# erlgo/openair4G

Measured on AMD Instinct MI355X. Metric: DL subframes/sec (20 MHz, 2x2, 64-QAM), higher is better.
Workload: dtype int16; 1 GPU; dlsim 20 MHz 2x2 TM3 (LARGE_CDD) 64-QAM MCS19x2CW, 2x14 IDFT-2048; config_id=C3, global_batch=8192, subframe_index=7, full_grid=False, parallelism=subframe-sharded x1

## Files before the change

include/oai4g.h:

```cpp
#ifndef OAI4G_H
#define OAI4G_H

#include <stddef.h>
#include <stdint.h>

#ifdef __cplusplus
extern "C" {
#endif

#define OAI4G_LTE_NULL 2
#define OAI4G_NSOFT 1827072
#define OAI4G_MAX_SEGMENTS 16
#define OAI4G_MAX_CHANNEL_BITS (14 * 1200 * 6)
#define OAI4G_D_BYTES (96 + 12 + 3 + 3 * 6144)
#define OAI4G_W_BYTES (3 * 6144 + 96)

enum {
  OAI4G_SISO = 0,
  OAI4G_ALAMOUTI = 1,
  OAI4G_LARGE_CDD = 2,
  OAI4G_UNIFORM_PRECODING11 = 3,
  OAI4G_UNIFORM_PRECODING1m1 = 4,
  OAI4G_UNIFORM_PRECODING1j = 5,
  OAI4G_UNIFORM_PRECODING1mj = 6,
  OAI4G_PUSCH_PRECODING0 = 7,
  OAI4G_PUSCH_PRECODING1 = 8
};
enum { OAI4G_CYCLIC_PREFIX = 0, OAI4G_CYCLIC_SUFFIX = 1, OAI4G_ZEROS = 2, OAI4G_NONE = 3 };

typedef struct {
  uint16_t N_RB_DL;
  uint16_t Nid_cell;
  uint8_t Ncp;
  uint8_t nushift;
  uint8_t mode1_flag;
  uint8_t nb_antennas_tx;
  uint8_t frame_type;
  uint8_t symbols_per_tti;
  uint8_t log2_symbol_size;
  uint8_t Nid_cell_mbsfn;
  uint16_t ofdm_symbol_size;
  uint16_t first_carrier_offset;
  uint16_t nb_prefix_samples;
  uint16_t nb_prefix_samples0;
  uint32_t samples_per_tti;
  uint8_t phich_resource;
  uint8_t phich_duration;
  uint8_t tdd_config;
  uint8_t nb_antennas_tx_eNB;
} oai4g_frame_parms_t;

typedef struct {
  uint8_t dci_length;
  uint8_t L;
  int32_t nCCE;
  uint8_t ra_flag;
  uint16_t rnti;
  uint32_t format;
  uint8_t dci_pdu[8];
} oai4g_dci_alloc_t;

typedef struct {
  uint32_t TBS;
  uint32_t B;
  uint8_t *b;
  uint8_t *c[OAI4G_MAX_SEGMENTS];
  uint32_t RTC[OAI4G_MAX_SEGMENTS];
  uint8_t round;
  uint8_t mcs;
  uint8_t rvidx;
  uint8_t mimo_mode;
  uint32_t rb_alloc[4];
  uint16_t nb_rb;
  uint8_t *e;
  uint8_t *d[OAI4G_MAX_SEGMENTS];
  uint8_t *w[OAI4G_MAX_SEGMENTS];
  uint32_t C, Cminus, Cplus, Kminus, Kplus, F;
  uint8_t Nl;
  uint8_t Nlayers;
  uint8_t first_layer;
  uint16_t pmi_alloc;
} oai4g_dl_harq_t;

typedef struct {
  uint16_t rnti;
  uint8_t current_harq_pid;
  uint8_t Mdlharq;
  uint8_t Kmimo;
  int16_t sqrt_rho_a;
  int16_t sqrt_rho_b;
  oai4g_dl_harq_t *harq_processes[8];
} oai4g_dlsch_t;

int oai4g_init(void);
const char *oai4g_last_error(void);
int oai4g_device_name(char *buf, int len);

int oai4g_init_frame_parms(oai4g_frame_parms_t *fp, uint16_t N_RB_DL, uint16_t Nid_cell, uint8_t Ncp,
                           uint8_t nb_antennas_tx, uint8_t mode1_flag, uint8_t frame_type);
uint8_t oai4g_get_Qm(uint8_t mcs);
int oai4g_get_G(const oai4g_frame_parms_t *fp, uint16_t nb_rb, const uint32_t *rb_alloc, uint8_t mod_order,
                uint8_t Nl, uint8_t num_pdcch_symbols, int frame, uint8_t subframe);
uint8_t oai4g_get_Qm_ul(uint8_t mcs);
uint8_t oai4g_get_I_TBS(uint8_t mcs);
uint8_t oai4g_get_I_TBS_UL(uint8_t mcs);
uint32_t oai4g_tbs_bits(uint8_t I_TBS, uint16_t nb_rb);
uint32_t oai4g_get_TBS_DL(uint8_t mcs, uint16_t nb_rb);
uint32_t oai4g_get_TBS_UL(uint8_t mcs, uint16_t nb_rb);
oai4g_dlsch_t *oai4g_new_dlsch(uint8_t Kmimo, uint8_t Mdlharq, uint8_t N_RB_DL);
void oai4g_free_dlsch(oai4g_dlsch_t *dlsch);
uint32_t oai4g_lte_gold_generic(uint32_t *x1, uint32_t *x2, uint8_t reset);
int oai4g_qpp_fold32(uint32_t K, uint32_t *s, uint16_t *tab);
int oai4g_rsc_scan_rows(uint32_t q, uint32_t rows[6]);
int oai4g_rm_pair_schedule(uint32_t C, uint32_t n0, const uint32_t nt[2], const uint32_t wrapt[2],
                           uint32_t *pairs, uint32_t *pair0);
int oai4g_mod_item_map(uint32_t item, uint32_t ips, uint32_t lz, uint32_t per, uint32_t *sf, uint32_t *l,
                       uint32_t *pair);
uint8_t oai4g_get_pmi(uint8_t N_RB_DL, uint8_t mimo_mode, uint16_t pmi_alloc, uint16_t rb);
void oai4g_set_modofdm_grid_cap(int n_workgroups);

uint32_t oai4g_crc24a(const uint8_t *in, int bitlen);
uint32_t oai4g_crc24b(const uint8_t *in, int bitlen);
int oai4g_lte_segmentation(const uint8_t *input_buffer, uint8_t **output_buffers, uint32_t B, uint32_t *C,
                           uint32_t *Cplus, uint32_t *Cminus, uint32_t *Kplus, uint32_t *Kminus, uint32_t *F);
void oai4g_threegpplte_turbo_encoder(const uint8_t *input, uint16_t input_length_bytes, uint8_t *output,
                                     uint8_t F, uint16_t interleaver_f1, uint16_t interleaver_f2);
uint32_t oai4g_sub_block_interleaving_turbo(uint32_t D, uint8_t *d, uint8_t *w);
uint32_t oai4g_lte_rate_matching_turbo(uint32_t RTC, uint32_t G, const uint8_t *w, uint8_t *e, uint8_t C,
                                       uint32_t Nsoft, uint8_t Mdlharq, uint8_t Kmimo, uint8_t rvidx,
                                       uint8_t Qm, uint8_t Nl, uint8_t r, uint8_t nb_rb, uint8_t m);
int oai4g_dlsch_encoding(uint8_t *a, const oai4g_frame_parms_t *frame_parms, uint8_t num_pdcch_symbols,
                         oai4g_dlsch_t *dlsch, int frame, uint8_t subframe);
void oai4g_dlsch_scrambling(const oai4g_frame_parms_t *frame_parms, int mbsfn_flag, oai4g_dlsch_t *dlsch, int G,
                            uint8_t q, uint8_t Ns);
int oai4g_dlsch_modulation(int32_t **txdataF, int16_t amp, uint32_t subframe_offset,
                           const oai4g_frame_parms_t *frame_parms, uint8_t num_pdcch_symbols,
                           oai4g_dlsch_t *dlsch0, oai4g_dlsch_t *dlsch1);
void oai4g_PHY_ofdm_mod(const int32_t *input, int32_t *output, uint8_t log2fftsize, uint8_t nb_symbols,
                        uint16_t nb_prefix_samples, int etype);
void oai4g_normal_prefix_mod(const int32_t *txdataF, int32_t *txdata, uint8_t nsymb,
                             const oai4g_frame_parms_t *frame_parms);
void oai4g_do_OFDM_mod(int32_t **txdataF, int32_t **txdata, uint32_t frame, uint16_t next_slot,
                       const oai4g_frame_parms_t *frame_parms);
void oai4g_generate_pilots(int32_t **txdataF, int16_t amp, const oai4g_frame_parms_t *frame_parms, uint16_t Ntti);
int oai4g_lte_dl_cell_spec(int32_t *output, int16_t amp, const oai4g_frame_parms_t *frame_parms, uint8_t Ns,
                           uint8_t l, uint8_t p);
int oai4g_idft(int log2n, const int16_t *x, int16_t *y, int scale);
void oai4g_idft2048(const int16_t *x, int16_t *y, int scale);
void oai4g_idft1024(const int16_t *x, int16_t *y, int scale);
void oai4g_idft512(const int16_t *x, int16_t *y, int scale);
void oai4g_idft256(const int16_t *x, int16_t *y, int scale);
void oai4g_idft128(const int16_t *x, int16_t *y, int scale);
void oai4g_idft64(const int16_t *x, int16_t *y, int scale);

void oai4g_generate_pcfich_reg_mapping(const oai4g_frame_parms_t *frame_parms, uint16_t pcfich_reg[4],
                                       uint8_t *pcfich_first_reg_idx);
int oai4g_generate_pcfich(uint8_t num_pdcch_symbols, int16_t amp, const oai4g_frame_parms_t *frame_parms,
                          int32_t **txdataF, uint8_t subframe);

uint8_t oai4g_get_mi(const oai4g_frame_parms_t *frame_parms, uint8_t subframe);
uint16_t oai4g_get_nquad(uint8_t num_pdcch_symbols, const oai4g_frame_parms_t *frame_parms, uint8_t mi);
uint16_t oai4g_get_nCCE(uint8_t num_pdcch_symbols, const oai4g_frame_parms_t *frame_parms, uint8_t mi);
uint8_t oai4g_get_num_pdcch_symbols(uint8_t num_dci, const oai4g_dci_alloc_t *dci_alloc,
                                    const oai4g_frame_parms_t *frame_parms, uint8_t subframe);
int oai4g_generate_phich_reg_mapping(const oai4g_frame_parms_t *frame_parms, uint16_t phich_reg[56][3]);
void oai4g_init_nCCE_table(void);
int oai4g_get_nCCE_offset(uint8_t L, int nCCE, int common_dci, uint16_t rnti, uint8_t subframe);
uint8_t oai4g_generate_dci_top(uint8_t num_ue_spec_dci, uint8_t num_common_dci, const oai4g_dci_alloc_t *dci_alloc,
                               uint32_t n_rnti, int16_t amp, const oai4g_frame_parms_t *frame_parms,
                               int32_t **txdataF, uint32_t subframe);

int oai4g_phy_viterbi_lte(const int8_t *y, uint8_t *decoded_bytes, uint16_t n);
int oai4g_diag_viterbi_lte(const int8_t *y, uint16_t n, uint8_t *decoded, uint8_t metrics[64], uint8_t *start_state);
int oai4g_cc_rx_plan(uint32_t D, uint16_t *plan);
int oai4g_dci_decoding(uint8_t DCI_LENGTH, uint8_t aggregation_level, const int8_t *e, uint8_t *decoded_output);
int oai4g_dci_decoding_crc(uint8_t DCI_LENGTH, uint8_t aggregation_level, const int8_t *e, uint8_t *decoded_output,
                           uint16_t *crc);
int oai4g_pbch_decode(const int8_t *llr, const oai4g_frame_parms_t *frame_parms, uint8_t frame_mod4,
                      uint8_t decoded_output[3]);
int oai4g_pbch_decode_batch(const int8_t *d_llr, int n, const oai4g_frame_parms_t *frame_parms,
                            const uint8_t *d_frame_mod4, uint8_t *d_out, void *stream);

int oai4g_pdcch_soft_bit_table(const oai4g_frame_parms_t *frame_parms, uint8_t subframe, uint8_t num_pdcch_symbols,
                               uint32_t *table, uint32_t cap);
int oai4g_pdcch_soft_bits(const int32_t *rxdataF_comp, const oai4g_frame_parms_t *frame_parms, uint8_t subframe,
                          uint8_t num_pdcch_symbols, int8_t *e_rx);
int oai4g_pdcch_candidates(const oai4g_frame_parms_t *frame_parms, uint8_t num_pdcch_symbols, uint8_t subframe,
                           uint16_t crnti, int do_common, uint8_t L, uint16_t *cce, int cap);
int oai4g_dci_decoding_procedure0(const int8_t *e_rx, uint8_t num_pdcch_symbols, uint16_t crnti, uint8_t *nCCE,
                                  int do_common, uint8_t subframe, oai4g_dci_alloc_t *dci_alloc,
                                  const oai4g_frame_parms_t *frame_parms, uint8_t mi, uint16_t si_rnti, uint16_t ra_rnti,
                                  uint8_t L, uint8_t format_si, uint8_t format_ra, uint8_t format_c, uint8_t sizeof_bits,
                                  uint8_t sizeof_bytes, uint8_t *dci_cnt, uint8_t *format0_found, uint8_t *format_c_found,
                                  uint32_t *CCEmap0, uint32_t *CCEmap1, uint32_t *CCEmap2);

typedef struct {
  uint8_t do_common, L, sizeof_bits, sizeof_bytes, format_si, format_ra, format_c, stop_if_found;
} oai4g_pdcch_plan_t;
#define OAI4G_PDCCH_MAX_DCI 8
typedef struct {
  uint8_t dci_cnt, format0_found, format_c_found;
  uint8_t overflow;
  int32_t nCCE;
  uint32_t CCEmap[3];
  oai4g_dci_alloc_t dci[OAI4G_PDCCH_MAX_DCI];
} oai4g_pdcch_rx_result_t;
typedef struct oai4g_pdcch_rx_config oai4g_pdcch_rx_config_t;
oai4g_pdcch_rx_config_t *oai4g_pdcch_rx_config_create(const oai4g_frame_parms_t *frame_parms, uint8_t num_pdcch_symbols,
                                                      uint16_t crnti, uint16_t si_rnti, uint16_t ra_rnti,
                                                      const oai4g_pdcch_plan_t *plan, int n_plan);
void oai4g_pdcch_rx_config_destroy(oai4g_pdcch_rx_config_t *cfg);
int oai4g_pdcch_rx_candidates(const oai4g_pdcch_rx_config_t *cfg, uint8_t subframe, uint16_t *cce, uint8_t *plan_entry,
                              int cap);
int oai4g_pdcch_rx_batch(oai4g_pdcch_rx_config_t *cfg, const int32_t *d_comp, int n_sf, int first_subframe,
                         oai4g_pdcch_rx_result_t *d_out, void *stream);
int oai4g_pdcch_rx_batch_detected(oai4g_pdcch_rx_config_t *const cfg[3], const int32_t *d_comp, const uint8_t *d_cfi,
                                  int n_sf, int first_subframe, int subframe_step, oai4g_pdcch_rx_result_t *d_out,
                                  void *stream);

int oai4g_rx_pdcch_front(int32_t *const *rxdataF, int32_t *const *dl_ch_estimates, const oai4g_frame_parms_t *frame_parms,
                         uint8_t nb_antennas_rx, uint8_t subframe, uint8_t mimo_mode, uint32_t high_speed_flag,
                         int32_t *rxdataF_comp, uint8_t *log2_maxh, uint8_t *num_pdcch_symbols, int32_t *diag_planes);
int oai4g_rx_pcfich(const oai4g_frame_parms_t *frame_parms, uint8_t subframe, const int32_t *rxdataF_comp, uint8_t mimo_mode);
int oai4g_rx_pdcch(int32_t *const *rxdataF, int32_t *const *dl_ch_estimates, const oai4g_frame_parms_t *frame_parms,
                   uint8_t nb_antennas_rx, uint8_t subframe, uint8_t mimo_mode, uint32_t high_speed_flag, int8_t *e_rx,
                   uint8_t *num_pdcch_symbols);
typedef struct oai4g_pdcch_front_config oai4g_pdcch_front_config_t;
oai4g_pdcch_front_config_t *oai4g_pdcch_front_config_create(const oai4g_frame_parms_t *frame_parms, uint8_t nb_antennas_rx,
                                                            uint8_t mimo_mode, uint32_t high_speed_flag,
                                                            uint8_t first_subframe, uint8_t subframe_step);
void oai4g_pdcch_front_config_destroy(oai4g_pdcch_front_config_t *cfg);
int oai4g_pdcch_front_batch(const oai4g_pdcch_front_config_t *cfg, int n_sf, const int32_t *d_rxdataF,
                            const int32_t *const d_est[4], int32_t *d_comp, uint8_t *d_cfi, uint8_t *d_log2_maxh,
                            void *stream);

int oai4g_rx_pbch_front(int32_t *const *rxdataF, int32_t *const *dl_ch_estimates, const oai4g_frame_parms_t *frame_parms,
                        uint8_t nb_antennas_rx, uint8_t nb_ports, uint8_t mimo_mode, uint32_t high_speed_flag,
                        int32_t *rxdataF_comp, uint8_t log2_maxh[4], int8_t *llr, int32_t *diag_planes);
int oai4g_rx_pbch(int32_t *const *rxdataF, int32_t *const *dl_ch_estimates, const oai4g_frame_parms_t *frame_parms,
                  uint8_t nb_antennas_rx, uint8_t nb_ports, uint8_t mimo_mode, uint32_t high_speed_flag,
                  uint8_t frame_mod4, uint8_t decoded_output[3]);
typedef struct oai4g_pbch_front_config oai4g_pbch_front_config_t;
oai4g_pbch_front_config_t *oai4g_pbch_front_config_create(const oai4g_frame_parms_t *frame_parms, uint8_t nb_antennas_rx,
                                                          uint8_t nb_ports, uint32_t high_speed_flag);
void oai4g_pbch_front_config_destroy(oai4g_pbch_front_config_t *cfg);
int oai4g_pbch_front_batch(const oai4g_pbch_front_config_t *cfg, int n, const int32_t *d_rxdataF,
                           const int32_t *const d_est[4], int8_t *d_llr, uint8_t *d_log2_maxh, void *stream);
typedef struct {
  uint8_t tx_ant;
  uint8_t frame_mod4, mimo_mode;
  uint8_t mib[3];
  uint8_t pad[2];
} oai4g_pbch_detect_t;
int oai4g_pbch_detect_batch(oai4g_pbch_front_config_t *cfg, int n, const int8_t *d_llr, oai4g_pbch_detect_t *d_out,
                            void *stream);

int oai4g_lte_sync_time_replicas(const oai4g_frame_parms_t *frame_parms, int32_t *out);
typedef struct oai4g_sync_config oai4g_sync_config_t;
oai4g_sync_config_t *oai4g_sync_config_create(const oai4g_frame_parms_t *frame_parms, uint8_t nb_antennas_rx);
void oai4g_sync_config_destroy(oai4g_sync_config_t *cfg);
int oai4g_sync_time_batch(oai4g_sync_config_t *cfg, int n, const int32_t *d_rx, int32_t *d_peak, int32_t *d_corr,
                          void *stream);
int oai4g_lte_sync_time(int32_t *const *rxdata, const oai4g_frame_parms_t *frame_parms, uint8_t nb_antennas_rx, int *eNB_id,
                        uint32_t *peak_val, int32_t *sync_corr);

int oai4g_fep_offset_batch(const oai4g_frame_parms_t *frame_parms, int n, int nb_antennas_rx, const int32_t *d_rx,
                           const int32_t *d_offset, uint32_t offset_stride, uint8_t first_slot, int nsym, int32_t *d_rxF,
                           size_t frame_stride, void *stream);
typedef struct {
  int32_t Nid_cell, rx_offset, metric, flip, phase, status;
} oai4g_cell_t;
int oai4g_sss_batch(oai4g_sync_config_t *cfg, int n, const int32_t *d_rx, const int32_t *d_peak, oai4g_cell_t *d_cell,
// ... 362 lines not shown
```

openair4g_amd/__init__.py:

```python
import ctypes
import os

import numpy as np

_HERE = os.path.dirname(os.path.abspath(__file__))
LIB_PATH = os.path.join(_HERE, "lib", "libopenair4g_amd.so")

LTE_NULL = 2
NSOFT = 1827072
MAX_SEGMENTS = 16
MAX_CHANNEL_BITS = 14 * 1200 * 6
D_BYTES = 96 + 12 + 3 + 3 * 6144
W_BYTES = 3 * 6144 + 96
SISO, ALAMOUTI, LARGE_CDD = 0, 1, 2
(UNIFORM_PRECODING11, UNIFORM_PRECODING1m1, UNIFORM_PRECODING1j, UNIFORM_PRECODING1mj, PUSCH_PRECODING0,
 PUSCH_PRECODING1) = 3, 4, 5, 6, 7, 8
CYCLIC_PREFIX = 0


class OAI4GError(RuntimeError):
    pass


u8p = ctypes.POINTER(ctypes.c_uint8)
# ... 168 lines not shown
                                                       ctypes.c_uint8, ctypes.c_uint8, ctypes.c_uint8, ctypes.c_uint8]),
    "oai4g_chest_filters": (None, [ctypes.c_uint8, ctypes.c_void_p]),
    "oai4g_chest_dc_filters": (None, [ctypes.c_uint8, ctypes.c_void_p]),
    "oai4g_ul_config_set_decoder": (ctypes.c_int, [ctypes.c_void_p, ctypes.c_int]),
    "oai4g_set_device": (ctypes.c_int, [ctypes.c_int]),
    "oai4g_dist_unique_id": (ctypes.c_int, [ctypes.c_void_p]),
    "oai4g_dist_init": (ctypes.c_int, [ctypes.c_int, ctypes.c_int, ctypes.c_void_p]),
    "oai4g_dist_broadcast_params": (ctypes.c_int, [ctypes.c_void_p, ctypes.c_int]),
    "oai4g_dist_allreduce_sum_u64": (ctypes.c_int, [ctypes.c_void_p, ctypes.c_int]),
    "oai4g_dist_allreduce_max_f64": (ctypes.c_int, [ctypes.c_void_p, ctypes.c_int]),
    "oai4g_dist_barrier": (ctypes.c_int, []),
    "oai4g_dist_rank": (ctypes.c_int, []),
    "oai4g_dist_world": (ctypes.c_int, []),
    "oai4g_dist_finalize": (ctypes.c_int, []),
    "oai4g_shard_range": (None, [ctypes.c_int, ctypes.c_int, ctypes.c_int, ctypes.POINTER(ctypes.c_int),
                                 ctypes.POINTER(ctypes.c_int)]),
    "oai4g_payload_seed": (ctypes.c_uint64, [ctypes.c_uint64, ctypes.c_uint64, ctypes.c_uint32, ctypes.c_uint32]),
    "oai4g_chest_config_set_stride": (ctypes.c_int, [ctypes.c_void_p, ctypes.c_uint32, ctypes.c_uint32]),
    "oai4g_rx_pdsch_tm3": (ctypes.c_int, [ctypes.POINTER(FrameParms), ctypes.c_int, ctypes.c_void_p, ctypes.c_void_p,
                                          ctypes.c_void_p, ctypes.c_uint8, ctypes.c_uint8, ctypes.c_uint8,
                                          ctypes.c_uint8, ctypes.c_uint8, ctypes.c_void_p, ctypes.c_void_p]),
    "oai4g_rx_config_create_tm3": (ctypes.c_void_p, [ctypes.POINTER(FrameParms), ctypes.c_void_p, ctypes.c_uint8,
                                                     ctypes.c_uint8, ctypes.c_uint8, ctypes.c_uint8, ctypes.c_uint16,
                                                     ctypes.c_uint8, ctypes.c_uint8, ctypes.c_uint8]),
    "oai4g_rx_batch_tm3": (ctypes.c_int, [ctypes.c_void_p, ctypes.c_int, ctypes.c_void_p, ctypes.c_void_p,
                                          ctypes.c_void_p, ctypes.c_int, ctypes.c_void_p]),
    "oai4g_rx_pdsch_tm3_2cw": (ctypes.c_int, [ctypes.POINTER(FrameParms), ctypes.c_int, ctypes.c_void_p,
                                              ctypes.c_void_p, ctypes.c_void_p, ctypes.c_uint8, ctypes.c_uint8,
                                              ctypes.c_uint8, ctypes.c_void_p, ctypes.c_void_p, ctypes.c_void_p]),
    "oai4g_rx_batch_tm3_2cw": (ctypes.c_int, [ctypes.c_void_p, ctypes.c_int, ctypes.c_void_p, ctypes.c_void_p,
                                              ctypes.c_void_p, ctypes.c_void_p, ctypes.c_int, ctypes.c_void_p]),
    "oai4g_rx_pdsch_tm2": (ctypes.c_int, [ctypes.POINTER(FrameParms), ctypes.c_int, ctypes.c_void_p, ctypes.c_void_p,
                                          ctypes.c_void_p, ctypes.c_uint8, ctypes.c_uint8, ctypes.c_uint8,
                                          ctypes.c_void_p, ctypes.c_void_p]),
    "oai4g_rx_config_create_tm2": (ctypes.c_void_p, [ctypes.POINTER(FrameParms), ctypes.c_void_p, ctypes.c_uint8,
                                                     ctypes.c_uint8, ctypes.c_uint16, ctypes.c_uint8, ctypes.c_uint8,
                                                     ctypes.c_uint8]),
    "oai4g_rx_batch_tm2": (ctypes.c_int, [ctypes.c_void_p, ctypes.c_int, ctypes.c_void_p, ctypes.c_void_p,
                                          ctypes.c_void_p, ctypes.c_int, ctypes.c_void_p]),
    "oai4g_rx_pdsch_tm56": (ctypes.c_int, [ctypes.POINTER(FrameParms), ctypes.c_int, ctypes.c_void_p, ctypes.c_void_p,
                                           ctypes.c_void_p, ctypes.c_uint8, ctypes.c_uint8, ctypes.c_uint16,
                                           ctypes.c_uint8, ctypes.c_uint8, ctypes.c_uint8, ctypes.c_void_p,
                                           ctypes.c_void_p]),
    "oai4g_rx_config_create_tm56": (ctypes.c_void_p, [ctypes.POINTER(FrameParms), ctypes.c_void_p, ctypes.c_uint8,
                                                      ctypes.c_uint8, ctypes.c_uint16, ctypes.c_int, ctypes.c_uint8,
                                                      ctypes.c_uint8, ctypes.c_uint16, ctypes.c_uint8, ctypes.c_uint8,
                                                      ctypes.c_uint8]),
    "oai4g_rx_batch_tm56": (ctypes.c_int, [ctypes.c_void_p, ctypes.c_int, ctypes.c_void_p, ctypes.c_void_p,
                                           ctypes.c_void_p, ctypes.c_int, ctypes.c_void_p]),
    "oai4g_rx_batch_tm56_pilots": (ctypes.c_int, [ctypes.c_void_p, ctypes.c_int, ctypes.c_void_p, ctypes.c_void_p,
                                                  ctypes.c_void_p, ctypes.c_int, ctypes.c_void_p]),
    "oai4g_dl_ch_estimates_time": (ctypes.c_int, [ctypes.POINTER(FrameParms), ctypes.c_int, ctypes.c_void_p,
                                                  ctypes.c_void_p]),
    "oai4g_chest_time_batch": (ctypes.c_int, [ctypes.POINTER(FrameParms), ctypes.c_int, ctypes.c_void_p,
                                              ctypes.c_size_t, ctypes.c_void_p, ctypes.c_size_t, ctypes.c_void_p]),
    "oai4g_lte_est_freq_offset": (ctypes.c_int, [ctypes.c_void_p, ctypes.POINTER(FrameParms), ctypes.c_int,
                                                 ctypes.POINTER(ctypes.c_int), ctypes.c_int]),
    "oai4g_freq_offset_omega_batch": (ctypes.c_int, [ctypes.POINTER(FrameParms), ctypes.c_int, ctypes.c_void_p,
                                                     ctypes.c_size_t, ctypes.c_int, ctypes.c_void_p, ctypes.c_void_p]),
    "oai4g_freq_offset_update": (ctypes.c_int, [ctypes.POINTER(FrameParms), ctypes.c_int32,
                                                ctypes.POINTER(ctypes.c_int), ctypes.POINTER(ctypes.c_int)]),
    "oai4g_signal_energy": (ctypes.c_int32, [ctypes.c_void_p, ctypes.c_uint32]),
    "oai4g_signal_energy_batch": (ctypes.c_int, [ctypes.c_void_p, ctypes.c_int, ctypes.c_size_t, ctypes.c_uint32,
                                                 ctypes.c_void_p, ctypes.c_void_p]),
    "oai4g_awgn_batch": (ctypes.c_int, [ctypes.c_void_p, ctypes.c_size_t, ctypes.c_uint32, ctypes.c_void_p,
                                        ctypes.c_uint32, ctypes.c_void_p, ctypes.c_size_t, ctypes.c_int,
                                        ctypes.c_void_p, ctypes.c_double, ctypes.c_uint64, ctypes.c_uint32,
                                        ctypes.c_void_p]),
    "oai4g_chest_config_create": (ctypes.c_void_p, [ctypes.POINTER(FrameParms), ctypes.c_uint8, ctypes.c_uint8,
                                                    ctypes.c_uint8]),
    "oai4g_chest_config_destroy": (None, [ctypes.c_void_p]),
    "oai4g_rx_batch_estimated": (ctypes.c_int, [ctypes.c_void_p, ctypes.c_void_p, ctypes.c_int, ctypes.c_void_p,
                                                ctypes.c_void_p, ctypes.c_int, ctypes.c_void_p]),
    "oai4g_chest_batch": (ctypes.c_int, [ctypes.c_void_p, ctypes.c_int, ctypes.c_void_p, ctypes.c_void_p,
                                         ctypes.c_void_p]),
    "oai4g_chest_batch_pilots": (ctypes.c_int, [ctypes.c_void_p, ctypes.c_int, ctypes.c_void_p, ctypes.c_void_p,
                                                ctypes.c_void_p]),
    "oai4g_rx_batch_tm3_pilots": (ctypes.c_int, [ctypes.c_void_p, ctypes.c_int, ctypes.c_void_p, ctypes.c_void_p,
                                                 ctypes.c_void_p, ctypes.c_int, ctypes.c_void_p]),
    "oai4g_rx_batch_tm3_2cw_pilots": (ctypes.c_int, [ctypes.c_void_p, ctypes.c_int, ctypes.c_void_p, ctypes.c_void_p,
                                                     ctypes.c_void_p, ctypes.c_void_p, ctypes.c_int, ctypes.c_void_p]),
    "oai4g_phy_threegpplte_turbo_decoder8": (ctypes.c_uint8, [ctypes.c_void_p, ctypes.c_void_p, ctypes.c_uint16,
                                                              ctypes.c_uint16, ctypes.c_uint16, ctypes.c_uint8,
                                                              ctypes.c_uint8, ctypes.c_uint8]),
    "oai4g_td8_scratch_bytes": (ctypes.c_size_t, [ctypes.c_uint16, ctypes.c_int]),
    "oai4g_td8_batch": (ctypes.c_int, [ctypes.c_int, ctypes.c_uint16, ctypes.c_void_p, ctypes.c_size_t, ctypes.c_void_p,
                                       ctypes.c_size_t, ctypes.c_void_p, ctypes.c_uint8, ctypes.c_uint8, ctypes.c_uint8,
                                       ctypes.c_void_p, ctypes.c_void_p]),
    "oai4g_generate_dummy_w": (ctypes.c_uint32, [ctypes.c_uint32, ctypes.c_void_p, ctypes.c_uint8]),
    "oai4g_ul_config_create": (ctypes.c_void_p, [ctypes.c_uint32, ctypes.c_uint32, ctypes.c_uint8, ctypes.c_uint8,
                                                 ctypes.c_uint8, ctypes.c_uint32, ctypes.c_uint8]),
    "oai4g_ul_config_destroy": (None, [ctypes.c_void_p]),
    "oai4g_ul_config_C": (ctypes.c_int, [ctypes.c_void_p]),
    "oai4g_ul_config_E": (ctypes.c_uint32, [ctypes.c_void_p, ctypes.c_int]),
    "oai4g_ul_config_G_offset": (ctypes.c_uint32, [ctypes.c_void_p, ctypes.c_int]),
    "oai4g_ul_decode_batch": (ctypes.c_int, [ctypes.c_void_p, ctypes.c_int, ctypes.c_void_p, ctypes.c_size_t,
                                             ctypes.c_void_p, ctypes.c_size_t, ctypes.c_void_p, ctypes.c_void_p]),
    "oai4g_ul_config_w_entries": (ctypes.c_size_t, [ctypes.c_void_p]),
    "oai4g_ul_decode_batch_harq": (ctypes.c_int, [ctypes.c_void_p, ctypes.c_int, ctypes.c_void_p, ctypes.c_size_t,
                                                  ctypes.c_void_p, ctypes.c_size_t, ctypes.c_uint8, ctypes.c_uint8,
                                                  ctypes.c_void_p, ctypes.c_size_t, ctypes.c_void_p, ctypes.c_void_p]),
    "oai4g_dft": (ctypes.c_int, [ctypes.c_int, ctypes.c_void_p, ctypes.c_void_p, ctypes.c_int]),
    "oai4g_dft2048": (None, [ctypes.c_void_p, ctypes.c_void_p, ctypes.c_int]),
    "oai4g_dft1024": (None, [ctypes.c_void_p, ctypes.c_void_p, ctypes.c_int]),
    "oai4g_dft512": (None, [ctypes.c_void_p, ctypes.c_void_p, ctypes.c_int]),
    "oai4g_dft256": (None, [ctypes.c_void_p, ctypes.c_void_p, ctypes.c_int]),
    "oai4g_dft128": (None, [ctypes.c_void_p, ctypes.c_void_p, ctypes.c_int]),
    "oai4g_dft64": (None, [ctypes.c_void_p, ctypes.c_void_p, ctypes.c_int]),
    "oai4g_slot_fep_offset": (ctypes.c_int64, [ctypes.POINTER(FrameParms), ctypes.c_uint8, ctypes.c_uint8,
                                               ctypes.c_int, ctypes.c_int]),
    "oai4g_slot_fep": (ctypes.c_int, [ctypes.POINTER(ctypes.c_void_p), ctypes.POINTER(ctypes.c_void_p),
                                      ctypes.POINTER(FrameParms), ctypes.c_uint8, ctypes.c_uint8, ctypes.c_uint8,
                                      ctypes.c_int, ctypes.c_int]),
    "oai4g_fep_batch": (ctypes.c_int, [ctypes.POINTER(FrameParms), ctypes.c_int, ctypes.c_int, ctypes.c_void_p,
                                       ctypes.c_void_p, ctypes.c_void_p]),
    "oai4g_tx_config_create": (ctypes.c_void_p, [ctypes.POINTER(TxParams)]),
    "oai4g_tx_config_destroy": (None, [ctypes.c_void_p]),
    "oai4g_tx_G": (ctypes.c_uint32, [ctypes.c_void_p, ctypes.c_int, ctypes.c_int]),
    "oai4g_tx_ebits_words": (ctypes.c_uint32, [ctypes.c_void_p]),
    "oai4g_tx_iq_samples": (ctypes.c_uint32, [ctypes.c_void_p]),
    "oai4g_tx_workspace_bytes": (ctypes.c_size_t, [ctypes.c_void_p, ctypes.c_int]),
    "oai4g_tx_batch": (ctypes.c_int, [ctypes.c_void_p, ctypes.c_int, ctypes.c_void_p, ctypes.c_void_p,
                                      ctypes.c_void_p, ctypes.c_void_p]),
    "oai4g_tx_batch_timed": (ctypes.c_int, [ctypes.c_void_p, ctypes.c_int, ctypes.c_void_p, ctypes.c_void_p,
                                            ctypes.c_void_p, ctypes.c_void_p, ctypes.POINTER(ctypes.c_float)]),
    "oai4g_tx_encode": (ctypes.c_int, [ctypes.c_void_p, ctypes.c_int, ctypes.c_void_p, ctypes.c_void_p,
                                       ctypes.c_void_p]),
    "oai4g_tx_modulate": (ctypes.c_int, [ctypes.c_void_p, ctypes.c_int, ctypes.c_void_p, ctypes.c_void_p,
                                         ctypes.c_void_p]),
    "oai4g_tx_mod_nosat": (ctypes.c_int, [ctypes.c_void_p]),
    "oai4g_diag_encode_phase_ms": (ctypes.c_int, [ctypes.c_void_p, ctypes.c_int, ctypes.c_void_p, ctypes.c_void_p,
                                                  ctypes.c_int, ctypes.c_int, ctypes.POINTER(ctypes.c_float)]),
    "oai4g_diag_encode_occupancy": (ctypes.c_int, [ctypes.c_void_p, ctypes.POINTER(ctypes.c_int),
                                                   ctypes.POINTER(ctypes.c_size_t)]),
    "oai4g_diag_stream": (ctypes.c_int, [ctypes.c_void_p, ctypes.c_void_p, ctypes.c_size_t, ctypes.c_int,
                                         ctypes.c_void_p]),
    "oai4g_dev_alloc": (ctypes.c_void_p, [ctypes.c_size_t]),
    "oai4g_dev_free": (None, [ctypes.c_void_p]),
    "oai4g_memcpy_h2d": (ctypes.c_int, [ctypes.c_void_p, ctypes.c_void_p, ctypes.c_size_t]),
    "oai4g_memcpy_d2h": (ctypes.c_int, [ctypes.c_void_p, ctypes.c_void_p, ctypes.c_size_t]),
    "oai4g_memset_d": (ctypes.c_int, [ctypes.c_void_p, ctypes.c_int, ctypes.c_size_t]),
    "oai4g_sync": (ctypes.c_int, []),
    "oai4g_fill_payload": (ctypes.c_int, [ctypes.c_void_p, ctypes.c_size_t, ctypes.c_uint64, ctypes.c_void_p]),
    "oai4g_qpp_fold32": (ctypes.c_int, [ctypes.c_uint32, ctypes.POINTER(ctypes.c_uint32), ctypes.c_void_p]),
    "oai4g_rsc_scan_rows": (ctypes.c_int, [ctypes.c_uint32, ctypes.POINTER(ctypes.c_uint32)]),
    "oai4g_rm_pair_schedule": (ctypes.c_int, [ctypes.c_uint32, ctypes.c_uint32, ctypes.POINTER(ctypes.c_uint32),
                                              ctypes.POINTER(ctypes.c_uint32), ctypes.POINTER(ctypes.c_uint32),
                                              ctypes.POINTER(ctypes.c_uint32)]),
    "oai4g_mod_item_map": (ctypes.c_int, [ctypes.c_uint32, ctypes.c_uint32, ctypes.c_uint32, ctypes.c_uint32,
                                          ctypes.POINTER(ctypes.c_uint32), ctypes.POINTER(ctypes.c_uint32),
                                          ctypes.POINTER(ctypes.c_uint32)]),
    "oai4g_get_pmi": (ctypes.c_uint8, [ctypes.c_uint8, ctypes.c_uint8, ctypes.c_uint16, ctypes.c_uint16]),
    "oai4g_set_modofdm_grid_cap": (None, [ctypes.c_int]),
    "oai4g_tx_mod_lz": (ctypes.c_int, [ctypes.c_void_p]),
    "oai4g_harq_advance": (ctypes.c_int, [ctypes.c_int, ctypes.c_int, ctypes.c_uint8, ctypes.c_int, ctypes.c_int]
                           + [ctypes.c_void_p] * 8 + [ctypes.c_size_t, ctypes.c_uint64, ctypes.c_void_p]),
    "oai4g_tx_config_enable_tb_rv": (ctypes.c_int, [ctypes.c_void_p]),
    "oai4g_tx_batch_rv": (ctypes.c_int, [ctypes.c_void_p, ctypes.c_int, ctypes.c_void_p, ctypes.c_void_p,
                                         ctypes.c_void_p, ctypes.c_void_p, ctypes.c_void_p]),
    "oai4g_tx_encode_rv": (ctypes.c_int, [ctypes.c_void_p, ctypes.c_int, ctypes.c_void_p, ctypes.c_void_p,
                                          ctypes.c_void_p, ctypes.c_void_p]),
    "oai4g_ul_decode_batch_harq_tb": (ctypes.c_int, [ctypes.c_void_p, ctypes.c_int, ctypes.c_void_p, ctypes.c_size_t,
                                                     ctypes.c_void_p, ctypes.c_size_t, ctypes.c_void_p, ctypes.c_void_p,
                                                     ctypes.c_void_p, ctypes.c_size_t, ctypes.c_void_p, ctypes.c_void_p]),
    "oai4g_phy_viterbi_lte": (ctypes.c_int, [ctypes.c_void_p, ctypes.c_void_p, ctypes.c_uint16]),
    "oai4g_diag_viterbi_lte": (ctypes.c_int, [ctypes.c_void_p, ctypes.c_uint16, ctypes.c_void_p, ctypes.c_void_p,
                                              ctypes.c_void_p]),
    "oai4g_cc_rx_plan": (ctypes.c_int, [ctypes.c_uint32, ctypes.c_void_p]),
    "oai4g_dci_decoding": (ctypes.c_int, [ctypes.c_uint8, ctypes.c_uint8, ctypes.c_void_p, ctypes.c_void_p]),
    "oai4g_dci_decoding_crc": (ctypes.c_int, [ctypes.c_uint8, ctypes.c_uint8, ctypes.c_void_p, ctypes.c_void_p,
                                              ctypes.POINTER(ctypes.c_uint16)]),
    "oai4g_pbch_decode": (ctypes.c_int, [ctypes.c_void_p, ctypes.POINTER(FrameParms), ctypes.c_uint8, ctypes.c_void_p]),
    "oai4g_pbch_decode_batch": (ctypes.c_int, [ctypes.c_void_p, ctypes.c_int, ctypes.POINTER(FrameParms),
                                               ctypes.c_void_p, ctypes.c_void_p, ctypes.c_void_p]),
    "oai4g_pdcch_soft_bit_table": (ctypes.c_int, [ctypes.POINTER(FrameParms), ctypes.c_uint8, ctypes.c_uint8,
                                                  ctypes.c_void_p, ctypes.c_uint32]),
    "oai4g_pdcch_soft_bits": (ctypes.c_int, [ctypes.c_void_p, ctypes.POINTER(FrameParms), ctypes.c_uint8, ctypes.c_uint8,
                                             ctypes.c_void_p]),
    "oai4g_dci_decoding_procedure0": (ctypes.c_int, [ctypes.c_void_p, ctypes.c_uint8, ctypes.c_uint16, ctypes.c_void_p,
                                                     ctypes.c_int, ctypes.c_uint8, ctypes.c_void_p,
                                                     ctypes.POINTER(FrameParms), ctypes.c_uint8, ctypes.c_uint16,
                                                     ctypes.c_uint16] + [ctypes.c_uint8] * 6 + [ctypes.c_void_p] * 6),
    "oai4g_pdcch_candidates": (ctypes.c_int, [ctypes.POINTER(FrameParms), ctypes.c_uint8, ctypes.c_uint8, ctypes.c_uint16,
                                              ctypes.c_int, ctypes.c_uint8, ctypes.c_void_p, ctypes.c_int]),
    "oai4g_pdcch_rx_config_create": (ctypes.c_void_p, [ctypes.POINTER(FrameParms), ctypes.c_uint8, ctypes.c_uint16,
                                                       ctypes.c_uint16, ctypes.c_uint16, ctypes.c_void_p, ctypes.c_int]),
    "oai4g_pdcch_rx_config_destroy": (None, [ctypes.c_void_p]),
    "oai4g_pdcch_rx_candidates": (ctypes.c_int, [ctypes.c_void_p, ctypes.c_uint8, ctypes.c_void_p, ctypes.c_void_p,
                                                 ctypes.c_int]),
    "oai4g_pdcch_rx_batch": (ctypes.c_int, [ctypes.c_void_p, ctypes.c_void_p, ctypes.c_int, ctypes.c_int, ctypes.c_void_p,
                                            ctypes.c_void_p]),
    "oai4g_pdcch_rx_batch_detected": (ctypes.c_int, [ctypes.POINTER(ctypes.c_void_p), ctypes.c_void_p, ctypes.c_void_p,
                                                     ctypes.c_int, ctypes.c_int, ctypes.c_int, ctypes.c_void_p,
                                                     ctypes.c_void_p]),
    "oai4g_rx_pdcch_front": (ctypes.c_int, [ctypes.POINTER(ctypes.c_void_p), ctypes.POINTER(ctypes.c_void_p),
                                            ctypes.POINTER(FrameParms), ctypes.c_uint8, ctypes.c_uint8, ctypes.c_uint8,
                                            ctypes.c_uint32, ctypes.c_void_p, ctypes.POINTER(ctypes.c_uint8),
                                            ctypes.POINTER(ctypes.c_uint8), ctypes.c_void_p]),
    "oai4g_rx_pcfich": (ctypes.c_int, [ctypes.POINTER(FrameParms), ctypes.c_uint8, ctypes.c_void_p, ctypes.c_uint8]),
    "oai4g_rx_pdcch": (ctypes.c_int, [ctypes.POINTER(ctypes.c_void_p), ctypes.POINTER(ctypes.c_void_p),
                                      ctypes.POINTER(FrameParms), ctypes.c_uint8, ctypes.c_uint8, ctypes.c_uint8,
                                      ctypes.c_uint32, ctypes.c_void_p, ctypes.POINTER(ctypes.c_uint8)]),
    "oai4g_pdcch_front_config_create": (ctypes.c_void_p, [ctypes.POINTER(FrameParms), ctypes.c_uint8, ctypes.c_uint8,
                                                          ctypes.c_uint32, ctypes.c_uint8, ctypes.c_uint8]),
    "oai4g_pdcch_front_config_destroy": (None, [ctypes.c_void_p]),
    "oai4g_pdcch_front_batch": (ctypes.c_int, [ctypes.c_void_p, ctypes.c_int, ctypes.c_void_p,
                                               ctypes.POINTER(ctypes.c_void_p), ctypes.c_void_p, ctypes.c_void_p,
                                               ctypes.c_void_p, ctypes.c_void_p]),
    "oai4g_rx_pbch_front": (ctypes.c_int, [ctypes.POINTER(ctypes.c_void_p), ctypes.POINTER(ctypes.c_void_p),
                                           ctypes.POINTER(FrameParms), ctypes.c_uint8, ctypes.c_uint8, ctypes.c_uint8,
                                           ctypes.c_uint32, ctypes.c_void_p, ctypes.c_void_p, ctypes.c_void_p,
                                           ctypes.c_void_p]),
    "oai4g_rx_pbch": (ctypes.c_int, [ctypes.POINTER(ctypes.c_void_p), ctypes.POINTER(ctypes.c_void_p),
                                     ctypes.POINTER(FrameParms), ctypes.c_uint8, ctypes.c_uint8, ctypes.c_uint8,
                                     ctypes.c_uint32, ctypes.c_uint8, ctypes.c_void_p]),
    "oai4g_pbch_front_config_create": (ctypes.c_void_p, [ctypes.POINTER(FrameParms), ctypes.c_uint8, ctypes.c_uint8,
                                                         ctypes.c_uint32]),
    "oai4g_pbch_front_config_destroy": (None, [ctypes.c_void_p]),
    "oai4g_pbch_front_batch": (ctypes.c_int, [ctypes.c_void_p, ctypes.c_int, ctypes.c_void_p,
                                              ctypes.POINTER(ctypes.c_void_p), ctypes.c_void_p, ctypes.c_void_p,
                                              ctypes.c_void_p]),
    "oai4g_pbch_detect_batch": (ctypes.c_int, [ctypes.c_void_p, ctypes.c_int, ctypes.c_void_p, ctypes.c_void_p,
                                               ctypes.c_void_p]),
    "oai4g_lte_sync_time_replicas": (ctypes.c_int, [ctypes.POINTER(FrameParms), ctypes.c_void_p]),
    "oai4g_sync_config_create": (ctypes.c_void_p, [ctypes.POINTER(FrameParms), ctypes.c_uint8]),
    "oai4g_sync_config_destroy": (None, [ctypes.c_void_p]),
    "oai4g_sync_time_batch": (ctypes.c_int, [ctypes.c_void_p, ctypes.c_int, ctypes.c_void_p, ctypes.c_void_p,
                                             ctypes.c_void_p, ctypes.c_void_p]),
    "oai4g_lte_sync_time": (ctypes.c_int, [ctypes.POINTER(ctypes.c_void_p), ctypes.POINTER(FrameParms), ctypes.c_uint8,
                                           ctypes.POINTER(ctypes.c_int), ctypes.POINTER(ctypes.c_uint32),
                                           ctypes.c_void_p]),
    "oai4g_fep_offset_batch": (ctypes.c_int, [ctypes.POINTER(FrameParms), ctypes.c_int, ctypes.c_int, ctypes.c_void_p,
                                              ctypes.c_void_p, ctypes.c_uint32, ctypes.c_uint8, ctypes.c_int,
                                              ctypes.c_void_p, ctypes.c_size_t, ctypes.c_void_p]),
    "oai4g_sss_batch": (ctypes.c_int, [ctypes.c_void_p, ctypes.c_int, ctypes.c_void_p, ctypes.c_void_p, ctypes.c_void_p,
                                       ctypes.c_void_p]),
    "oai4g_sss_rows_batch": (ctypes.c_int, [ctypes.c_void_p, ctypes.c_int, ctypes.c_void_p, ctypes.c_void_p,
                                            ctypes.c_void_p, ctypes.c_void_p]),
    "oai4g_rx_sss": (ctypes.c_int, [ctypes.POINTER(ctypes.c_void_p), ctypes.POINTER(FrameParms), ctypes.c_uint8,
                                    ctypes.c_uint8, ctypes.c_int, ctypes.POINTER(ctypes.c_int32),
                                    ctypes.POINTER(ctypes.c_uint8), ctypes.POINTER(ctypes.c_uint8)]),
    "oai4g_initial_sync": (ctypes.c_int, [ctypes.POINTER(ctypes.c_void_p), ctypes.POINTER(FrameParms), ctypes.c_uint8,
                                          ctypes.c_uint8, ctypes.c_uint32, ctypes.c_void_p]),
    "oai4g_rx_phich": (ctypes.c_int, [ctypes.POINTER(FrameParms), ctypes.c_uint8, ctypes.c_void_p, ctypes.c_uint8,
                                      ctypes.c_uint8, ctypes.POINTER(ctypes.c_int16)]),
    "oai4g_phich_rx_config_create": (ctypes.c_void_p, [ctypes.POINTER(FrameParms), ctypes.c_uint8, ctypes.c_uint8]),
    "oai4g_phich_rx_config_destroy": (None, [ctypes.c_void_p]),
    "oai4g_phich_rx_batch": (ctypes.c_int, [ctypes.c_void_p, ctypes.c_void_p, ctypes.c_int, ctypes.c_void_p, ctypes.c_int,
                                            ctypes.c_void_p, ctypes.c_void_p]),
    "oai4g_channel_config_create": (ctypes.c_void_p, [ctypes.c_uint8, ctypes.c_uint8, ctypes.c_int, ctypes.c_double,
                                                      ctypes.c_double, ctypes.c_int32, ctypes.c_double, ctypes.c_int]),
    "oai4g_channel_config_destroy": (None, [ctypes.c_void_p]),
    "oai4g_channel_config_query": (ctypes.c_int, [ctypes.c_void_p, ctypes.c_void_p, ctypes.c_void_p]),
    "oai4g_channel_model_describe": (ctypes.c_int, [ctypes.c_int, ctypes.c_uint8, ctypes.c_uint8, ctypes.c_double,
                                                    ctypes.c_void_p, ctypes.c_void_p]),
    "oai4g_channel_random_batch": (ctypes.c_int, [ctypes.c_void_p, ctypes.c_int, ctypes.c_uint64, ctypes.c_uint32,
                                                  ctypes.c_uint32, ctypes.c_void_p, ctypes.c_void_p]),
    "oai4g_channel_set_taps": (ctypes.c_int, [ctypes.c_void_p, ctypes.c_int, ctypes.c_int, ctypes.c_void_p, ctypes.c_void_p]),
    "oai4g_channel_get_taps": (ctypes.c_int, [ctypes.c_void_p, ctypes.c_int, ctypes.c_int, ctypes.c_void_p, ctypes.c_void_p]),
    "oai4g_multipath_batch": (ctypes.c_int, [ctypes.c_void_p, ctypes.c_int, ctypes.c_void_p, ctypes.c_size_t, ctypes.c_size_t,
                                             ctypes.c_uint32, ctypes.c_void_p, ctypes.c_uint32, ctypes.c_void_p,
                                             ctypes.c_size_t, ctypes.c_size_t, ctypes.c_uint32, ctypes.c_size_t,
                                             ctypes.c_void_p, ctypes.c_double, ctypes.c_uint64, ctypes.c_uint32,
                                             ctypes.c_void_p]),
    "oai4g_random_channel": (ctypes.c_int, [ctypes.c_void_p]),
    "oai4g_multipath_channel": (ctypes.c_int, [ctypes.c_void_p] + [ctypes.POINTER(ctypes.c_void_p)] * 4
                                + [ctypes.c_uint32, ctypes.c_uint8]),
    "oai4g_pusch_dft_plan": (ctypes.c_int, [ctypes.c_int32, ctypes.c_void_p, ctypes.c_void_p, ctypes.c_uint32]),
    "oai4g_pusch_config_create": (ctypes.c_void_p, [ctypes.POINTER(FrameParms), ctypes.c_uint16, ctypes.c_uint16, ctypes.c_uint8,
                                                    ctypes.c_uint8, ctypes.c_uint16, ctypes.c_uint8, ctypes.c_uint8]),
    "oai4g_pusch_config_destroy": (None, [ctypes.c_void_p]),
    "oai4g_pusch_mod_batch": (ctypes.c_int, [ctypes.c_void_p, ctypes.c_int, ctypes.c_void_p, ctypes.c_size_t, ctypes.c_int16,
                                             ctypes.c_void_p, ctypes.c_void_p]),
    "oai4g_pusch_dft_batch": (ctypes.c_int, [ctypes.c_void_p, ctypes.c_int, ctypes.c_void_p, ctypes.c_void_p, ctypes.c_void_p]),
    "oai4g_pusch_idft_batch": (ctypes.c_int, [ctypes.c_void_p, ctypes.c_int, ctypes.c_void_p, ctypes.c_void_p]),
    "oai4g_dft_lte": (ctypes.c_int, [ctypes.c_void_p, ctypes.c_void_p, ctypes.c_int32, ctypes.c_uint8]),
    "oai4g_pusch_dft": (ctypes.c_int, [ctypes.c_int32, ctypes.c_void_p, ctypes.c_void_p, ctypes.c_uint8]),
    "oai4g_lte_idft": (ctypes.c_int, [ctypes.POINTER(FrameParms), ctypes.c_void_p, ctypes.c_uint16]),
    "oai4g_ulsch_modulation": (ctypes.c_int, [ctypes.POINTER(ctypes.c_void_p), ctypes.c_int16, ctypes.c_uint32, ctypes.c_uint32,
                                              ctypes.POINTER(FrameParms), ctypes.c_void_p]),
}


def load_library(path=None):
    global _lib
    if _lib is not None:
        return _lib
    path = path or os.environ.get("OAI4G_LIB") or LIB_PATH
    if not os.path.exists(path):
        raise OAI4GError(f"HIP library not built: {path} (run __graft_entry__.build())")
    lib = ctypes.CDLL(path)
    for name, (res, args) in _SIGS.items():
        fn = getattr(lib, name)
        fn.restype = res
        fn.argtypes = args
    _lib = lib
    return lib


def exported_symbols():
    return sorted(_SIGS)


def lib():
    return load_library()

# ... 1630 lines not shown
```

openair4g_amd/csrc/oai4g_encode.hip:

```cpp
#include "oai4g_internal.h"

struct rsc_tables_t {
  uint8_t next[8][16];
  uint8_t par[8][16];
  uint8_t apow[8][8];
  uint32_t hz;
  uint32_t zs[8];
  uint32_t fm[3];
};

static constexpr uint8_t rsc_step_c(uint8_t u, uint8_t s, uint8_t *out)
{
  *out = (uint8_t)((u ^ (s >> 2) ^ (s >> 1)) & 1);
  return (uint8_t)((((u << 2) ^ (s >> 1)) ^ ((s >> 1) << 2) ^ (s << 2)) & 7);
}

static constexpr rsc_tables_t make_rsc_tables()
{
  rsc_tables_t t{};
  for (int s = 0; s < 8; s++)
    for (int nib = 0; nib < 16; nib++) {
      uint8_t st = (uint8_t)s, p = 0;
      for (int b = 0; b < 4; b++) {
        uint8_t o = 0;
// ... 65 lines not shown
}

__constant__ rsc_tables_t c_rsc = k_rsc;



static __device__ __forceinline__ uint32_t bytes_to_seq(uint32_t le) { return __builtin_bswap32(__builtin_bitreverse32(le)); }

static __device__ void crc_table_init(uint32_t *tab, uint32_t poly)
{
  for (uint32_t v = threadIdx.x; v < 256; v += blockDim.x) {
    uint32_t r = v << 16;
    for (int i = 0; i < 8; i++) r = (r & 0x800000u) ? ((r << 1) ^ poly) & 0xffffffu : (r << 1) & 0xffffffu;
    tab[v] = r;
  }
}

static __device__ __forceinline__ void gold_step(uint32_t &x1, uint32_t &x2)
{
  x1 = (x1 >> 1) ^ (x1 >> 4);
  x1 = x1 ^ (x1 << 31) ^ (x1 << 28);
  x2 = (x2 >> 1) ^ (x2 >> 2) ^ (x2 >> 3) ^ (x2 >> 4);
  x2 = x2 ^ (x2 << 31) ^ (x2 << 30) ^ (x2 << 29) ^ (x2 << 28);
}

typedef const __attribute__((address_space(1))) uint32_t gu32_t;

[[maybe_unused]] static __device__ __forceinline__ void gold_generate(uint32_t *gold, uint32_t nwords, uint32_t c_init,
                                                     const uint32_t *gx1, const uint32_t *gx2j)
{
  const uint32_t l = threadIdx.x, w0 = OAI4G_GOLD_STRIDE * l;
  if (l >= OAI4G_GOLD_LANES || w0 >= nwords) return;
  const uint32_t x2i = c_init ^ ((c_init ^ (c_init >> 1) ^ (c_init >> 2) ^ (c_init >> 3)) << 31);
  gu32_t *col = (gu32_t *)(gx2j + l);
  uint32_t cv[32];
#pragma unroll
  for (int b = 0; b < 32; b++) cv[b] = col[OAI4G_GOLD_LANES * b];
  uint32_t x2 = 0;
#pragma unroll
  for (int b = 0; b < 32; b++) x2 ^= cv[b] & (0u - ((x2i >> b) & 1u));
  uint32_t x1 = *(gu32_t *)(gx1 + l);
  const uint32_t wend = min(w0 + OAI4G_GOLD_STRIDE, nwords);
  gold[w0] = x1 ^ x2;
  for (uint32_t w = w0 + 1; w < wend; w++) {
    gold_step(x1, x2);
    gold[w] = x1 ^ x2;
  }
}

static __device__ __forceinline__ uint32_t crc_step(uint32_t reg, uint32_t byte, const uint32_t *tab)
{
  return ((reg << 8) & 0xffffffu) ^ tab[((reg >> 16) ^ byte) & 0xffu];
}

static __device__ __forceinline__ uint32_t crc_mul_tab(uint32_t a, const uint32_t *t )
{
  return t[a & 15u] ^ t[16 + ((a >> 4) & 15u)] ^ t[32 + ((a >> 8) & 15u)] ^ t[48 + ((a >> 12) & 15u)] ^
         t[64 + ((a >> 16) & 15u)] ^ t[80 + ((a >> 20) & 15u)];
}

static __device__ __forceinline__ uint32_t crc_chunk(const uint8_t *buf, uint32_t nbytes, uint32_t per, uint32_t lane,
                                                     uint32_t nl, const uint32_t *tab)
{
  const int vstart = (int)(lane * per) - (int)(per * nl - nbytes);
  uint32_t reg = 0;
  for (uint32_t i = 0; i < per; i += 4) {
    uint32_t b[4];
#pragma unroll
    for (int q = 0; q < 4; q++) {
      const int idx = vstart + (int)i + q;
      b[q] = idx >= 0 ? (uint32_t)buf[idx] : 0u;
    }
#pragma unroll
    for (int q = 0; q < 4; q++) reg = crc_step(reg, b[q], tab);
  }
  return reg;
}

static __device__ __forceinline__ uint32_t crc_stream_word(const uint32_t *base32, uint32_t start, int o)
{
  const uint32_t ad = start + (uint32_t)(o > 0 ? o : 0), wi = ad >> 2;
  uint32_t w = __builtin_amdgcn_alignbit(base32[wi + 1], base32[wi], (ad & 3u) * 8u);
  if (o < 0) w = o <= -4 ? 0u : w << (8 * (uint32_t)(-o));
  return w;
}

static __device__ __forceinline__ void crc_chunk_w2r(const uint32_t *base32, uint32_t start, uint32_t nbytes,
                                                     uint32_t per, uint32_t pos, uint32_t nl, const uint8_t *r2a,
                                                     const uint8_t *r2b, uint32_t &ra, uint32_t &rb)
{
  const int vstart = (int)(pos * per) - (int)(per * nl - nbytes);
  uint32_t a = 0, b = 0;
  for (uint32_t i = 0; i < per; i += 4) {
    const uint32_t w = crc_stream_word(base32, start, vstart + (int)i);
    const uint32_t x[4] = {w << 2, w >> 6, w >> 14, w >> 22};
#pragma unroll
    for (int q = 0; q < 4; q++) {
      a = (a >> 8) ^ *(const uint32_t *)(r2a + ((a ^ x[q]) & 0x3fcu));
      b = (b >> 8) ^ *(const uint32_t *)(r2b + ((b ^ x[q]) & 0x3fcu));
    }
  }
  ra = __builtin_bitreverse32(a >> 2) >> 8;
  rb = __builtin_bitreverse32(b >> 2) >> 8;
}

static __device__ __forceinline__ uint32_t crc_chunk_w1r(const uint32_t *base32, uint32_t start, uint32_t nbytes,
                                                         uint32_t per, uint32_t pos, uint32_t nl, const uint8_t *r2a)
{
  const int vstart = (int)(pos * per) - (int)(per * nl - nbytes);
  uint32_t a = 0;
  for (uint32_t i = 0; i < per; i += 4) {
    const uint32_t w = crc_stream_word(base32, start, vstart + (int)i);
    const uint32_t x[4] = {w << 2, w >> 6, w >> 14, w >> 22};
#pragma unroll
    for (int q = 0; q < 4; q++) a = (a >> 8) ^ *(const uint32_t *)(r2a + ((a ^ x[q]) & 0x3fcu));
  }
  return __builtin_bitreverse32(a >> 2) >> 8;
}

static __device__ __forceinline__ uint32_t crc_step_r2(uint32_t a, uint32_t byte, const uint8_t *r2)
{
  return (a >> 8) ^ *(const uint32_t *)(r2 + ((a ^ (__builtin_bitreverse32(byte) >> 22)) & 0x3fcu));
}

static __device__ __forceinline__ void crc_group_tree2(uint32_t &ra, uint32_t &rb, uint32_t pos, uint32_t lpb,
                                                       const uint32_t (*ma)[8][96], const uint32_t (*mb)[8][96])
{
  const uint32_t j0 = 7 - (pos & 7), j1 = (lpb >> 3) - 1 - (pos >> 3);
  ra = crc_mul_tab(ra, ma[0][j0]);
  rb = crc_mul_tab(rb, mb[0][j0]);
#pragma unroll
  for (int m = 1; m < 8; m <<= 1) {
    ra ^= __shfl_xor(ra, m, 64);
    rb ^= __shfl_xor(rb, m, 64);
  }
  ra = crc_mul_tab(ra, ma[1][j1]);
  rb = crc_mul_tab(rb, mb[1][j1]);
  for (uint32_t m = 8; m < lpb; m <<= 1) {
    ra ^= __shfl_xor(ra, (int)m, 64);
    rb ^= __shfl_xor(rb, (int)m, 64);
  }
}

[[maybe_unused]] static __device__ __forceinline__ uint32_t crc_wave_tree(uint32_t reg, const uint32_t *mul)
{
  const uint32_t lane = threadIdx.x & 63;
  for (int d = 0; d < 6; d++) {
    uint32_t other = __shfl_down(reg, 1u << d, 64);
    if ((lane & ((2u << d) - 1u)) == 0) reg = crc_mul_tab(reg, mul + d * 96) ^ other;
  }
  return reg;
}

static __device__ __forceinline__ uint32_t crc_wave_tree2(uint32_t reg, const uint32_t (*mul)[8][96])
{
  const uint32_t lane = threadIdx.x & 63;
  reg = crc_mul_tab(reg, mul[0][7 - (lane & 7)]);
  reg ^= __shfl_xor(reg, 1, 64);
  reg ^= __shfl_xor(reg, 2, 64);
  reg ^= __shfl_xor(reg, 4, 64);
  reg = crc_mul_tab(reg, mul[1][7 - (lane >> 3)]);
  reg ^= __shfl_xor(reg, 8, 64);
  reg ^= __shfl_xor(reg, 16, 64);
  reg ^= __shfl_xor(reg, 32, 64);
  return reg;
}

static __device__ __forceinline__ uint32_t crc_mulmod(uint32_t a, uint32_t b, uint32_t poly)
{
  uint32_t r = 0;
  for (int i = 23; i >= 0; i--) {
    r <<= 1;
    if (r & 0x1000000u) r ^= 0x1000000u | poly;
    if ((b >> i) & 1u) r ^= a;
  }
  return r;
}

static __device__ uint32_t crc24_wave(const uint8_t *buf, uint32_t nbytes, uint32_t poly, const uint32_t *tab)
{
  const uint32_t lane = threadIdx.x & 63;
  uint32_t per = (((nbytes + 63) >> 6) + 3) & ~3u;
  if (nbytes == 0) return 0;
  uint32_t reg = crc_chunk(buf, nbytes, per, lane, 64, tab);
  uint32_t m = 1;
  for (uint32_t i = 0; i < per; i++) m = crc_step(m, 0, tab);
  for (int d = 0; d < 6; d++) {
    uint32_t other = __shfl_down(reg, 1u << d, 64);
    if ((lane & ((2u << d) - 1u)) == 0) reg = crc_mulmod(reg, m, poly) ^ other;
    m = crc_mulmod(m, m, poly);
  }
  return __shfl(reg, 0, 64);
}

struct enc_tabs_t {
  uint8_t next[8][16];
  uint8_t par[8][16];
  uint8_t apow[8][8];
  uint32_t zs[8];
};

static __device__ __forceinline__ uint32_t qpp_start(uint32_t K, uint32_t f1, uint32_t f2, uint32_t j)
{
  uint32_t k = 32 * j;
  uint32_t pi = (((f2 * k) % K) * k + f1 * k) % K;
  uint32_t dl = (f1 + ((f2 * ((2 * k + 1) % K)) % K)) % K;
  return pi | (dl << 16);
}

static __device__ __forceinline__ uint32_t qpp_gather_word(const uint32_t *sys, uint32_t K, uint32_t start,
                                                           uint32_t d2, uint32_t j)
{
  uint32_t pi = start & 0xffffu, dl = start >> 16, word = 0;
#pragma unroll
  for (int b = 0; b < 32; b++) {
    word |= __builtin_amdgcn_ubfe(sys[pi >> 5], pi & 31u, 1u) << b;
    pi += dl;
    pi = min(pi, pi - K);
    dl += d2;
    dl = min(dl, dl - K);
  }
  const uint32_t n = K - 32 * j;
  return n >= 32 ? word : word & ((1u << n) - 1u);
}

static __device__ __forceinline__ void turbo_segment(const uint32_t *in, uint32_t *par_out, uint32_t K,
                                                     uint32_t *tail_out, const enc_tabs_t *tb)
{
  const uint32_t lane = threadIdx.x & 63;
  const uint32_t nch = (K + 31) >> 5;
  const uint32_t lq = nch <= 64 ? 0 : (nch <= 128 ? 1 : 2), qp = 1u << lq;
  uint32_t u[4], v[4];
  uint32_t S = 0;
#pragma unroll
  for (int t = 0; t < 4; t++) {
    u[t] = 0;
    uint32_t j = lane * qp + t;
    if (t < (int)qp && j < nch) u[t] = in[j];
    v[t] = rsc_feedback_word(u[t]);
    if (t < (int)qp) S = tb->apow[0][S] ^ (v[t] >> 29);
  }
#pragma unroll
  for (int d = 0; d < 6; d++) {
    uint32_t other = __shfl_up(S, 1u << d, 64);
    uint32_t ln = lane;
    asm volatile("" : "+v"(ln));
    S ^= tb->apow[lq + d][ln >= (1u << d) ? other : 0u];
  }
  uint32_t s = __shfl_up(S, 1, 64);
  if (lane == 0) s = 0;
#pragma unroll
  for (int t = 0; t < 4; t++) {
    uint32_t j = lane * qp + t;
    if (t < (int)qp && j < nch) {
      uint32_t n = min(32u, K - 32 * j);
      uint32_t par = rsc_parity_of_feedback(v[t]) ^ tb->zs[s];
      if (n < 32) {
        par &= (1u << n) - 1u;
        for (uint32_t q = 0; q < (n >> 2); q++) s = tb->next[s][(u[t] >> (4 * q)) & 15u];
      } else {
        s = tb->apow[0][s] ^ (v[t] >> 29);
      }
      par_out[j] = par;
      if (j == nch - 1) {
        uint32_t tbits = 0;
        for (int stp = 0; stp < 3; stp++) {
          uint32_t z = ((s >> 2) ^ s) & 1u, x = (s ^ (s >> 1)) & 1u;
          s >>= 1;
          tbits |= (x << (2 * stp)) | (z << (2 * stp + 1));
        }
        *tail_out = tbits;
      }
    }
  }
}

static constexpr uint32_t rsc_prop_packed(uint32_t n)
{
  uint32_t w = 0;
  for (uint32_t s = 0; s < 8; s++) {
    uint8_t st = (uint8_t)s;
    for (uint32_t i = 0; i < n % 7; i++) {
      uint8_t o = 0;
      st = rsc_step_c(0, st, &o);
    }
    w |= (uint32_t)st << (4 * s);
  }
  return w;
}
static_assert(rsc_prop_packed(7) == 0x76543210u && rsc_prop_packed(1) != 0x76543210u, "RSC zero-input period");

static __device__ __forceinline__ uint32_t rsc_prop(uint32_t packed, uint32_t s) { return (packed >> (4 * s)) & 7u; }

extern "C" int oai4g_rsc_scan_rows(uint32_t q, uint32_t rows[6])
{
  if (q < 1 || q > 3) return -1;
  for (uint32_t d = 0; d < 6; d++) rows[d] = rsc_prop_packed((32 * q) << d);
  return 0;
}

template <int Q>
static __device__ __forceinline__ void turbo_segment32(const uint32_t *in, uint32_t *par_out, uint32_t nch,
                                                       uint32_t *tail_out, const enc_tabs_t *tb)
{
  constexpr uint32_t A1 = rsc_prop_packed(32), AQinv = rsc_prop_packed(7 - (32 * Q) % 7);
  const uint32_t lane = threadIdx.x & 63, j0 = lane * Q, last = nch - 1;
  uint32_t v[Q], S = 0;
#pragma unroll
  for (int t = 0; t < Q; t++) {
    v[t] = rsc_feedback_word(in[min(j0 + t, last)]);
    S = (t ? rsc_prop(A1, S) : 0u) ^ (v[t] >> 29);
  }
  const uint32_t Sloc = S;
#pragma unroll
  for (int d = 0; d < 6; d++) {
    const uint32_t o = (uint32_t)__builtin_amdgcn_ds_bpermute((int)((lane - (1u << d)) << 2), (int)S);
    uint32_t ln = lane;
    asm volatile("" : "+v"(ln));
    S ^= rsc_prop(rsc_prop_packed((32u * Q) << d), ln >= (1u << d) ? o : 0u);
  }
  uint32_t s = rsc_prop(AQinv, S ^ Sloc), fin = 0;
  uint32_t par[Q];
#pragma unroll
  for (int t = 0; t < Q; t++) {
    const uint32_t j = j0 + t;
    const uint32_t p = rsc_parity_of_feedback(v[t]) ^ tb->zs[s];
    s = rsc_prop(A1, s) ^ (v[t] >> 29);
    par[t] = (t == 0 || j < nch) ? p : 0u;
    fin = j == last ? s : fin;
  }
  uint32_t tbits = 0;
#pragma unroll
  for (int stp = 0; stp < 3; stp++) {
    const uint32_t z = ((fin >> 2) ^ fin) & 1u, x = (fin ^ (fin >> 1)) & 1u;
    fin >>= 1;
    tbits |= (x << (2 * stp)) | (z << (2 * stp + 1));
  }
  if (j0 < nch) {
#pragma unroll
    for (int t = 0; t < Q; t++) par_out[j0 + t] = par[t];
  }
  if (last - j0 < (uint32_t)Q) *tail_out = tbits;
}

static __device__ __forceinline__ uint32_t tail_bit(const uint32_t *tails, uint32_t r, uint32_t m)
{
  return m < 6 ? (tails[2 * r] >> m) & 1u : (tails[2 * r + 1] >> (m - 6)) & 1u;
}

static __device__ __forceinline__ uint32_t dstream_bit(const uint32_t *blk, uint32_t sw, const uint32_t *tails,
                                                       uint32_t r, uint32_t K, uint32_t s, uint32_t idx)
{
  if (idx < K) return (blk[s * sw + (idx >> 5)] >> (idx & 31)) & 1u;
  return tail_bit(tails, r, 3 * (idx - K) + s);
}

static __device__ __forceinline__ uint32_t colperm(uint32_t col) { return __builtin_bitreverse32(col) >> 27; }

struct wwalk_t {
  uint32_t p, region, col, row, which;
};

static __device__ __forceinline__ void wwalk_init(wwalk_t &w, uint32_t p, uint32_t R, uint32_t Kpi)
{
  w.p = p;
  if (p < Kpi) {
    w.region = 0; w.col = p / R; w.row = p - w.col * R; w.which = 0;
  } else {
    uint32_t q = p - Kpi;
    w.region = 1; w.col = q / (2 * R);
    uint32_t rr = q - w.col * 2 * R;
    w.row = rr >> 1; w.which = rr & 1u;
  }
}

static __device__ __forceinline__ uint32_t wwalk_bit(const wwalk_t &w, const uint32_t *blk, uint32_t sw,
                                                     const uint32_t *tails, uint32_t r, uint32_t K, uint32_t ND,
                                                     uint32_t Kpi)
{
  uint32_t j = colperm(w.col) + 32 * w.row;
  if (w.region == 0) return dstream_bit(blk, sw, tails, r, K, 0, j - ND);
  if (w.which == 0) return dstream_bit(blk, sw, tails, r, K, 1, j - ND);
  uint32_t j2 = (j + 1 == Kpi) ? 0 : j + 1;
  return dstream_bit(blk, sw, tails, r, K, 2, j2 - ND);
}

static __device__ __forceinline__ bool wwalk_null(const wwalk_t &w, uint32_t R, uint32_t ND)
{
  if (w.row != 0) return (w.region == 1 && w.which == 1 && w.col == 31 && w.row == R - 1 && ND > 0);
  uint32_t cp = colperm(w.col);
  if (w.region == 0 || w.which == 0) return cp < ND;
  return (cp + 1 < ND) || (w.col == 31 && R == 1 && ND > 0);
}

[[maybe_unused]] static __device__ __forceinline__ uint32_t sx32(const uint32_t *a, int pos)
{
  const int wi = pos >> 5;
  const uint32_t lo = a[(uint32_t)max(wi, 0)] & (wi >= 0 ? 0xffffffffu : 0u);
  const uint32_t hi = a[(uint32_t)(wi + 1)];
  return __builtin_amdgcn_alignbit(hi, lo, (uint32_t)pos & 31u);
}

#ifndef OAI4G_ENC_XOR_DPP
template <uint32_t J>
static __device__ __forceinline__ uint32_t xor_lane(uint32_t x)
{
  if constexpr (J == 1) return (uint32_t)__builtin_amdgcn_mov_dpp((int)x, 0xB1, 0xf, 0xf, false);
  else if constexpr (J == 2) return (uint32_t)__builtin_amdgcn_mov_dpp((int)x, 0x4E, 0xf, 0xf, false);
  else return (uint32_t)__builtin_amdgcn_ds_swizzle((int)x, (int)((J << 10) | 0x1f));
}
#else
template <uint32_t J>
static __device__ __forceinline__ uint32_t xor_lane(uint32_t x)
{
  if constexpr (J == 1) return (uint32_t)__builtin_amdgcn_mov_dpp((int)x, 0xB1, 0xf, 0xf, false);
  else if constexpr (J == 2) return (uint32_t)__builtin_amdgcn_mov_dpp((int)x, 0x4E, 0xf, 0xf, false);
  else if constexpr (J == 4) {
    const int m = __builtin_amdgcn_mov_dpp((int)x, 0x141, 0xf, 0xf, false);
    return (uint32_t)__builtin_amdgcn_mov_dpp(m, 0x1B, 0xf, 0xf, false);
  } else if constexpr (J == 8) {
    return (uint32_t)__builtin_amdgcn_mov_dpp((int)x, 0x128, 0xf, 0xf, false);
  } else {
    static_assert(J == 16, "xor_lane");
    const auto r = __builtin_amdgcn_permlane16_swap(x, x, false, false);
    return (threadIdx.x & 16u) ? (uint32_t)r[0] : (uint32_t)r[1];
  }
}
#endif

struct tp_lane_t {
  uint32_t sel16, sel8;
  uint32_t rot[3], mm[3];
};

static __device__ __forceinline__ tp_lane_t tp_lane(uint32_t lane32)
{
  tp_lane_t t;
  t.sel16 = (lane32 & 16u) ? 0x03020706u : 0x05040100u;
  t.sel8 = (lane32 & 8u) ? 0x03070105u : 0x06020400u;
  const uint32_t M[3] = {0x0f0f0f0fu, 0x33333333u, 0x55555555u};
#pragma unroll
  for (int k = 0; k < 3; k++) {
    const uint32_t J = 4u >> k;
    const bool hi = (lane32 & J) != 0;
    t.rot[k] = hi ? J : 32u - J;
    t.mm[k] = hi ? ~M[k] : M[k];
  }
  return t;
}

template <int K = 0>
static __device__ __forceinline__ uint32_t transpose32_t(uint32_t x, const tp_lane_t &t)
{
  if constexpr (K == 5) {
    return x;
  } else if constexpr (K < 2) {
    const uint32_t p = xor_lane<(16u >> K)>(x);
    return transpose32_t<K + 1>(__builtin_amdgcn_perm(p, x, K == 0 ? t.sel16 : t.sel8), t);
  } else {
    const uint32_t p = xor_lane<(16u >> K)>(x);
    const uint32_t sh = __builtin_amdgcn_alignbit(p, p, t.rot[K - 2]);
    uint32_t r;
    asm("v_bitop3_b32 %0, %1, %2, %3 bitop3:0xe4" : "=v"(r) : "v"(x), "v"(sh), "v"(t.mm[K - 2]));
    return transpose32_t<K + 1>(r, t);
  }
}

static __device__ __forceinline__ void or_bits(uint32_t *w, uint32_t bit, uint32_t v)
{
  if (!v) return;
  const uint32_t wi = bit >> 5, sh = bit & 31u;
  atomicOr(&w[wi], v << sh);
  if (sh && (v >> (32 - sh))) atomicOr(&w[wi + 1], v >> (32 - sh));
}

static __device__ __forceinline__ void or_bits2(uint32_t *w, uint32_t bit, uint32_t v)
{
  const uint64_t s = (uint64_t)v << (bit & 31u);
  uint32_t *p = w + (bit >> 5);
  atomicOr(p, (uint32_t)s);
  atomicOr(p + 1, (uint32_t)(s >> 32));
}

template <bool DEBUG, bool RV = false>
static __device__ void encode_codeword(const cfg_dev_t *__restrict__ c, uint32_t sf, uint32_t cwi,
                                       const uint8_t *__restrict__ payload, uint32_t *__restrict__ ebits,
                                       enc_debug_t dbg, uint32_t *lds_base, int stop_phase = 99, uint32_t sf0 = 0,
                                       const enc_rv_tab_t *__restrict__ rvt = nullptr)
{
  const cw_dev_t &cw = c->cw[cwi];
  const uint32_t tid = threadIdx.x, nth = blockDim.x, lane = tid & 63, nwaves = nth >> 6;
  const uint32_t wave = __builtin_amdgcn_readfirstlane(tid >> 6);
  const uint32_t sfi = DEBUG ? sf : (c->first_sf + (sf0 + sf) * c->sf_step) % 10;
  const uint32_t C = __builtin_amdgcn_readfirstlane(cw.C), sw = __builtin_amdgcn_readfirstlane(cw.stream_words);
  uint32_t *strm = lds_base + c->lds_a_words;
  uint32_t *crctab_a = lds_base;
  uint32_t *crctab_b = crctab_a + 256;
  uint32_t *tails = strm + c->lds_b_words;
  uint32_t *crcs = tails + 2 * OAI4G_MAX_CB;
  uint32_t *red = crcs + OAI4G_MAX_CB + 2;
  enc_tabs_t *tabs = (enc_tabs_t *)(red + 4);
  uint32_t *dbg_ebuf = (uint32_t *)(tabs + 1);
  const uint32_t G = cw.G[sfi];

  const uint32_t nw = cw.ilv_off[C], u0 = cw.u0, n0 = cw.n0;
  const uint32_t kw0 = __builtin_amdgcn_readfirstlane(cw.kw[0]), kw1 = __builtin_amdgcn_readfirstlane(cw.kw[1]);
  const uint32_t km0 = __builtin_amdgcn_readfirstlane(cw.kmag[0]), km1 = __builtin_amdgcn_readfirstlane(cw.kmag[1]);
  const uint32_t kk0 = __builtin_amdgcn_readfirstlane(cw.kk[0]), kk1 = __builtin_amdgcn_readfirstlane(cw.kk[1]);
  const uint32_t L8 = __builtin_amdgcn_readfirstlane(cw.L) >> 3, F8 = __builtin_amdgcn_readfirstlane(cw.F) >> 3;
  const uint32_t cb0 = (kk0 >> 3) - L8, cb1 = (kk1 >> 3) - L8;
  auto seg_of = [&](uint32_t r, uint32_t &fill, uint32_t &ncopy, uint32_t &s0) {
    const uint32_t ki = r >= n0 ? 1u : 0u;
    fill = r == 0 ? F8 : 0u;
    ncopy = (ki ? cb1 : cb0) - fill;
    s0 = r == 0 ? 0u : (ki ? n0 * cb0 + (r - n0) * cb1 : r * cb0) - F8;
  };

  const uint8_t *src = payload + (size_t)(DEBUG ? 0 : (sf * c->n_cw + cwi)) * c->payload_stride;
  const uint32_t Ab = cw.A_bytes;
  {
    constexpr uint32_t ENC_BLK = 6;
    const uint32_t nsl = (kw1 + 63) >> 6;
    const uint32_t lim = ((Ab + 3) & ~3u) - 4;
    for (uint32_t sl = wave; sl < nsl; sl += nwaves) {
      const uint32_t j0 = sl << 6, j = j0 + lane, i0 = 4 * j;
      for (uint32_t rb = 0; rb < C; rb += ENC_BLK) {
        uint32_t v[ENC_BLK];
#pragma unroll
        for (uint32_t u = 0; u < ENC_BLK; u++) {
          const uint32_t r = rb + u;
          v[u] = 0;
          if (r >= C) break;
          uint32_t fill, ncopy, s0;
          seg_of(r, fill, ncopy, s0);
          const uint32_t a = s0 + (i0 > fill ? i0 - fill : 0u);
          v[u] = ld_u32_any(src + min(a, lim));
        }
#pragma unroll
        for (uint32_t u = 0; u < ENC_BLK; u++) {
          const uint32_t r = rb + u;
          if (r >= C) break;
          const uint32_t kw = r < n0 ? kw0 : kw1;
          if (j0 >= kw) continue;
          uint32_t fill, ncopy, s0;
          seg_of(r, fill, ncopy, s0);
          const uint32_t nd = s0 + ncopy > Ab ? (Ab > s0 ? Ab - s0 : 0u) : ncopy;
          const uint32_t dend = fill + nd;
          uint32_t *sys = strm + r * 3 * sw;
          if ((sl == 0 && fill != 0) || 4 * (j0 + 64) > dend) {
            if (j < kw) {
              const int pre = (int)fill - (int)i0, valid = (int)dend - (int)i0;
              const uint32_t a = s0 + (pre < 0 ? (uint32_t)-pre : 0u);
              uint32_t le = v[u] >> ((8 * (a - min(a, lim))) & 31u);
              if (pre > 0) le <<= (8 * (uint32_t)pre) & 31u;
              if (valid < 4) le &= (1u << ((8 * (uint32_t)valid) & 31u)) - 1u;
              if (valid <= 0 || pre >= 4) le = 0;
              sys[j] = bytes_to_seq(le);
            }
          } else {
            sys[j] = bytes_to_seq(v[u]);
          }
        }
      }
    }
    for (uint32_t i = tid; i < C * 3 * 4; i += nth) {
      const uint32_t slot = i >> 2, r = slot / 3;
      const uint32_t w = (r < n0 ? kw0 : kw1) + (i & 3u);
      if (w < sw) strm[slot * sw + w] = 0u;
    }
    if (tid == 0) crcs[0] = 0u;
    {
      const uint32_t tv = __builtin_bitreverse32(tid) >> 24, tr = tid & 127u;
      const uint32_t ta = c->crctab[0][tv], tb = c->crctab[1][tv];
      const uint32_t rsc_n = (&c_rsc.next[0][0])[tr], rsc_p = (&c_rsc.par[0][0])[tr];
      const uint32_t rsc_a = (&c_rsc.apow[0][0])[tr & 63u], rsc_z = c_rsc.zs[tr & 7u];
      crctab_a[tid] = __builtin_bitreverse32(ta << 8) << 2;
      if (C > 1) crctab_b[tid] = __builtin_bitreverse32(tb << 8) << 2;
      if (tid < 128) {
        (&tabs->next[0][0])[tid] = (uint8_t)rsc_n;
        (&tabs->par[0][0])[tid] = (uint8_t)rsc_p;
        if (tid < 64) (&tabs->apow[0][0])[tid] = (uint8_t)rsc_a;
        if (tid < 8) tabs->zs[tid] = rsc_z;
      }
    }
  }
  __syncthreads();
  if (stop_phase <= 0) return;

  if (C > 1) {
    const uint32_t lpb = __builtin_amdgcn_readfirstlane(cw.crc_lpb), per = __builtin_amdgcn_readfirstlane(cw.crc_per_cb);
    const uint32_t pos = tid & (lpb - 1);
    for (uint32_t r = tid / lpb; r < C; r += nth / lpb) {
      uint32_t fill, n, s0;
      seg_of(r, fill, n, s0);
      if (s0 + n > Ab) n = Ab > s0 ? Ab - s0 : 0;
      uint32_t ra, rb;
      crc_chunk_w2r(strm, 4 * (r * 3 * sw) + fill, n, per, pos, lpb, (const uint8_t *)crctab_a, (const uint8_t *)crctab_b, ra,
                    rb);
      crc_group_tree2(ra, rb, pos, lpb, cw.crc2_cb[0], cw.crc2_cb[1]);
      if (pos == 0) {
        crcs[1 + r] = rb;
        atomicXor(&crcs[0], crc_mul_tab(ra, cw.crcmul_blk[r]));
      }
    }
    __syncthreads();
    if (tid >= 1 && tid < C) {
      const uint32_t r = tid - 1;
      const uint32_t v = __builtin_bitreverse32(crcs[1 + r] << 8);
      uint8_t *p = (uint8_t *)(strm + r * 3 * sw) + ((r < n0 ? kk0 : kk1) >> 3) - 3;
      p[0] = (uint8_t)v;
      p[1] = (uint8_t)(v >> 8);
      p[2] = (uint8_t)(v >> 16);
    }
    if (tid == 0) {
      const uint32_t crc = crcs[0];
      uint32_t a = __builtin_bitreverse32(crcs[C] << 8) << 2;
      const uint8_t *r2b = (const uint8_t *)crctab_b;
      a = crc_step_r2(a, crc >> 16, r2b);
      a = crc_step_r2(a, (crc >> 8) & 0xffu, r2b);
      a = crc_step_r2(a, crc & 0xffu, r2b);
      const uint32_t va = __builtin_bitreverse32(crc << 8), vb = a >> 2;
      uint8_t *p = (uint8_t *)(strm + (C - 1) * 3 * sw) + (kk1 >> 3) - 6;
      p[0] = (uint8_t)va;
      p[1] = (uint8_t)(va >> 8);
      p[2] = (uint8_t)(va >> 16);
      p[3] = (uint8_t)vb;
      p[4] = (uint8_t)(vb >> 8);
      p[5] = (uint8_t)(vb >> 16);
    }
  } else {
    const uint32_t reg = crc_wave_tree2(crc_chunk_w1r(strm, F8, Ab, cw.crc_per_tb, tid, nth, (const uint8_t *)crctab_a), cw.crc2_tb);
    if (lane == 0) red[wave] = reg;
    __syncthreads();
    if (tid == 0) {
      uint32_t v01 = crc_mul_tab(red[0], cw.crcmul_tb[6][0]) ^ red[1];
      uint32_t v23 = crc_mul_tab(red[2], cw.crcmul_tb[6][0]) ^ red[3];
      uint32_t crc = crc_mul_tab(v01, cw.crcmul_tb[7][0]) ^ v23;
      const uint32_t va = __builtin_bitreverse32(crc << 8);
      uint8_t *p = (uint8_t *)strm + F8 + Ab;
      p[0] = (uint8_t)va;
      p[1] = (uint8_t)(va >> 8);
      p[2] = (uint8_t)(va >> 16);
      if (DEBUG) crcs[0] = crc;
    }
  }
  __syncthreads();
  if (DEBUG && dbg.b) {
    for (uint32_t i = tid; i < Ab; i += nth) dbg.b[i] = src[i];
    if (tid < 3) dbg.b[Ab + tid] = (uint8_t)(crcs[0] >> (8 * (2 - tid)));
  }
  if (stop_phase <= 2) return;

  auto unit_of = [&](uint32_t i, uint32_t &r, uint32_t &j, uint32_t &K, uint32_t &ki) {
    ki = i >= u0 ? 1u : 0u;
    const uint32_t ii = ki ? i - u0 : i, kw = ki ? kw1 : kw0;
    const uint32_t rr = __umul24(ii, ki ? km1 : km0) >> 20;
    j = ii - __umul24(rr, kw);
    r = ki ? n0 + rr : rr;
    K = ki ? kk1 : kk0;
  };

  uint32_t *ilv = lds_base;
  const uint32_t fw0 = __builtin_amdgcn_readfirstlane(cw.qpp_f32[0]), fw1 = __builtin_amdgcn_readfirstlane(cw.qpp_f32[1]);
  const bool f32a = n0 != 0 && fw0 != 0, f32b = fw1 != 0;
  const uint32_t ft0 = f32a ? n0 * (kw0 >> 5) : 0u, ftn = ft0 + (f32b ? (C - n0) * (kw1 >> 5) : 0u);
  const uint32_t fm0 = fw0 >> 5, fm1 = fw1 >> 5;
  uint32_t *etab0 = strm + 2 * sw, *etab1 = strm + (n0 * 3 + 2) * sw;
  uint32_t te0 = 0, te1 = 0;
  if (f32a && tid < kw0) te0 = ((const uint16_t *)cw.qpp_tab[0])[tid];
  if (f32b && tid < kw1) te1 = ((const uint16_t *)cw.qpp_tab[1])[tid];
  auto tile_of = [&](uint32_t i, uint32_t &r, uint32_t &t, uint32_t &nt, uint32_t &ki) {
    ki = i >= ft0 ? 1u : 0u;
    const uint32_t ii = ki ? i - ft0 : i;
    nt = (ki ? kw1 : kw0) >> 5;
    const uint32_t rr = __umul24(ii, ki ? fm1 : fm0) >> 20;
    t = ii - __umul24(rr, nt);
    r = ki ? n0 + rr : rr;
  };
  if (ftn) {
    const tp_lane_t tpl = tp_lane(tid & 31);
    const uint32_t l32 = tid & 31u;
    const uint32_t sa = fw0 & 31u, sb = fw1 & 31u;
    for (uint32_t base = 0; base < ftn; base += nth >> 5) {
      uint32_t r, t, nt, ki;
      tile_of(min(base + (tid >> 5), ftn - 1), r, t, nt, ki);
      uint32_t *sys = strm + r * 3 * sw;
      const uint32_t v = sys[t + nt * (((ki ? sb : sa) * l32) & 31u)];
      sys[sw + 32 * t + l32] = transpose32_t<0>(v, tpl);
    }
    if (f32a && tid < kw0) etab0[tid] = te0;
    if (f32b && tid < kw1) etab1[tid] = te1;
  }
  for (uint32_t r = 0; r < C; r++) {
    if (r < n0 ? f32a : f32b) continue;
    const uint32_t K = r < n0 ? kk0 : kk1, Kw = (K + 31) >> 5, Q = K >> 2, io = r < n0 ? r * kw0 : u0 + (r - n0) * kw1;
    const uint32_t *sys = strm + r * 3 * sw;
    for (uint32_t w = tid; w < Kw; w += nth) ilv[io + w] = 0u;
    const uint32_t ng = (Q + 31) >> 5, nbw = (Q + 7) >> 3;
    for (uint32_t g = tid; g < ng; g += nth) {
      uint32_t P[4];
#pragma unroll
      for (uint32_t q = 0; q < 4; q++) {
        const uint32_t src = 32 * g + q * Q, wi = src >> 5;
        const uint32_t lo = sys[wi], hi = wi + 1 < Kw ? sys[wi + 1] : 0u;
        uint32_t v = __builtin_amdgcn_alignbit(hi, lo, src);
        if (src + 32 > K) v |= sys[0] << (K - src);
        P[q] = v;
      }
#pragma unroll
      for (uint32_t jb = 0; jb < 4; jb++) {
        const uint32_t t01 = __builtin_amdgcn_perm(P[1], P[0], 0x0c0c0000u | jb | ((4 + jb) << 8));
        const uint32_t t23 = __builtin_amdgcn_perm(P[3], P[2], 0x00000c0cu | (jb << 16) | ((4 + jb) << 24));
        if (4 * g + jb < nbw) strm[(r * 3 + 1) * sw + 4 * g + jb] = t01 | t23;
      }
    }
  }
  __syncthreads();
  if (ftn) {
    const tp_lane_t tpl = tp_lane(tid & 31);
    const uint32_t l32 = tid & 31u;
    for (uint32_t base = 0; base < ftn; base += nth >> 5) {
      uint32_t r, t, nt, ki;
      tile_of(min(base + (tid >> 5), ftn - 1), r, t, nt, ki);
      const uint32_t e = (ki ? etab1 : etab0)[32 * t + l32];
      const uint32_t *T = strm + (r * 3 + 1) * sw;
      const uint32_t D = *(const uint32_t *)((const uint8_t *)T + __builtin_amdgcn_ubfe(e, 5, 10));
      const uint32_t io = r < n0 ? r * kw0 : u0 + (r - n0) * kw1;
      ilv[io + t + nt * l32] = transpose32_t<0>(__builtin_amdgcn_alignbit(D, D, e), tpl);
    }
  }
  {
    const bool s3a = __builtin_amdgcn_readfirstlane(cw.qpp_s3[0]) != 0, s3b = __builtin_amdgcn_readfirstlane(cw.qpp_s3[1]) != 0;
    const uint32_t ulo = f32a ? u0 : 0u, uhi = f32b ? u0 : nw;
    for (uint32_t i = ulo + tid; i < uhi; i += nth) {
      uint32_t r, j, K, ki;
      unit_of(i, r, j, K, ki);
      const uint32_t Q = K >> 2;
      const uint4 e4 = *(const uint4 *)&cw.qpp_tab[ki][4 * j];
      const uint32_t ew[4] = {e4.x, e4.y, e4.z, e4.w};
      const uint32_t *b8 = strm + (r * 3 + 1) * sw;
      uint32_t acc = 0;
#pragma unroll
      for (int b = 0; b < 8; b++) {
        const uint32_t e = (b & 1) ? ew[b >> 1] >> 16 : ew[b >> 1];
        const uint32_t D = *(const uint32_t *)((const uint8_t *)b8 + __builtin_amdgcn_ubfe(e, 5, 10));
        acc |= __builtin_amdgcn_alignbit(D, D, e) & (0x01010101u << b);
      }
      uint32_t a0 = acc & 0xffu, a1 = (acc >> 8) & 0xffu, a2 = (acc >> 16) & 0xffu, a3 = acc >> 24;
      const uint32_t n = Q - 8 * j;
      if (n < 8) {
        const uint32_t m = (1u << n) - 1u;
        a0 &= m; a1 &= m; a2 &= m; a3 &= m;
      }
      const bool s3 = ki ? s3b : s3a;
      const uint32_t q1 = s3 ? a3 : a1, q3 = s3 ? a1 : a3;
      uint32_t *o = ilv + (i - j);
      if ((Q & 7u) == 0) {
        uint8_t *ob = (uint8_t *)o + j;
        const uint32_t qb = Q >> 3;
        ob[0] = (uint8_t)a0; ob[qb] = (uint8_t)q1; ob[2 * qb] = (uint8_t)a2; ob[3 * qb] = (uint8_t)q3;
      } else {
        or_bits(o, 8 * j, a0);
        or_bits(o, Q + 8 * j, q1);
        or_bits(o, 2 * Q + 8 * j, a2);
        or_bits(o, 3 * Q + 8 * j, q3);
      }
    }
  }
  __syncthreads();
  if (stop_phase == 23) return;

  for (uint32_t seg = wave; seg < 2 * C; seg += nwaves) {
    const uint32_t r = seg >> 1, e = seg & 1u;
    uint32_t *blk = strm + r * 3 * sw;
    const uint32_t io = r < n0 ? r * kw0 : u0 + (r - n0) * kw1;
    const uint32_t *in = e ? ilv + io : blk;
    uint32_t *par = blk + (1 + e) * sw, *tail = &tails[2 * r + e];
    const uint32_t K = r < n0 ? kk0 : kk1, nch = K >> 5;
    if (K & 31u) turbo_segment(in, par, K, tail, tabs);
    else if (nch > 128) turbo_segment32<3>(in, par, nch, tail, tabs);
    else if (nch > 64) turbo_segment32<2>(in, par, nch, tail, tabs);
    else turbo_segment32<1>(in, par, nch, tail, tabs);
  }
  __syncthreads();
  if (stop_phase <= 3) return;

  if (DEBUG) {
    for (uint32_t r = 0; r < C; r++) {
      uint32_t K = cw.K[r], R = cw.R[r], Kpi = cw.Kpi[r], ND = cw.ND[r];
      const uint32_t *blk = strm + r * 3 * sw;
      if (dbg.c)
        for (uint32_t i = tid; i < K / 8; i += nth) {
          uint32_t wv = blk[(i >> 2)];
          uint32_t byte = (wv >> (8 * (i & 3))) & 0xffu;
          dbg.c[r * (8 + 3 + 768) + i] = (uint8_t)(__builtin_bitreverse32(byte) >> 24);
        }
      if (dbg.d) {
        uint8_t *d = dbg.d + (size_t)r * OAI4G_D_BYTES;
        for (uint32_t i = tid; i < 96; i += nth) d[i] = OAI4G_LTE_NULL;
        for (uint32_t i = tid; i < 3 * K + 12; i += nth) {
          uint32_t kk = i / 3, s = i - 3 * kk;
          d[96 + i] = (uint8_t)(kk < K ? dstream_bit(blk, sw, tails, r, K, s, kk) : tail_bit(tails, r, i - 3 * K));
        }
        if (tid == 0) d[96 + 3 * (K + 4) + 2] = (uint8_t)dstream_bit(blk, sw, tails, r, K, 2, 0);
      }
      if (dbg.w) {
        uint8_t *w = dbg.w + (size_t)r * OAI4G_W_BYTES;
        for (uint32_t p = tid; p < 3 * Kpi; p += nth) {
          wwalk_t wk;
          wwalk_init(wk, p, R, Kpi);
          w[p] = wwalk_null(wk, R, ND) ? OAI4G_LTE_NULL : (uint8_t)wwalk_bit(wk, blk, sw, tails, r, K, ND, Kpi);
        }
      }
    }
    if (!dbg.e) return;
  }

  const uint32_t nd0 = __builtin_amdgcn_readfirstlane(cw.NDk[0]), nd1 = __builtin_amdgcn_readfirstlane(cw.NDk[1]);
  for (uint32_t r = tid; r < C; r += nth) {
    const uint32_t K = r < n0 ? kk0 : kk1, ND = r < n0 ? nd0 : nd1;
    uint32_t *blk = strm + r * 3 * sw;
    for (uint32_t s = 0; s < 3; s++) {
      uint32_t t4 = tail_bit(tails, r, s) | (tail_bit(tails, r, 3 + s) << 1) | (tail_bit(tails, r, 6 + s) << 2) |
                    (tail_bit(tails, r, 9 + s) << 3);
      uint32_t w0 = K >> 5, off = K & 31;
      blk[s * sw + w0] |= t4 << off;
      if (off > 28) blk[s * sw + (w0 + 1)] |= t4 >> (32 - off);
    }
    if (ND == 0) blk[2 * sw + ((K + 4) >> 5)] |= (blk[2 * sw] & 1u) << ((K + 4) & 31u);
  }
  __syncthreads();

  {
    const tp_lane_t tpl = tp_lane(tid & 31);
    const uint32_t sw3 = __builtin_amdgcn_readfirstlane(3 * sw);
    const uint32_t Nnn0 = __builtin_amdgcn_readfirstlane(cw.Nnnk[0]), Nnn1 = __builtin_amdgcn_readfirstlane(cw.Nnnk[1]);
    bool once;
    {
      const uint32_t Elo = __builtin_amdgcn_readfirstlane(cw.E[sfi][0]), Ehi = __builtin_amdgcn_readfirstlane(cw.E[sfi][C - 1]);
      const uint32_t *wrapt = RV ? rvt->rm_wrapt : cw.rm_wrapt;
      const uint32_t wrapt0 = __builtin_amdgcn_readfirstlane(wrapt[0]), wrapt1 = __builtin_amdgcn_readfirstlane(wrapt[1]);
      once = Ehi <= min(Nnn0, Nnn1) && Elo <= min(Nnn0, Nnn1) && wrapt0 != ~1u && wrapt1 != ~1u;
    }
    typedef const __attribute__((address_space(4))) uint32_t cu32_t;
    cu32_t *pdesc = (cu32_t *)(RV ? rvt->rm_pairs : cw.rm_pairs), *ppair0 = (cu32_t *)(RV ? rvt->rm_pair0 : cw.rm_pair0);
    cu32_t *pE = (cu32_t *)cw.E[sfi], *proff = (cu32_t *)cw.roff[sfi];
    gu32_t *gold = (gu32_t *)(c->gold_tab + (size_t)(sfi * c->n_cw + cwi) * c->ebits_words);
    uint32_t *eout = DEBUG ? nullptr : ebits + (size_t)(sf * c->n_cw + cwi) * c->ebits_words;
    uint32_t *ebuf = DEBUG ? dbg_ebuf : lds_base;
    const uint32_t hb = DEBUG ? C : (C + 1) >> 1, nhalf = DEBUG ? 1u : 2u;
    uint32_t carry = 0;
    for (uint32_t h = 0; h < nhalf; h++) {
      const uint32_t rb0 = h ? hb : 0, rb1 = h ? C : hb;
      const uint32_t eb0 = proff[rb0], eb1 = rb1 < C ? proff[rb1] : G;
      const uint32_t w0 = eb0 >> 5, nwh = ((eb1 + 31) >> 5) - w0;
      for (uint32_t i = tid; i < nwh + 1; i += nth) ebuf[i] = (i == 0 && h) ? carry : 0u;
      __syncthreads();
      const uint32_t pb = ppair0[rb0], pe = ppair0[rb1], bit0 = 32 * w0;
      const char *rsrc0 = (const char *)&cw.rm_src[0][0][0];
      const char *rdst0 = (const char *)(RV ? &rvt->rm_dst[0][0][0] : &cw.rm_dst[0][0][0]);
      auto pair_loop = [&](auto ONCE) {
        uint32_t P = pb + wave;
        if (P >= pe) return;
        const uint32_t plast = pe - 1;
        uint32_t d = pdesc[P], dn = pdesc[min(P + nwaves, plast)];
        uint32_t E, ro, nsrc, ndst;
        auto fetch = [&]() {
          E = pE[(d >> 2) & 15u];
          ro = proff[(d >> 2) & 15u];
          nsrc = *(const uint32_t *)(rsrc0 + ((d >> 16) + 4 * lane));
          ndst = *(const uint32_t *)(rdst0 + ((d >> 16) + 4 * lane));
        };
        fetch();
        for (;;) {
          const uint32_t src = nsrc, dst = ndst, dc = d, Ec = E, rob = ro - bit0;
          d = dn;
          dn = pdesc[min(P + 2 * nwaves, plast)];
          fetch();
          const uint32_t *bb = (const uint32_t *)((const char *)strm + (dc & 0x3cu) * sw3) - 1;
          const uint32_t *wp = bb + ((src >> 5) & 0x7fffu);
          uint32_t y = __builtin_amdgcn_alignbit(wp[1], wp[0], src);
          y = transpose32_t<0>(y, tpl);
          y >>= (dst >> 16) & 31u;
          const uint32_t o = dst & 0xffffu, m = __builtin_amdgcn_ubfe(dst, 21, 6);
          if constexpr (decltype(ONCE)::value) {
            const int l = min((int)m, (int)Ec - (int)o);
            if (l > 0) or_bits2(ebuf, rob + o, y & (0xffffffffu >> (32 - l)));
            if (dc & 1u) {
              asm volatile("" ::: "memory");
              if (dst & OAI4G_RM_DST_WRAP) {
                const uint32_t ma = ((dc & 2u) ? Nnn1 : Nnn0) - o;
                const uint32_t l2 = min(m - ma, Ec);
                or_bits2(ebuf, rob, (y >> ma) & (0xffffffffu >> (32 - l2)));
              }
            }
          } else if (m) {
            const uint32_t Nnn = (dc & 2u) ? Nnn1 : Nnn0;
            y &= 0xffffffffu >> (32 - m);
            const uint32_t ma = min(m, Nnn - o);
            for (uint32_t part = 0; part < 2; part++) {
              const uint32_t len = part ? m - ma : ma, os = part ? 0u : o;
              const uint32_t v = part ? (ma < 32 ? y >> ma : 0u) : (ma < 32 ? y & ((1u << ma) - 1u) : y);
              for (uint32_t x = os; len && x < Ec; x += Nnn) {
                const uint32_t l = min(len, Ec - x);
                or_bits(ebuf, rob + x, v & (0xffffffffu >> (32 - l)));
              }
            }
          }
          P += nwaves;
          if (P >= pe) break;
        }
      };
      if (once) pair_loop(std::true_type{});
      else pair_loop(std::false_type{});
      __syncthreads();
      if (DEBUG) {
        for (uint32_t k = tid; k < G; k += nth) dbg.e[k] = (uint8_t)((ebuf[k >> 5] >> (k & 31)) & 1u);
        return;
      }
      const uint32_t nst = stop_phase <= 4 ? 0u : ((h + 1 < nhalf && (eb1 & 31u)) ? nwh - 1 : nwh);
      for (uint32_t i = tid; i < nst; i += nth) {
        const uint32_t wi = w0 + i;
        uint32_t v = ebuf[i] ^ gold[wi];
        const uint32_t nb = min(32u, G - 32 * wi);
        if (nb < 32) v &= (1u << nb) - 1u;
        eout[wi] = v;
      }
      if (h + 1 < nhalf) {
        carry = (eb1 & 31u) ? ebuf[nwh - 1] : 0u;
        __syncthreads();
      }
    }
  }
}

__global__ void __launch_bounds__(256) __attribute__((amdgpu_num_sgpr(80))) k_encode(const cfg_dev_t *__restrict__ c, const uint8_t *__restrict__ payload,
                                                uint32_t *__restrict__ ebits, int stop_phase, uint32_t sf0)
{
  extern __shared__ uint32_t lds_dyn[];
  uint32_t sf = blockIdx.x / c->n_cw, cwi = blockIdx.x % c->n_cw;
  enc_debug_t none = {nullptr, nullptr, nullptr, nullptr, nullptr};
  encode_codeword<false>(c, sf, cwi, payload, ebits, none, lds_dyn, stop_phase, sf0);
}

__global__ void __launch_bounds__(256) __attribute__((amdgpu_num_sgpr(80))) k_encode_rv(const cfg_dev_t *__restrict__ c, const uint8_t *__restrict__ payload,
                                                const uint8_t *__restrict__ rv, const enc_rv_tab_t *__restrict__ tabs,
                                                uint32_t *__restrict__ ebits)
{
  extern __shared__ uint32_t lds_dyn[];
  uint32_t sf = blockIdx.x / c->n_cw, cwi = blockIdx.x % c->n_cw;
  const uint32_t v = __builtin_amdgcn_readfirstlane((uint32_t)rv[blockIdx.x]) & 3u;
  enc_debug_t none = {nullptr, nullptr, nullptr, nullptr, nullptr};
  encode_codeword<false, true>(c, sf, cwi, payload, ebits, none, lds_dyn, 99, 0, tabs + (v * c->n_cw + cwi));
}

__global__ void __launch_bounds__(256) k_encode_debug(const cfg_dev_t *__restrict__ c, uint32_t sf, uint32_t cwi,
                                                      const uint8_t *__restrict__ payload, enc_debug_t dbg)
{
  extern __shared__ uint32_t lds_dyn[];
  encode_codeword<true>(c, sf, cwi, payload, nullptr, dbg, lds_dyn);
}

static size_t enc_lds_bytes(const cfg_dev_t *h)
{
  size_t words = (size_t)h->lds_a_words + h->lds_b_words + 2 * OAI4G_MAX_CB + OAI4G_MAX_CB + 2 + 4;
  size_t bytes = words * 4 + sizeof(enc_tabs_t);
#ifdef OAI4G_ENC_LDS_PAD
  bytes += OAI4G_ENC_LDS_PAD;
#endif
  return (bytes + 15) & ~(size_t)15;
}

static hipError_t launch_encode_impl(const cfg_dev_t *d_cfg, const cfg_dev_t *h_cfg, int sf0, int n_sf,
                                     const uint8_t *d_payload, uint32_t *d_ebits, int stop_phase, hipStream_t s);

hipError_t oai4g_launch_encode(const cfg_dev_t *d_cfg, const cfg_dev_t *h_cfg, int sf0, int n_sf,
                               const uint8_t *d_payload, uint32_t *d_ebits, hipStream_t s)
{
  return launch_encode_impl(d_cfg, h_cfg, sf0, n_sf, d_payload, d_ebits, 99, s);
}

hipError_t oai4g_launch_encode_phase(const cfg_dev_t *d_cfg, const cfg_dev_t *h_cfg, int n_sf,
                                     const uint8_t *d_payload, uint32_t *d_ebits, int stop_phase, hipStream_t s)
{
  return launch_encode_impl(d_cfg, h_cfg, 0, n_sf, d_payload, d_ebits, stop_phase, s);
}

static hipError_t launch_encode_impl(const cfg_dev_t *d_cfg, const cfg_dev_t *h_cfg, int sf0, int n_sf,
                                     const uint8_t *d_payload, uint32_t *d_ebits, int stop_phase, hipStream_t s)
{
  if (n_sf <= 0) return hipSuccess;
  d_payload += (size_t)sf0 * h_cfg->n_cw * h_cfg->payload_stride;
  d_ebits += (size_t)sf0 * h_cfg->n_cw * h_cfg->ebits_words;
  size_t lds = enc_lds_bytes(h_cfg);
  static bool attr_set = false;
  if (!attr_set) {
    (void)hipFuncSetAttribute((const void *)k_encode, hipFuncAttributeMaxDynamicSharedMemorySize, 160 * 1024);
    (void)hipFuncSetAttribute((const void *)k_encode_debug, hipFuncAttributeMaxDynamicSharedMemorySize, 160 * 1024);
    attr_set = true;
  }
  hipLaunchKernelGGL(k_encode, dim3(n_sf * h_cfg->n_cw), dim3(256), lds, s, d_cfg, d_payload, d_ebits, stop_phase,
                     (uint32_t)sf0);
  return hipGetLastError();
}

hipError_t oai4g_launch_encode_rv(const cfg_dev_t *d_cfg, const cfg_dev_t *h_cfg, int n_sf, const uint8_t *d_payload,
                                  const uint8_t *d_rv, const enc_rv_tab_t *d_tabs, uint32_t *d_ebits, hipStream_t s)
{
  if (n_sf <= 0) return hipSuccess;
  static bool attr_set = false;
  if (!attr_set) {
    (void)hipFuncSetAttribute((const void *)k_encode_rv, hipFuncAttributeMaxDynamicSharedMemorySize, 160 * 1024);
    attr_set = true;
  }
  hipLaunchKernelGGL(k_encode_rv, dim3(n_sf * h_cfg->n_cw), dim3(256), enc_lds_bytes(h_cfg), s, d_cfg, d_payload, d_rv,
                     d_tabs, d_ebits);
  return hipGetLastError();
}

hipError_t oai4g_encode_occupancy(const cfg_dev_t *h_cfg, int *blocks_per_cu, size_t *lds_bytes)
{
  *lds_bytes = enc_lds_bytes(h_cfg);
  (void)hipFuncSetAttribute((const void *)k_encode, hipFuncAttributeMaxDynamicSharedMemorySize, 160 * 1024);
  return hipOccupancyMaxActiveBlocksPerMultiprocessor(blocks_per_cu, k_encode, 256, *lds_bytes);
}

hipError_t oai4g_launch_encode_debug(const cfg_dev_t *d_cfg, const cfg_dev_t *h_cfg, int cw, int sf,
                                     const uint8_t *d_payload, enc_debug_t dbg, hipStream_t s)
{
  size_t lds = enc_lds_bytes(h_cfg) + 4 * ((size_t)h_cfg->lds_gold_words + 1);
  (void)hipFuncSetAttribute((const void *)k_encode_debug, hipFuncAttributeMaxDynamicSharedMemorySize, 160 * 1024);
  hipLaunchKernelGGL(k_encode_debug, dim3(1), dim3(256), lds, s, d_cfg, (uint32_t)sf, (uint32_t)cw, d_payload, dbg);
  return hipGetLastError();
}


__global__ void __launch_bounds__(64) k_crc24(const uint8_t *__restrict__ in, int bitlen, uint32_t poly,
                                              uint32_t *__restrict__ out)
{
  __shared__ uint32_t tab[256];
  extern __shared__ uint8_t buf[];
  uint32_t nbytes = (uint32_t)bitlen / 8, rem = (uint32_t)bitlen % 8;
  for (uint32_t i = threadIdx.x; i < nbytes + (rem ? 1 : 0); i += blockDim.x) buf[i] = in[i];
  crc_table_init(tab, poly);
  __syncthreads();
  uint32_t reg = crc24_wave(buf, nbytes, poly, tab);
  if (threadIdx.x == 0) {
    if (rem) {
      uint32_t r32 = reg << 8;
      uint32_t idx = ((uint32_t)buf[nbytes] >> (8 - rem)) ^ (r32 >> (32 - rem));
      out[0] = (r32 << rem) ^ (tab[idx & 0xffu] << 8);
    } else {
      out[0] = reg << 8;
    }
  }
}

hipError_t oai4g_launch_crc24(const uint8_t *d_in, int bitlen, uint32_t poly_top, uint32_t *d_out, hipStream_t s)
{
  uint32_t nbytes = (uint32_t)(bitlen + 7) / 8;
  hipLaunchKernelGGL(k_crc24, dim3(1), dim3(64), nbytes + 4, s, d_in, bitlen, poly_top >> 8, d_out);
  return hipGetLastError();
}

__global__ void __launch_bounds__(256) k_turbo_bytes(const uint8_t *__restrict__ cin, uint32_t K, uint32_t f1,
                                                     uint32_t f2, uint8_t *__restrict__ dout)
{
  const uint32_t sw = 208;
  __shared__ uint32_t strm[3 * sw];
  __shared__ uint32_t tails[2];
  __shared__ enc_tabs_t tabs;
  uint32_t nw = (K + 31) >> 5;
  for (uint32_t i = threadIdx.x; i < 3 * sw; i += blockDim.x) strm[i] = 0;
  if (threadIdx.x < 128) {
    (&tabs.next[0][0])[threadIdx.x] = (&c_rsc.next[0][0])[threadIdx.x];
    (&tabs.par[0][0])[threadIdx.x] = (&c_rsc.par[0][0])[threadIdx.x];
    if (threadIdx.x < 64) (&tabs.apow[0][0])[threadIdx.x] = (&c_rsc.apow[0][0])[threadIdx.x];
    if (threadIdx.x < 8) tabs.zs[threadIdx.x] = c_rsc.zs[threadIdx.x];
  }
  __syncthreads();
  for (uint32_t j = threadIdx.x; j < nw; j += blockDim.x) {
    uint32_t le = 0;
    for (uint32_t q = 0; q < 4; q++) {
      uint32_t i = 4 * j + q;
      le |= (uint32_t)(i < K / 8 ? cin[i] : 0) << (8 * q);
    }
    uint32_t wv = bytes_to_seq(le);
    if (32 * (j + 1) > K) wv &= (1u << (K - 32 * j)) - 1u;
    strm[j] = wv;
  }
  __syncthreads();
  __shared__ uint32_t ilv[OAI4G_MAX_CHUNKS];
  const uint32_t d2 = (2 * f2) % K;
  for (uint32_t j = threadIdx.x; j < nw; j += blockDim.x) ilv[j] = qpp_gather_word(strm, K, qpp_start(K, f1, f2, j), d2, j);
  __syncthreads();
  uint32_t wave = threadIdx.x >> 6;
  if (wave < 2) turbo_segment(wave ? ilv : strm, strm + (1 + wave) * sw, K, &tails[wave], &tabs);
  __syncthreads();
  for (uint32_t i = threadIdx.x; i < 3 * K + 12; i += blockDim.x) {
    uint32_t kk = i / 3, s = i - 3 * kk;
    dout[i] = (uint8_t)(kk < K ? dstream_bit(strm, sw, tails, 0, K, s, kk) : tail_bit(tails, 0, i - 3 * K));
  }
}

hipError_t oai4g_launch_turbo_bytes(const uint8_t *d_c, int nbytes, uint8_t *d_out, uint32_t f1, uint32_t f2,
                                    hipStream_t s)
{
  hipLaunchKernelGGL(k_turbo_bytes, dim3(1), dim3(256), 0, s, d_c, (uint32_t)nbytes * 8, f1, f2, d_out);
  return hipGetLastError();
}

__global__ void __launch_bounds__(256) k_subblock_bytes(uint32_t D, const uint8_t *__restrict__ dfull,
                                                        uint8_t *__restrict__ w)
{
  uint32_t R = (D + 31) >> 5, Kpi = R << 5, ND = Kpi - D;
  const uint8_t *base = dfull + 96 - 3 * ND;
  for (uint32_t k = blockIdx.x * blockDim.x + threadIdx.x; k < Kpi; k += gridDim.x * blockDim.x) {
    uint32_t col = k / R, row = k - col * R;
    uint32_t j = colperm(col) + 32 * row;
    w[k] = base[3 * j];
    w[Kpi + 2 * k] = base[3 * j + 1];
    uint32_t i5 = 3 * j + 5;
    w[Kpi + 2 * k + 1] = (i5 == 3 * Kpi + 2) ? dfull[96 + 2] : base[i5];
    if (ND > 0 && k == Kpi - 1) w[3 * Kpi - 1] = OAI4G_LTE_NULL;
  }
}

hipError_t oai4g_launch_subblock_bytes(uint32_t D, const uint8_t *d_dfull, uint8_t *d_w, hipStream_t s)
{
  hipLaunchKernelGGL(k_subblock_bytes, dim3(32), dim3(256), 0, s, D, d_dfull, d_w);
  return hipGetLastError();
}

static __device__ __forceinline__ void rm_bytes_block(const uint8_t *__restrict__ w, uint32_t Ncb, uint32_t k0,
                                                      uint32_t E, uint8_t *__restrict__ e, uint32_t *status)
{
  extern __shared__ uint8_t comp[];
  __shared__ uint32_t wsum[4];
  __shared__ uint32_t s_start, s_total;
  const uint32_t tid = threadIdx.x, nth = blockDim.x;
  uint32_t per = (Ncb + nth - 1) / nth, a = tid * per, b = min(a + per, Ncb);
  uint32_t cnt = 0, before_k0 = 0;
  for (uint32_t i = a; i < b; i++)
    if (w[i] != OAI4G_LTE_NULL) { cnt++; if (i < k0) before_k0++; }
  uint32_t lane = tid & 63, wv = tid >> 6, incl = cnt;
  for (int off = 1; off < 64; off <<= 1) {
    uint32_t v = __shfl_up(incl, off, 64);
    if (lane >= (uint32_t)off) incl += v;
  }
  if (lane == 63) wsum[wv] = incl;
  if (tid == 0) { s_start = 0; s_total = 0; }
  __syncthreads();
  uint32_t wbase = 0;
  for (uint32_t i = 0; i < wv; i++) wbase += wsum[i];
  uint32_t excl = wbase + incl - cnt;
  uint32_t o = excl;
  for (uint32_t i = a; i < b; i++)
    if (w[i] != OAI4G_LTE_NULL) comp[o++] = w[i];
  atomicAdd(&s_start, before_k0);
  atomicAdd(&s_total, cnt);
  __syncthreads();
  uint32_t nnz = s_total, st = s_start;
  if (nnz == 0) { if (tid == 0) status[0] = 1; return; }
  for (uint32_t k = tid; k < E; k += nth) e[k] = comp[(st + k) % nnz];
  if (tid == 0) status[0] = 0;
}

__global__ void __launch_bounds__(256) k_rm_bytes(const uint8_t *__restrict__ w, uint32_t Ncb, uint32_t k0,
                                                   uint32_t E, uint8_t *__restrict__ e, uint32_t *status)
{
  rm_bytes_block(w, Ncb, k0, E, e, status);
}

__global__ void __launch_bounds__(256) k_rm_bytes_blocks(const uint8_t *__restrict__ w, const rm_blk_t *__restrict__ blk,
                                                          uint8_t *__restrict__ e, uint32_t *status)
{
  const rm_blk_t b = blk[blockIdx.x];
  if (b.E == 0) return;
  rm_bytes_block(w + b.woff, b.Ncb, b.k0, b.E, e + b.eoff, status + blockIdx.x);
}

hipError_t oai4g_launch_rm_bytes(const uint8_t *d_w, uint32_t Ncb, uint32_t k0, uint32_t E, uint8_t *d_e,
                                 uint32_t *d_status, hipStream_t s)
{
  hipLaunchKernelGGL(k_rm_bytes, dim3(1), dim3(256), (Ncb + 15) & ~15u, s, d_w, Ncb, k0, E, d_e, d_status);
  return hipGetLastError();
}

hipError_t oai4g_launch_rm_bytes_blocks(const uint8_t *d_w, const rm_blk_t *d_blk, int C, uint32_t max_Ncb, uint8_t *d_e,
                                        uint32_t *d_status, hipStream_t s)
{
  if (C <= 0) return hipSuccess;
  hipLaunchKernelGGL(k_rm_bytes_blocks, dim3(C), dim3(256), (max_Ncb + 15) & ~15u, s, d_w, d_blk, d_e, d_status);
  return hipGetLastError();
}

__global__ void __launch_bounds__(256) k_scramble_bytes(uint8_t *__restrict__ e, uint32_t n_entries, uint32_t c_init,
                                                        const uint32_t *__restrict__ gx1,
                                                        const uint32_t *__restrict__ gx2j)
{
  extern __shared__ uint32_t gold[];
  uint32_t nwords = (n_entries + 31) >> 5;
  gold_generate(gold, nwords, c_init, gx1, gx2j);
  __syncthreads();
  for (uint32_t k = threadIdx.x; k < n_entries; k += blockDim.x)
    e[k] = (uint8_t)((e[k] & 1u) ^ ((gold[k >> 5] >> (k & 31)) & 1u));
}

hipError_t oai4g_launch_scramble_bytes(uint8_t *d_e, int n_entries, uint32_t c_init, const uint32_t *d_gold_x1,
                                       const uint32_t *d_gold_x2j, hipStream_t s)
{
  uint32_t nwords = ((uint32_t)n_entries + 31) >> 5;
  if (nwords > OAI4G_MAX_GOLD_WORDS) return hipErrorInvalidValue;
  hipLaunchKernelGGL(k_scramble_bytes, dim3(1), dim3(256), nwords * 4, s, d_e, (uint32_t)n_entries, c_init,
                     d_gold_x1, d_gold_x2j);
  return hipGetLastError();
}

__global__ void k_fill(uint8_t *__restrict__ d, size_t bytes, uint64_t seed)
{
  size_t nw = bytes / 8;
  for (size_t i = blockIdx.x * (size_t)blockDim.x + threadIdx.x; i < (bytes + 7) / 8; i += (size_t)gridDim.x * blockDim.x) {
    const uint64_t z = oai4g_payload_word(seed, i);
    if (i < nw) ((uint64_t *)d)[i] = z;
    else
      for (size_t b = 0; b < bytes - 8 * i; b++) d[8 * i + b] = (uint8_t)(z >> (8 * b));
  }
}

hipError_t oai4g_launch_fill(uint8_t *d, size_t bytes, uint64_t seed, hipStream_t s)
{
  hipLaunchKernelGGL(k_fill, dim3(1024), dim3(256), 0, s, d, bytes, seed);
  return hipGetLastError();
}

__global__ void __launch_bounds__(256) k_diag_stream(const uint32_t *__restrict__ src, uint32_t *__restrict__ dst,
                                                     size_t n_words, int mode)
{
  const size_t stride = (size_t)gridDim.x * blockDim.x;
  size_t i = (size_t)blockIdx.x * blockDim.x + threadIdx.x;
  if (mode == 1) {
    for (; i < n_words; i += stride) dst[i] = (uint32_t)i;
    return;
  }
  uint32_t acc = 0;
  for (; i < n_words; i += stride) acc ^= src[i];
  if (acc == 0x9e3779b9u) dst[0] = acc;
}

hipError_t oai4g_launch_diag_stream(const void *src, void *dst, size_t bytes, int mode, hipStream_t s)
// ... 7 lines not shown
```

openair4g_amd/csrc/oai4g_host.cpp:

```cpp
#include <hip/hip_runtime.h>
#include <math.h>
#include <pthread.h>
#include <stdarg.h>
#include <stdio.h>
#include <stdlib.h>
#include <string.h>

#include <algorithm>
#include <cmath>
#include <cstdlib>
#include <vector>
#include <map>
#include <memory>
#include <mutex>
#include <vector>

#include "../../include/oai4g.h"
#include "../../include/oai4g_qpp.h"
#include "../../include/oai4g_tbs.h"
#include "oai4g_internal.h"
#include "oai4g_dev_buf.h"
#include "oai4g_rm_geom.h"

static thread_local char g_err[512] = "";
// ... 455 lines not shown
  if (*C == 1) { *Cplus = 1; *Kminus = 0; *Cminus = 0; }
  else { *Cminus = (*C * *Kplus - Bp) / (*Kplus - *Kminus); *Cplus = *C - *Cminus; }
  *F = *Cplus * *Kplus + *Cminus * *Kminus - Bp;
  return 0;
}

static const uint8_t k_colperm[32] = {0, 16, 8, 24, 4, 20, 12, 28, 2, 18, 10, 26, 6, 22, 14, 30,
                                      1, 17, 9, 25, 5, 21, 13, 29, 3, 19, 11, 27, 7, 23, 15, 31};
static int null_positions(uint32_t K, uint16_t *out, uint32_t maxn)
{
  uint32_t D = K + 4, R = (D + 31) >> 5, Kpi = R << 5, ND = Kpi - D;
  std::vector<uint8_t> d(96 + 3 * D + 16, 0);
  memset(d.data(), OAI4G_LTE_NULL, 96);
  uint8_t *dd = d.data() + 96;
  dd[3 * D + 2] = dd[2];
  const uint8_t *base = dd - 3 * ND;
  std::vector<uint8_t> w(3 * Kpi);
  uint32_t k = 0;
  for (uint32_t col = 0; col < 32; col++)
    for (uint32_t row = 0; row < R; row++, k++) {
      uint32_t j = k_colperm[col] + 32 * row;
      w[k] = base[3 * j];
      w[Kpi + 2 * k] = base[3 * j + 1];
      w[Kpi + 2 * k + 1] = base[3 * j + 5];
    }
  if (ND > 0) w[3 * Kpi - 1] = OAI4G_LTE_NULL;
  uint32_t n = 0;
  for (uint32_t p = 0; p < 3 * Kpi; p++)
    if (w[p] == OAI4G_LTE_NULL) {
      if (n >= maxn) return -1;
      out[n++] = (uint16_t)p;
    }
  return (int)n;
}

static uint32_t crc_mulmod_h(uint32_t a, uint32_t b, uint32_t poly)
{
  uint32_t r = 0;
  for (int i = 23; i >= 0; i--) {
    r <<= 1;
    if (r & 0x1000000u) r ^= 0x1000000u | poly;
    if ((b >> i) & 1u) r ^= a;
  }
  return r;
}

static uint32_t crc_xpow8_h(uint64_t n, uint32_t poly)
{
  uint32_t result = 1, base = 0x100;
  while (n) {
    if (n & 1u) result = crc_mulmod_h(result, base, poly);
    base = crc_mulmod_h(base, base, poly);
    n >>= 1;
  }
  return result;
}

static void crc_mul_tables2(uint32_t per, uint32_t poly, uint32_t (*tab)[8][96])
{
  for (int lv = 0; lv < 2; lv++)
    for (uint32_t j = 0; j < 8; j++) {
      const uint32_t m = crc_xpow8_h((uint64_t)per * j * (lv ? 8u : 1u), poly);
      for (int k = 0; k < 6; k++)
        for (uint32_t v = 0; v < 16; v++) tab[lv][j][16 * k + v] = crc_mulmod_h((v << (4 * k)) & 0xffffffu, m, poly);
    }
}

static void crc_mul_tables(uint32_t per, int levels, uint32_t poly, uint32_t (*tab)[6][16])
{
  for (int d = 0; d < levels; d++) {
    uint32_t m = crc_xpow8_h((uint64_t)per << d, poly);
    for (int k = 0; k < 6; k++)
      for (uint32_t v = 0; v < 16; v++) tab[d][k][v] = crc_mulmod_h((v << (4 * k)) & 0xffffffu, m, poly);
  }
}

static void qam_tables_scaled(int Qm, int16_t amp, int16_t srho_a, int16_t srho_b, bool alamouti, cw_dev_t &c)
{
  int32_t q16[4], q64[8];
  for (int a = -1; a <= 1; a += 2)
    for (int b = -1; b <= 1; b += 2) {
      q16[(1 + a) + (1 + b) / 2] = -a * (20724 + b * 10362);
      for (int cc = -1; cc <= 1; cc += 2)
        q64[(1 + a) * 2 + (1 + b) + (1 + cc) / 2] = -a * (20225 + b * (10112 + cc * 5056));
    }
  int16_t amp_a = (int16_t)(((int32_t)amp * srho_a) >> 13), amp_b = (int16_t)(((int32_t)amp * srho_b) >> 13);
  c.qpsk_a = (int16_t)((amp_a * 23170) >> 15);
  c.qpsk_b = (int16_t)((amp_b * 23170) >> 15);
  const int16_t sa = alamouti ? (int16_t)(((int32_t)amp_a * 23170) >> 15) : amp_a;
  const int16_t sb = alamouti ? (int16_t)(((int32_t)amp_b * 23170) >> 15) : amp_b;
  for (int i = 0; i < 8; i++) {
    const int32_t v = Qm == 4 ? q16[i & 3] : q64[i];
    c.qam_a[i] = (int16_t)((v * sa) >> 15);
    c.qam_b[i] = (int16_t)((v * sb) >> 15);
  }
  const int16_t g[2] = {c.qpsk_a, c.qpsk_b};
  for (int pil = 0; pil < 2; pil++) {
    c.alm_qpsk[pil][0] = (int16_t)(((int32_t)g[pil] * 23170) >> 15);
    c.alm_qpsk[pil][1] = (int16_t)(((int32_t)(int16_t)-g[pil] * 23170) >> 15);
  }
}

static uint32_t mod_nosat_ok(const cfg_dev_t &h, int v_static)
{
  if (h.log2N != 11 || h.nsymb != 14 || getenv("OAI4G_MOD_SAT")) return 0;
  int v = v_static;
  for (uint32_t cw = 0; cw < h.n_cw; cw++) {
    const cw_dev_t &c = h.cw[cw];
    for (int i = 0; i < 8; i++) v = std::max(v, std::max(std::abs((int)c.qam_a[i]), std::abs((int)c.qam_b[i])));
    v = std::max(v, std::max(std::abs((int)c.qpsk_a), std::abs((int)c.qpsk_b)));
    for (int i = 0; i < 2; i++)
      v = std::max(v, std::max(std::abs((int)c.alm_qpsk[i][0]), std::abs((int)c.alm_qpsk[i][1])));
  }
  const double R = std::sqrt(2.0) * v, band = 12.0 * h.N_RB_DL;
  const double c32 = std::ceil(band / 32) + 1, c8 = std::ceil(band / 8) + 1, c2 = std::ceil(band / 2) + 1;
  return (c32 * R + 128 <= 32767 && c8 * R / 8 + 128 <= 32767 && c2 * R / 16 + 128 <= 32767 &&
          (band + 1) * R / 32 + 128 <= 32767) ? 1u : 0u;
}

static int packed_iq_max(const std::vector<uint32_t> &t)
{
  int v = 0;
  for (uint32_t w : t) v = std::max(v, std::max(std::abs((int)(int16_t)(w & 0xFFFFu)), std::abs((int)(int16_t)(w >> 16))));
  return v;
}

static void mod_items_setup(cfg_dev_t &h)
{
  uint32_t lz = 0;
  if (!h.with_crs && !h.ctl_on)
    for (; lz < OAI4G_MOD_LZ_MAX && lz + 1 < h.nsymb / 2; lz++) {
      bool empty = true;
      for (int sf = 0; sf < 10 && empty; sf++) empty = h.symnre[sf][lz] == 0;
      if (!empty) break;
    }
  h.mod_lz = lz;
  h.mod_per = h.nsymb - lz;
  h.mod_permag = oai4g_mod_permag(h.mod_per);
}

extern "C" int oai4g_mod_item_map(uint32_t item, uint32_t ips, uint32_t lz, uint32_t per, uint32_t *sf, uint32_t *l,
                                  uint32_t *pair)
{
  if (ips < 1 || ips > 2 || per < 1 || lz > OAI4G_MOD_LZ_MAX) return -1;
  const oai4g_mod_item_t m = oai4g_mod_item(item, ips, lz, per, oai4g_mod_permag(per));
  *sf = m.sf;
  *l = m.l;
  *pair = m.pair;
  return m.l == lz && lz > 0 ? 1 : 0;
}

int g_modofdm_grid_cap = 0;
extern "C" void oai4g_set_modofdm_grid_cap(int n_workgroups) { g_modofdm_grid_cap = n_workgroups > 0 ? n_workgroups : 0; }

extern "C" uint8_t oai4g_get_pmi(uint8_t N_RB_DL, uint8_t mimo_mode, uint16_t pmi_alloc, uint16_t rb)
{
  const uint32_t sb = N_RB_DL == 6 ? rb : N_RB_DL == 50 ? rb / 6u : N_RB_DL == 100 ? rb >> 3 : rb >> 2;
  const uint32_t two = mimo_mode <= OAI4G_PUSCH_PRECODING1, sh = two ? sb << 1 : sb;
  return sh >= 32 ? 0 : (uint8_t)(((uint32_t)pmi_alloc >> sh) & (two ? 3u : 1u));
}

static int not_pilot(int pilots, int re, int nushift, int use2nd)
{
  int off = (pilots == 2) ? 3 : 0, v = nushift % 3;
  if (pilots == 0) return 1;
  if (use2nd) return (re != nushift + off) && (re != ((nushift + 6 + off) % 12));
  return (re != v) && (re != v + 6) && (re != v + 3) && (re != v + 9);
}

static int build_remap(const oai4g_frame_parms_t *fp, const uint32_t *rb_alloc, int num_pdcch, int subframe,
                       int mimo_mode, uint16_t pmi_alloc, uint16_t *remap , uint32_t *symbase ,
                       int *re_alloc )
{
  const bool alm = mimo_mode == OAI4G_ALAMOUTI, prec1 = oai4g_mode_prec1((uint32_t)mimo_mode);
  int ralloc = 0;
  int N = fp->ofdm_symbol_size, nsymb = fp->Ncp == 0 ? 14 : 12, half = fp->N_RB_DL >> 1;
  int use2nd = fp->mode1_flag == 1;
  for (int i = 0; i < 14 * N; i++) remap[i] = 0xFFFF;
  uint32_t total = 0;
  for (int l = 0; l < 14; l++) symbase[l] = 0;
  for (int l = num_pdcch; l < nsymb; l++) {
    symbase[l] = total;
    uint32_t idx = 0;
    int pilots;
    if (fp->Ncp == 0) pilots = (l == 4 || l == 11) ? 2 : (l == 7 ? 1 : 0);
    else pilots = (l == 3 || l == 9) ? 2 : (l == 6 ? 1 : 0);
    if (fp->nb_antennas_tx == 4 && l % (nsymb >> 1) == 1) pilots = 3;
    int re_offset = fp->first_carrier_offset;
    for (int rb = 0; rb < fp->N_RB_DL; rb++) {
      int alloc = rb_bit(rb_alloc, rb), skip_half = 0, skip_dc = 0;
      if (fp->N_RB_DL & 1) {
        skip_dc = (rb == half);
        if (subframe == 0 && rb > half - 3 && rb < half + 3 && l >= (nsymb >> 1) && l < (nsymb >> 1) + 4) alloc = 0;
        if (subframe == 0 && rb == half - 3 && l >= (nsymb >> 1) && l < (nsymb >> 1) + 4) skip_half = 1;
        else if (subframe == 0 && rb == half + 3 && l >= (nsymb >> 1) && l < (nsymb >> 1) + 4) skip_half = 2;
        if (fp->frame_type == 1) {
          if ((subframe == 0 || subframe == 5) && rb > half - 3 && rb < half + 3 && l == nsymb - 1) alloc = 0;
          if ((subframe == 0 || subframe == 5) && rb == half - 3 && l == nsymb - 1) skip_half = 1;
          else if ((subframe == 0 || subframe == 5) && rb == half + 3 && l == nsymb - 1) skip_half = 2;
          if ((subframe == 1 || subframe == 6) && rb > half - 3 && rb < half + 3 && l == 2) alloc = 0;
          if ((subframe == 1 || subframe == 6) && rb == half - 3 && l == 2) skip_half = 1;
          else if ((subframe == 1 || subframe == 6) && rb == half + 3 && l == 2) skip_half = 2;
        } else {
          int ls = (nsymb >> 1) - 1, lp = (nsymb >> 1) - 2;
          if ((subframe == 0 || subframe == 5) && rb > half - 3 && rb < half + 3 && l == ls) alloc = 0;
          if ((subframe == 0 || subframe == 5) && rb == half - 3 && l == ls) skip_half = 1;
          else if ((subframe == 0 || subframe == 5) && rb == half + 3 && l == ls) skip_half = 2;
          if ((subframe == 0 || subframe == 5) && rb > half - 3 && rb < half + 3 && l == lp) alloc = 0;
          if ((subframe == 0 || subframe == 5) && rb == half - 3 && l == lp) skip_half = 1;
          else if ((subframe == 0 || subframe == 5) && rb == half + 3 && l == lp) skip_half = 2;
        }
      } else {
        if (subframe == 0 && rb >= half - 3 && rb < half + 3 && l >= (nsymb >> 1) && l < (nsymb >> 1) + 4) alloc = 0;
        if (fp->frame_type == 1) {
          if ((subframe == 0 || subframe == 5) && rb >= half - 3 && rb < half + 3 && l == nsymb - 1) alloc = 0;
          if ((subframe == 1 || subframe == 6) && rb >= half - 3 && rb < half + 3 && l == 2) alloc = 0;
        } else {
          if ((subframe == 0 || subframe == 5) && rb >= half - 3 && rb < half + 3 && l == (nsymb >> 1) - 2) alloc = 0;
          if ((subframe == 0 || subframe == 5) && rb >= half - 3 && rb < half + 3 && l == (nsymb >> 1) - 1) alloc = 0;
        }
      }
      if (alloc) {
        int first = 0, last = 12, re_off = re_offset, par = 0;
        if (skip_half == 1) last = 6;
        else if (skip_half == 2) first = 6;
        for (int re = first; re < last; re++) {
          if (skip_dc && re == 6) re_off = re_off - N + 1;
          if (!not_pilot(pilots, re, fp->nushift, use2nd)) continue;
          int k = re_off + re;
          if (k < 0 || k >= N) return -1;
          if (alm) {
            int k2 = k + (not_pilot(pilots, re + 1, fp->nushift, use2nd) ? 1 : 2);
            if (k2 >= N || remap[l * N + k] != 0xFFFF || remap[l * N + k2] != 0xFFFF) return -1;
            remap[l * N + k] = (uint16_t)idx;
            remap[l * N + k2] = (uint16_t)(idx | 1u);
            idx += 2;
            ralloc += 2;
            re++;
            if (!not_pilot(pilots, re, fp->nushift, use2nd)) {
              re++;
              ralloc++;
            }
            continue;
          }
          if (prec1)
            remap[l * N + k] = (uint16_t)(idx | ((uint32_t)oai4g_get_pmi(fp->N_RB_DL, (uint8_t)mimo_mode, pmi_alloc, (uint16_t)rb)
                                                 << OAI4G_MOD_PMI_SHIFT));
          else
            remap[l * N + k] = (uint16_t)(idx | (par << 15));
          idx++;
          ralloc++;
          par ^= 1;
        }
      }
      re_offset += 12;
      if (re_offset >= N) re_offset = skip_dc == 0 ? 1 : 7;
    }
    total += idx;
  }
  if (re_alloc) *re_alloc = ralloc;
  return (int)total;
}

struct oai4g_tx_config {
  oai4g_tx_params_t p;
  oai4g_frame_parms_t fp;
  cfg_dev_t h;
  dev_buf<cfg_dev_t> d;
  dev_buf<uint16_t> d_remap;
  std::vector<uint16_t> h_remap;
  dev_buf<uint32_t> d_gold;
  dev_buf<enc_rv_tab_t> d_rvtab;
  std::vector<uint32_t> h_crs;
  std::vector<uint32_t> h_ctl;
  uint32_t ctl_planes = 2;
  dev_buf<uint32_t> d_stat;
  int ctl_vmax = 0;
  std::vector<oai4g_dci_alloc_t> dci;
  uint8_t n_ue_dci = 0, n_common_dci = 0;
  bool common_on = false;
  oai4g_common_sig_t common;
  int re_count[10];
  int re_alloc[10];
  hipStream_t s_mod = nullptr;
  hipEvent_t ev_enc[OAI4G_PIPE_MAX_CHUNKS] = {};
  hipEvent_t ev_done = nullptr;
  int pipe_chunk = 0;
  ~oai4g_tx_config()
  {
    for (auto &e : ev_enc)
      if (e) hipEventDestroy(e);
    if (ev_done) hipEventDestroy(ev_done);
    if (s_mod) hipStreamDestroy(s_mod);
  }
};

static void rm_plan(cw_dev_t &c, int ki)
{
  const uint32_t R = c.Rk[ki], ND = c.NDk[ki], Ncb = c.Ncbk[ki], Nnn = c.Nnnk[ki], k0c = c.k0ck[ki];
  const uint32_t tz = c.t0k[ki], nt = c.ntk[ki], sw = c.stream_words;
  memset(c.rm_dst[ki], 0, sizeof(c.rm_dst[ki]));
  c.rm_wrapt[ki] = ~0u;
  for (uint32_t t = 0; t <= OAI4G_RM_TILES; t++)
    for (uint32_t L = 0; L < 32; L++) c.rm_src[ki][t][L] = 1u << 5;
  for (uint32_t t = 0; t < nt; t++) {
    const bool il = t >= tz;
// ... 40 lines not shown
  for (uint32_t ki = 0; ki < 2; ki++)
    if ((ki ? n0 < C : n0 > 0) && (nt[ki] < 1 || nt[ki] > OAI4G_RM_TILES)) return -1;
  uint32_t n = 0;
  for (uint32_t r = 0; r < C; r++) {
    const uint32_t ki = r >= n0 ? 1u : 0u, pp = (nt[ki] + 1) / 2;
    pair0[r] = n;
    for (uint32_t p = 0; p < pp; p++) {
      const uint32_t t0 = 2 * p, row = ki * ((OAI4G_RM_TILES + 1) * 32) + t0 * 32;
      const uint32_t wrap = wrapt[ki] - t0 < 2u ? 1u : 0u;
      pairs[n++] = wrap | (ki << 1) | (r << 2) | ((4 * row) << 16);
    }
  }
  pair0[C] = n;
  return (int)n;
}

extern "C" int oai4g_qpp_fold32(uint32_t K, uint32_t *s_out, uint16_t *tab)
{
  const int qi = oai4g_qpp_index(K);
  if (qi < 0 || oai4g_qpp_table[qi].K != K) return -1;
  if (K & 1023u) return 0;
  const uint64_t f1 = oai4g_qpp_table[qi].f1, f2 = oai4g_qpp_table[qi].f2;
  const uint32_t Q = K >> 5;
  auto pi = [&](uint64_t k) { return (uint32_t)((f1 * k + f2 * k * k) % K); };
  const uint32_t d = (pi(Q) + K - pi(0)) % K;
  if (d % Q) return 0;
  const uint32_t s = d / Q;
  if (!(s & 1u)) return 0;
  for (uint32_t k = 0; k < K; k++)
    if ((pi(k + Q) + K - pi(k)) % K != d) return 0;
  uint32_t si = 1;
  while (((si * s) & 31u) != 1u) si += 2;
  *s_out = s;
  for (uint32_t k = 0; k < Q; k++) {
    const uint32_t x = pi(k);
    tab[k] = (uint16_t)(((x % Q) << 7) | ((si * (x / Q)) & 31u));
  }
  return 1;
}

static void rm_condition_exit(const rm_ncb_t &g, uint32_t Nsoft)
{
  printf("Exiting, RM condition (Nir %u, Nsoft %u, Kw %u\n", g.Nir, Nsoft, g.Kw);
}

static uint32_t rm_k0c_of_rv(const cw_dev_t &c, uint32_t ki, uint32_t R, uint32_t Ncb, uint32_t rv)
{
  return rm_compact(rm_k0(R, Ncb, rv), rm_null_list{c.nullpos[ki], c.nnull[ki]});
}

static int derive_cfg(oai4g_tx_config *cfg, const oai4g_tx_params_t *p, const uint8_t Nl[2], bool need_remap,
                      int only_sf)
{
  memset(&cfg->h, 0, sizeof(cfg->h));
  cfg->p = *p;
  oai4g_frame_parms_t &fp = cfg->fp;
  if (oai4g_init_frame_parms(&fp, p->N_RB_DL, p->Nid_cell, p->Ncp, p->nb_antennas_tx, p->mode1_flag,
                             p->frame_type) != 0)
    return -1;
  cfg_dev_t &h = cfg->h;
  if (p->n_cw < 1 || p->n_cw > 2) { set_err("n_cw must be 1 or 2"); return -1; }
  const bool prec1 = oai4g_mode_prec1(p->mimo_mode);
  if (p->mimo_mode != OAI4G_SISO && p->mimo_mode != OAI4G_LARGE_CDD && p->mimo_mode != OAI4G_ALAMOUTI && !prec1) {
    set_err("mimo_mode %u not supported (SISO, ALAMOUTI, LARGE_CDD and the single-layer precoding modes 3..8)", p->mimo_mode);
    return -1;
  }
  if (prec1 && (p->n_cw != 1 || p->nb_antennas_tx > 2)) {
    set_err("single-layer precoding (mimo_mode %u) takes one codeword and at most 2 TX antennas (dlsch_modulation.c:750)",
            p->mimo_mode);
    return -1;
  }
  if (p->pmi_alloc > 0xFFFFu) { set_err("pmi_alloc %#x: only the low 16 bits may be set", p->pmi_alloc); return -1; }
  if (p->mimo_mode == OAI4G_ALAMOUTI && (p->nb_antennas_tx != 2 || p->n_cw != 1)) {
    set_err("ALAMOUTI requires 2 TX antennas and one codeword (dlsch_modulation.c:362)");
    return -1;
  }
  if (p->mimo_mode == OAI4G_LARGE_CDD && ((p->nb_antennas_tx != 2 && p->nb_antennas_tx != 4) || p->n_cw != 2)) {
    set_err("LARGE_CDD requires 2 (dlsch_modulation.c:551) or 4 (C4 extension) TX antennas and 2 codewords");
    return -1;
  }
  if (p->nb_antennas_tx == 4 && p->mimo_mode != OAI4G_LARGE_CDD) {
    set_err("4 TX antennas: LARGE_CDD only (C4 extension)");
    return -1;
  }
  if (p->payload_stride % 4) { set_err("payload_stride must be a multiple of 4"); return -1; }
  h.N_RB_DL = fp.N_RB_DL;
  h.N = fp.ofdm_symbol_size;
  h.log2N = fp.log2_symbol_size;
  h.cp0 = fp.nb_prefix_samples0;
  h.cp = fp.nb_prefix_samples;
  h.spt = fp.samples_per_tti;
  h.nsymb = fp.symbols_per_tti;
  h.n_ant = fp.nb_antennas_tx;
  h.first_carrier = fp.first_carrier_offset;
  h.n_cw = p->n_cw;
  h.mimo_mode = p->mimo_mode;
  h.num_pdcch = p->num_pdcch_symbols;
  h.rnti = p->rnti;
  h.Nid_cell = p->Nid_cell;
  h.first_sf = p->first_subframe % 10;
  h.sf_step = p->subframe_step;
  h.payload_stride = p->payload_stride;
  for (uint32_t v = 0; v < 256; v++) {
    uint32_t ra = v << 16, rb = v << 16;
    for (int i = 0; i < 8; i++) {
      ra = (ra & 0x800000u) ? ((ra << 1) ^ 0x864cfbu) & 0xffffffu : (ra << 1) & 0xffffffu;
      rb = (rb & 0x800000u) ? ((rb << 1) ^ 0x800063u) & 0xffffffu : (rb << 1) & 0xffffffu;
    }
    h.crctab[0][v] = ra;
    h.crctab[1][v] = rb;
  }
  uint32_t max_tb_words = 0, max_stream_words = 0, max_gw = 0, max_bits = 0, max_w = 0, max_inw = 0;
  bool rm_fail = false;
  for (int cw = 0; cw < p->n_cw; cw++) {
    cw_dev_t &c = h.cw[cw];
    c.TBS = p->TBS[cw];
    if (c.TBS == 0 || (c.TBS & 7)) { set_err("TBS[%d]=%u must be a positive multiple of 8", cw, c.TBS); return -1; }
    c.A_bytes = c.TBS >> 3;
    if (p->payload_stride < ((c.A_bytes + 3) & ~3u)) {
      set_err("payload_stride %u < TBS/8 rounded to 4 (%u)", p->payload_stride, (c.A_bytes + 3) & ~3u);
      return -1;
    }
    c.Qm = oai4g_get_Qm(p->mcs[cw]);
    c.q = p->q[cw];
    uint32_t C, Cp, Cm, Kp, Km, F, L;
    if (seg_params(c.TBS + 24, &C, &Cp, &Cm, &Kp, &Km, &F, &L) < 0) { set_err("segmentation failed"); return -1; }
    c.C = C; c.Cminus = Cm; c.Kplus = Kp; c.Kminus = Km; c.F = F; c.L = L;
    uint32_t src = 0, maxK = 0;
    for (uint32_t r = 0; r < C; r++) {
      uint32_t K = r < Cm ? Km : Kp;
      int qi = oai4g_qpp_index(K);
      if (qi < 0) { set_err("illegal code block size %u", K); return -1; }
      c.K[r] = K;
      c.f1[r] = oai4g_qpp_table[qi].f1;
      c.f2[r] = oai4g_qpp_table[qi].f2;
      c.fill[r] = r == 0 ? F / 8 : 0;
      c.ncopy[r] = (K - L) / 8 - c.fill[r];
      c.src[r] = src;
      src += c.ncopy[r];
      maxK = K > maxK ? K : maxK;
      uint32_t D = K + 4, R = (D + 31) >> 5, Kpi = R << 5;
      c.R[r] = R; c.Kpi[r] = Kpi; c.ND[r] = Kpi - D;
      const rm_ncb_t g = rm_ncb(OAI4G_NSOFT, p->Kmimo, p->Mdlharq, C, R);
      c.Ncb[r] = g.Ncb;
      if (g.shorter && !p->rm_limited_buffer) {
        rm_condition_exit(g, OAI4G_NSOFT);
        set_err("RM condition: Ncb %u < Kw %u (the reference emits E=0, lte_rate_matching.c:518-521)", g.Ncb, g.Kw);
        rm_fail = true;
        c.Ncb[r] = g.Kw;
      }
      c.kidx[r] = (C > 1 && r < Cm) ? 0 : 1;
    }
    if (src != (c.TBS + 24) / 8) { set_err("segmentation byte accounting mismatch"); return -1; }
    for (int ki = 0; ki < 2; ki++) {
      uint32_t K = ki == 0 ? Km : Kp;
      if (K == 0 || (ki == 0 && !(C > 1 && Cm > 0))) continue;
      int qi = oai4g_qpp_index(K);
      uint64_t f1 = oai4g_qpp_table[qi].f1, f2 = oai4g_qpp_table[qi].f2;
      for (uint32_t j = 0; j < (K + 31) / 32; j++) {
        uint64_t k = 8 * j;
        uint32_t pi = (uint32_t)((f1 * k + f2 * k * k) % K), pi1 = (uint32_t)((f1 * (k + 1) + f2 * (k + 1) * (k + 1)) % K);
        c.qpp0[ki][j] = pi | (((pi1 + K - pi) % K) << 16);
      }
      memset(c.qpp_tab[ki], 0, sizeof(c.qpp_tab[ki]));
      for (uint64_t k = 0; k < K / 4; k++) {
        const uint32_t x = (uint32_t)((f1 * k + f2 * k * k) % K), Q = K / 4, xp = x % Q, u = x / Q;
        const uint32_t rot = (8 * u + (xp & 7) + 32 - (uint32_t)(k & 7)) & 31u;
        c.qpp_tab[ki][k >> 1] |= (((xp >> 3) << 7) | rot) << (16 * (k & 1));
      }
      c.qpp_s3[ki] = (uint32_t)((f1 * (K / 4)) % K) == K / 4 ? 0u : 1u;
      static_assert(sizeof(c.qpp_tab[0]) >= OAI4G_MAX_CHUNKS * sizeof(uint16_t), "32-fold entries fit qpp_tab");
      uint32_t s32 = 0;
      uint16_t t32[OAI4G_MAX_CHUNKS];
      if (oai4g_qpp_fold32(K, &s32, t32) == 1) {
        memset(c.qpp_tab[ki], 0, sizeof(c.qpp_tab[ki]));
        memcpy(c.qpp_tab[ki], t32, (K / 32) * sizeof(uint16_t));
        c.qpp_f32[ki] = s32 | ((((1u << 20) + K / 1024 - 1) / (K / 1024)) << 5);
      }
    }
    {
      uint32_t o = 0;
      for (uint32_t r = 0; r < C; r++) {
        c.ilv_off[r] = o;
        o += (c.K[r] + 31) / 32;
      }
      c.ilv_off[C] = o;
      c.n0 = (C > 1) ? Cm : 0;
      c.kk[0] = c.n0 ? Km : Kp;
      c.kk[1] = Kp;
      for (int ki = 0; ki < 2; ki++) {
        c.kw[ki] = (c.kk[ki] + 31) / 32;
        c.kmag[ki] = ((1u << 20) + c.kw[ki] - 1) / c.kw[ki];
      }
      c.u0 = c.n0 * c.kw[0];
    }
    c.crc_per_tb = (((c.A_bytes + 255) / 256) + 3) & ~3u;
    crc_mul_tables(c.crc_per_tb, 8, 0x864cfbu, c.crcmul_tb);
    crc_mul_tables2(c.crc_per_tb, 0x864cfbu, c.crc2_tb);
    uint32_t ncb_max = 0;
    for (uint32_t r = 0; r < C; r++) {
      uint32_t n = c.ncopy[r];
      if (c.src[r] + n > c.A_bytes) n = c.A_bytes > c.src[r] ? c.A_bytes - c.src[r] : 0;
      ncb_max = n > ncb_max ? n : ncb_max;
    }
    c.crc_lpb = C <= 4 ? 64u : (C <= 8 ? 32u : 16u);
    c.crc_per_cb = (((ncb_max + c.crc_lpb - 1) / c.crc_lpb) + 3) & ~3u;
    crc_mul_tables2(c.crc_per_cb ? c.crc_per_cb : 1, 0x864cfbu, c.crc2_cb[0]);
    crc_mul_tables2(c.crc_per_cb ? c.crc_per_cb : 1, 0x800063u, c.crc2_cb[1]);
    for (uint32_t r = 0; r < C; r++) {
      uint32_t end = c.src[r] + c.ncopy[r];
      if (end > c.A_bytes) end = c.A_bytes;
      const uint32_t m = crc_xpow8_h(c.A_bytes - (end > c.src[r] ? end : c.src[r]), 0x864cfbu);
      for (int k = 0; k < 6; k++)
        for (uint32_t v = 0; v < 16; v++) c.crcmul_blk[r][16 * k + v] = crc_mulmod_h((v << (4 * k)) & 0xffffffu, m, 0x864cfbu);
    }
    for (int ki = 0; ki < 2; ki++) {
      uint32_t K = ki == 0 ? (Km ? Km : Kp) : Kp;
      int n = null_positions(K, c.nullpos[ki], OAI4G_MAX_NULLS);
      if (n < 0) { set_err("too many NULL positions"); return -1; }
      c.nnull[ki] = (uint32_t)n;
    }
    for (uint32_t r = 0; r < C; r++) {
      c.k0c[r] = rm_k0c_of_rv(c, c.kidx[r], c.R[r], c.Ncb[r], p->rvidx[cw]);
      c.Nnn[r] = rm_compact(c.Ncb[r], rm_null_list{c.nullpos[c.kidx[r]], c.nnull[c.kidx[r]]});
    }
    uint32_t nw = (maxK + 31) >> 5;
    c.stream_words = nw + 3;
    uint32_t inw = 0;
    for (uint32_t r = 0; r < C; r++) inw += (c.K[r] + 31) >> 5;
    max_inw = inw > max_inw ? inw : max_inw;
    uint32_t wwords = 0, ntask = 0;
    for (uint32_t r = 0; r < C; r++) {
      c.wpk_off[r] = wwords;
      wwords += 3 * c.R[r] + 2;
      for (uint32_t rb = 0; rb < (c.R[r] + 31) / 32; rb++) c.tasks[ntask++] = (uint16_t)(r | (rb << 5));
      for (uint32_t rb = 0; rb < (c.R[r] + 15) / 16; rb++) c.tasks[ntask++] = (uint16_t)(r | (1u << 4) | (rb << 5));
    }
    c.wpk_off[C] = wwords;
    c.ntask = ntask;
    for (uint32_t r = 0; r < C; r++) {
      const uint32_t ki = r < c.n0 ? 0 : 1;
      if (c.K[r] != c.kk[ki]) { set_err("block size order"); return -1; }
      c.Rk[ki] = c.R[r]; c.NDk[ki] = c.ND[r]; c.Ncbk[ki] = c.Ncb[r]; c.Nnnk[ki] = c.Nnn[r]; c.k0ck[ki] = c.k0c[r];
    }
    for (uint32_t r = 0; r < C; r++) {
      const uint32_t ki = r < c.n0 ? 0 : 1;
      if (c.R[r] != c.Rk[ki] || c.ND[r] != c.NDk[ki] || c.Ncb[r] != c.Ncbk[ki] || c.Nnn[r] != c.Nnnk[ki] ||
          c.k0c[r] != c.k0ck[ki] || c.kidx[r] != ki) {
        set_err("per-size block geometry differs");
        return -1;
      }
    }
    if (c.n0 == 0) { c.Rk[0] = c.Rk[1]; c.NDk[0] = c.NDk[1]; c.Ncbk[0] = c.Ncbk[1]; c.Nnnk[0] = c.Nnnk[1]; c.k0ck[0] = c.k0ck[1]; }
    for (int ki = 0; ki < 2; ki++) {
      c.nullcol[ki][0] = c.nullcol[ki][1] = 0;
      for (uint32_t wc = 0; wc < 32; wc++) {
        uint32_t pc = 0;
        for (int b = 0; b < 5; b++) pc |= ((wc >> b) & 1u) << (4 - b);
        if (pc < c.NDk[ki]) c.nullcol[ki][0] |= 1u << wc;
        if (pc + 1 < c.NDk[ki]) c.nullcol[ki][1] |= 1u << wc;
      }
      c.t0k[ki] = (c.Rk[ki] + 31) / 32;
      c.ntk[ki] = c.t0k[ki] + (c.Rk[ki] + 15) / 16;
      c.ntmag[ki] = ((1u << 20) + c.ntk[ki] - 1) / c.ntk[ki];
      if (c.ntk[ki] > OAI4G_RM_TILES) { set_err("rate-matching plan: %u tiles", c.ntk[ki]); return -1; }
      rm_plan(c, ki);
    }
    if (oai4g_rm_pair_schedule(C, c.n0, c.ntk, c.rm_wrapt, c.rm_pairs, c.rm_pair0) < 0) {
      set_err("rate-matching pair schedule");
      return -1;
    }
    max_w = wwords > max_w ? wwords : max_w;
    uint32_t tbw = (c.A_bytes + 3 + 3) / 4 + 1;
    max_tb_words = tbw > max_tb_words ? tbw : max_tb_words;
    uint32_t strw = C * 3 * c.stream_words;
    max_stream_words = strw > max_stream_words ? strw : max_stream_words;
    for (int sf = 0; sf < 10; sf++) {
      int G;
      if (fp.nb_antennas_tx == 4) {
        std::vector<uint16_t> tmp((size_t)14 * fp.ofdm_symbol_size);
        uint32_t sb[14];
        int n = build_remap(&fp, p->rb_alloc, p->num_pdcch_symbols, sf, p->mimo_mode, (uint16_t)p->pmi_alloc, tmp.data(), sb,
                            nullptr);
        G = n < 0 ? -1 : n * (int)c.Qm;
      } else {
        G = oai4g_get_G(&fp, p->nb_rb, p->rb_alloc, (uint8_t)c.Qm, Nl[cw], p->num_pdcch_symbols, 0, (uint8_t)sf);
      }
      if (G <= 0 || G > OAI4G_MAX_CHANNEL_BITS) { set_err("G=%d out of range", G); return -1; }
      c.G[sf] = (uint32_t)G;
      uint32_t off = 0;
      for (uint32_t r = 0; r < C; r++) {
        c.E[sf][r] = rm_E((uint32_t)G, Nl[cw], c.Qm, C, r);
        c.roff[sf][r] = off;
        off += c.E[sf][r];
      }
      c.roff[sf][C] = off;
      c.esplit[sf] = rm_esplit((uint32_t)G, Nl[cw], c.Qm, C);
      for (int h = 0; h < 2; h++) {
        const uint32_t E = c.E[sf][h ? C - 1 : 0], w = (E + 31) / 32;
        c.ew[sf][h] = w;
        c.emag[sf][h] = w ? (uint32_t)(((1ull << 32) + w - 1) / w) : 0u;
      }
      uint32_t gw = (off + 31) / 32;
      max_gw = gw > max_gw ? gw : max_gw;
      max_bits = (uint32_t)G > max_bits ? (uint32_t)G : max_bits;
    }
// ... 5438 lines not shown
```

openair4g_amd/csrc/oai4g_internal.h:

```cpp
#pragma once
#include <hip/hip_runtime.h>
#include <stdint.h>

#include "../../include/oai4g.h"

#define OAI4G_MAX_CB 16
#define OAI4G_MAX_NULLS 104
#define OAI4G_MAX_CHUNKS 192
#define OAI4G_MAX_TASKS (OAI4G_MAX_CB * 20)
#define OAI4G_RM_TILES 20
#define OAI4G_RM_SRC_LAST (1u << 20)
#define OAI4G_RM_DST_WRAP (1u << 27)
#define OAI4G_PIPE_MAX_CHUNKS 16
#define OAI4G_CRS_CODE 0xE000u
#define OAI4G_CTL_CODE 0xC000u
static constexpr uint32_t oai4g_mod_entry_shift(uint32_t mimo_mode, uint32_t n_ant, uint32_t log2N)
{
  return log2N != 11 ? 1u : mimo_mode == OAI4G_LARGE_CDD && n_ant == 2 ? 3u : mimo_mode == OAI4G_SISO ? 2u : 1u;
}
static constexpr uint32_t oai4g_mod_addr_mask(uint32_t shift) { return 0x7FFFu & ~((1u << shift) - 1u); }
static constexpr uint32_t oai4g_mod_sentinel(uint32_t N) { return (3u * N) / 4u; }
static constexpr bool oai4g_mode_prec1(uint32_t mimo_mode)
{
  return mimo_mode >= OAI4G_UNIFORM_PRECODING11 && mimo_mode <= OAI4G_PUSCH_PRECODING1;
}
#define OAI4G_MOD_PMI_SHIFT 12u
static constexpr uint32_t oai4g_mod_pmi_bits = 3u << OAI4G_MOD_PMI_SHIFT;
static constexpr uint32_t oai4g_mod_pmi_idx_mask = (1u << OAI4G_MOD_PMI_SHIFT) - 1u;
static_assert(2u * (oai4g_mod_sentinel(2048) + 4u) <= (1u << OAI4G_MOD_PMI_SHIFT), "staged offsets must stay below the precoder bits");
static constexpr bool oai4g_mod_nre_fits(uint32_t nre, uint32_t N) { return nre + 3u <= oai4g_mod_sentinel(N); }
struct oai4g_mod_item_t {
  uint32_t sf, l, pair;
};
static constexpr uint32_t oai4g_mod_permag(uint32_t per) { return (uint32_t)(((1ull << 32) + per - 1) / per); }
static inline __host__ __device__ oai4g_mod_item_t oai4g_mod_item(uint32_t item, uint32_t ips, uint32_t lz, uint32_t per,
                                                                  uint32_t permag)
{
  const uint32_t it = item / ips;
  const uint32_t sf = (uint32_t)(((uint64_t)it * permag) >> 32);
  return {sf, lz + it - sf * per, item - it * ips};
}
#define OAI4G_MOD_LZ_MAX 4u
#define OAI4G_ENC_CRC_TABLE_WORDS (256 + 256)
#define OAI4G_GOLD_LANES 256
#define OAI4G_GOLD_STRIDE 17
#define OAI4G_MAX_GOLD_WORDS (OAI4G_GOLD_LANES * OAI4G_GOLD_STRIDE)
#define OAI4G_TW_TOTAL (16 + 64 + 128 + 256 + 512 + 1024 + 2048)

typedef uint32_t __attribute__((aligned(1))) u32_a1_t;
static __device__ __forceinline__ uint32_t ld_u32_any(const uint8_t *p)
{
  return *(const __attribute__((address_space(1))) u32_a1_t *)p;
}

static inline __host__ __device__ uint64_t oai4g_payload_word(uint64_t seed, uint64_t w)
{
  uint64_t z = seed + 0x9e3779b97f4a7c15ull * (w + 1);
  z = (z ^ (z >> 30)) * 0xbf58476d1ce4e5b9ull;
  z = (z ^ (z >> 27)) * 0x94d049bb133111ebull;
  return z ^ (z >> 31);
}

static inline __host__ __device__ uint32_t oai4g_tw_offset(int log2s)
{
  switch (log2s) {
  case 4: return 0;
  case 6: return 16;
  case 7: return 80;
  case 8: return 208;
  case 9: return 464;
  case 10: return 976;
  case 11: return 2000;
  default: return 0;
  }
}

struct cw_dev_t {
  uint32_t TBS;
  uint32_t A_bytes;
  uint32_t C, Cminus, Kplus, Kminus, F, L;
  uint32_t Qm;
  uint32_t q;
  uint32_t K[OAI4G_MAX_CB];
  uint32_t f1[OAI4G_MAX_CB], f2[OAI4G_MAX_CB];
  uint32_t src[OAI4G_MAX_CB];
  uint32_t fill[OAI4G_MAX_CB];
  uint32_t ncopy[OAI4G_MAX_CB];
  uint32_t crc_off[OAI4G_MAX_CB];
  uint32_t R[OAI4G_MAX_CB], Kpi[OAI4G_MAX_CB], ND[OAI4G_MAX_CB], Ncb[OAI4G_MAX_CB];
  uint32_t Nnn[OAI4G_MAX_CB];
  uint32_t k0c[OAI4G_MAX_CB];
  uint32_t kidx[OAI4G_MAX_CB];
  uint32_t wpk_off[OAI4G_MAX_CB + 1];
  uint32_t ntask;
  uint16_t tasks[OAI4G_MAX_TASKS];
  uint32_t ilv_off[OAI4G_MAX_CB + 1];
  uint32_t qpp0[2][OAI4G_MAX_CHUNKS];
  alignas(16) uint32_t qpp_tab[2][OAI4G_MAX_CHUNKS * 4];
  uint32_t qpp_f32[2];
  uint32_t qpp_s3[2];
  uint32_t n0, u0, kk[2], kw[2], kmag[2];
  uint32_t Rk[2], NDk[2], Ncbk[2], Nnnk[2], k0ck[2];
  uint32_t ntk[2], t0k[2], ntmag[2];
  uint32_t rm_wrapt[2];
  uint32_t nullcol[2][2];
  uint32_t esplit[10], ew[10][2], emag[10][2];
  uint32_t nnull[2];
  uint16_t nullpos[2][OAI4G_MAX_NULLS];
  uint32_t G[10];
  uint32_t E[10][OAI4G_MAX_CB];
  uint32_t roff[10][OAI4G_MAX_CB + 1];
  int16_t qam_a[8], qam_b[8];
  int16_t qpsk_a, qpsk_b;
  int16_t alm_qpsk[2][2];
  uint32_t stream_words;
  uint32_t crc_per_tb;
  uint32_t crc_per_cb;
  uint32_t crc_lpb;
  uint32_t crcmul_tb[8][6][16];
  uint32_t crcmul_blk[OAI4G_MAX_CB][96];
  uint32_t crc2_tb[2][8][96];
  uint32_t crc2_cb[2][2][8][96];
  uint32_t rm_src[2][OAI4G_RM_TILES + 1][32];
  uint32_t rm_dst[2][OAI4G_RM_TILES + 1][32];
  uint32_t rm_pair0[OAI4G_MAX_CB + 1];
  uint32_t rm_pairs[OAI4G_MAX_CB * ((OAI4G_RM_TILES + 1) / 2)];
};

struct cfg_dev_t {
  uint32_t N_RB_DL, N, log2N, cp0, cp, spt, nsymb, n_ant, first_carrier;
  uint32_t n_cw, mimo_mode, num_pdcch, rnti, Nid_cell, first_sf, sf_step;
  uint32_t payload_stride;
  uint32_t ebits_words;
  uint32_t lds_tb_words;
  uint32_t lds_stream_words;
  uint32_t lds_gold_words;
  uint32_t lds_w_words;
  uint32_t lds_a_words;
  uint32_t lds_b_words;
  uint32_t mod_nosat;
  uint32_t mod_lz, mod_per, mod_permag;
  uint32_t crctab[2][256];
  cw_dev_t cw[2];
  uint32_t symbase[10][14];
  uint32_t symnre[10][14];
  uint32_t n_cu;
  const uint16_t *remap;
  const uint16_t *remap_tm;
  uint32_t with_crs;
  uint32_t pilmask;
  uint32_t ctlmask[10];
  uint32_t ctl_on;
  const uint32_t *gold_tab;
  const uint32_t *gold_x1;
  const uint32_t *gold_x2j;
  const uint32_t *tw;
  const uint32_t *stat_tm;
  uint32_t stat_planes;
  uint32_t pad2;
};

struct enc_rv_tab_t {
  uint32_t rm_dst[2][OAI4G_RM_TILES + 1][32];
  uint32_t rm_pair0[OAI4G_MAX_CB + 1];
  uint32_t rm_pairs[OAI4G_MAX_CB * ((OAI4G_RM_TILES + 1) / 2)];
  uint32_t rm_wrapt[2];
  uint32_t k0ck[2];
  uint32_t pad[3];
};
static_assert(sizeof(enc_rv_tab_t) % 16 == 0, "tables are laid out back to back");

hipError_t oai4g_launch_encode_rv(const cfg_dev_t *d_cfg, const cfg_dev_t *h_cfg, int n_sf, const uint8_t *d_payload,
                                  const uint8_t *d_rv, const enc_rv_tab_t *d_tabs, uint32_t *d_ebits, hipStream_t s);
hipError_t oai4g_launch_encode(const cfg_dev_t *d_cfg, const cfg_dev_t *h_cfg, int sf0, int n_sf,
                               const uint8_t *d_payload, uint32_t *d_ebits, hipStream_t s);
hipError_t oai4g_encode_occupancy(const cfg_dev_t *h_cfg, int *blocks_per_cu, size_t *lds_bytes);
hipError_t oai4g_launch_encode_phase(const cfg_dev_t *d_cfg, const cfg_dev_t *h_cfg, int n_sf,
                                     const uint8_t *d_payload, uint32_t *d_ebits, int stop_phase, hipStream_t s);
struct enc_debug_t {
  uint8_t *c;
  uint8_t *d;
  uint8_t *w;
  uint8_t *e;
  uint8_t *b;
};
hipError_t oai4g_launch_encode_debug(const cfg_dev_t *d_cfg, const cfg_dev_t *h_cfg, int cw, int sf,
                                     const uint8_t *d_payload, enc_debug_t dbg, hipStream_t s);
hipError_t oai4g_launch_crc24(const uint8_t *d_in, int bitlen, uint32_t poly_top, uint32_t *d_out, hipStream_t s);
hipError_t oai4g_launch_turbo_bytes(const uint8_t *d_c, int nbytes, uint8_t *d_out, uint32_t f1, uint32_t f2,
                                    hipStream_t s);
hipError_t oai4g_launch_subblock_bytes(uint32_t D, const uint8_t *d_dfull, uint8_t *d_w, hipStream_t s);
hipError_t oai4g_launch_rm_bytes(const uint8_t *d_w, uint32_t Ncb, uint32_t k0, uint32_t E, uint8_t *d_e,
                                 uint32_t *d_status, hipStream_t s);
struct rm_blk_t {
  uint32_t woff, Ncb, k0, E, eoff, pad[3];
};
hipError_t oai4g_launch_rm_bytes_blocks(const uint8_t *d_w, const rm_blk_t *d_blk, int C, uint32_t max_Ncb, uint8_t *d_e,
                                        uint32_t *d_status, hipStream_t s);
hipError_t oai4g_launch_scramble_bytes(uint8_t *d_e, int n_entries, uint32_t c_init, const uint32_t *d_gold_x1,
                                       const uint32_t *d_gold_x2j, hipStream_t s);
hipError_t oai4g_launch_fill(uint8_t *d, size_t bytes, uint64_t seed, hipStream_t s);
struct crs_job_t {
  uint32_t off;
  uint8_t Ns, l, p, pad;
};
hipError_t oai4g_launch_crs(int32_t *d_out, const crs_job_t *jobs, int n_jobs, const uint32_t *d_gold, int16_t amp,
                            uint32_t N, uint32_t N_RB, uint32_t nushift, uint32_t first_carrier, hipStream_t s);
hipError_t oai4g_launch_diag_stream(const void *src, void *dst, size_t bytes, int mode, hipStream_t s);

size_t oai4g_td_block_bytes(uint32_t K);
hipError_t oai4g_launch_td16(int n_cb, uint32_t K, const int16_t *d_llr, size_t llr_stride, uint8_t *d_out,
                             size_t out_stride, uint8_t *d_iters, uint32_t max_it, uint32_t crc_type, uint32_t F,
                             const uint16_t *d_pi , uint8_t *d_scratch, hipStream_t s,
                             uint32_t cg = 1, uint32_t c_per = 1, uint32_t r0 = 0);
size_t oai4g_td8_wave_bytes(uint32_t K);
hipError_t oai4g_launch_td8(int n_cb, uint32_t K, const int16_t *d_llr, size_t llr_stride, uint8_t *d_out,
                            size_t out_stride, uint8_t *d_iters, uint32_t max_it, uint32_t crc_type, uint32_t F,
                            const uint16_t *d_pi, uint8_t *d_scratch, hipStream_t s);
#define OAI4G_UL_MAX_C 16
struct ul_pat_t {
  uint32_t D, R, Ncb, Nnn, k0c;
  uint32_t k0cr[4];
  const uint8_t *dummy;
  const uint32_t *cidx;
};
struct ul_dev_t {
  uint32_t C, Rmax;
  uint32_t E[OAI4G_UL_MAX_C], off[OAI4G_UL_MAX_C], pat_of[OAI4G_UL_MAX_C];
  ul_pat_t pat[3];
};
hipError_t oai4g_launch_ul_rm_deint(const ul_dev_t *d_cfg, const ul_dev_t *h_cfg, int n_tb, const int16_t *d_e,
                                    size_t e_stride, int16_t *d_dfull, size_t d_stride, hipStream_t s);
hipError_t oai4g_launch_ul_rm_harq(const ul_dev_t *d_cfg, const ul_dev_t *h_cfg, int n_tb, const int16_t *d_e,
                                   size_t e_stride, int16_t *d_w, size_t w_stride, uint32_t rv, int clear,
                                   int16_t *d_dfull, size_t d_stride, hipStream_t s);
hipError_t oai4g_launch_ul_rm_harq_tb(const ul_dev_t *d_cfg, const ul_dev_t *h_cfg, int n_tb, const int16_t *d_e,
                                      size_t e_stride, int16_t *d_w, size_t w_stride, const uint8_t *d_rv,
                                      const uint8_t *d_clear, int16_t *d_dfull, size_t d_stride, hipStream_t s);
hipError_t oai4g_launch_rm_rx(const int16_t *d_soft, uint32_t E, int16_t *d_w, const uint8_t *d_dummy,
                              const uint32_t *d_cidx, uint32_t Ncb, uint32_t Nnn, uint32_t k0c, int clear, hipStream_t s);
hipError_t oai4g_launch_subblock_deint(uint32_t D, int16_t *d_dfull, const int16_t *d_w, hipStream_t s);

extern int g_modofdm_grid_cap;
hipError_t oai4g_launch_modofdm(const cfg_dev_t *d_cfg, const cfg_dev_t *h_cfg, int sf0, int n_sf,
                                const uint32_t *d_ebits, int32_t *d_iq, hipStream_t s);
struct ofdm_sym_t {
  uint32_t in_off;
  uint32_t out_off;
  uint32_t cp;
};
hipError_t oai4g_launch_ofdm(const int32_t *d_in, int32_t *d_out, int log2n, int nsym, const ofdm_sym_t *syms,
                             int scale, const uint32_t *d_tw, hipStream_t s);
hipError_t oai4g_launch_idft_strided(const int32_t *d_in, int32_t *d_out, int log2n, int n_jobs, size_t in_stride,
                                     uint32_t in_off, size_t out_stride, int scale, const uint32_t *d_tw, hipStream_t s);
hipError_t oai4g_launch_freq_offset(const int32_t *d_est, size_t est_stride, int n_jobs, int N_RB, uint32_t row_off,
                                    uint32_t prev_off, int32_t *d_omega, hipStream_t s);
struct pcfich_args_t {
  uint32_t c_init;
  uint32_t cfi;
  int16_t gain;
  uint8_t mode1;
  uint8_t nushift3;
  uint32_t reg_off[4];
  uint32_t n_ant;
};
hipError_t oai4g_launch_pcfich(int32_t *d_g0, int32_t *d_g1, const pcfich_args_t &a, hipStream_t s);

#define OAI4G_MAX_DCI 32
struct dci_dev_t {
  uint8_t flip[8];
  uint32_t A;
  uint32_t L;
  int32_t nCCE;
  uint32_t rnti;
};
struct dci_args_t {
  uint32_t n_dci;
  dci_dev_t dci[OAI4G_MAX_DCI];
  uint32_t nbits;
  uint32_t c_init;
  uint32_t n_re;
  int16_t gain;
  uint8_t mode1;
  uint8_t n_ant;
};
hipError_t oai4g_launch_dci(const dci_args_t &a, const uint32_t *d_map, const uint16_t *d_src, int32_t *d_g0,
                            int32_t *d_g1, uint32_t g1_stride, hipStream_t s);

struct sync_args_t {
  int16_t val[62][2];
  int16_t a;
  uint8_t pss;
  uint8_t n_ant;
  uint32_t N;
};
hipError_t oai4g_launch_sync(int32_t *const *d_sym , const sync_args_t &a,
                             hipStream_t s);
struct pbch_args_t {
  uint8_t a[3];
  uint8_t encode;
  uint16_t amask;
  uint16_t E;
  uint32_t Nid;
  uint32_t quarter;
  uint32_t N;
  uint32_t pil_mask;
  uint32_t nushift3;
  int16_t gain;
  uint8_t mode1;
  uint8_t n_ant;
};
hipError_t oai4g_launch_pbch(int32_t *const *d_g, uint8_t *d_e, const pbch_args_t &a, hipStream_t s);
#define OAI4G_MAX_PHICH 64
struct phich_item_t {
  uint32_t c_init;
  uint32_t reg_off[3];
  uint8_t nseq, hi;
};
struct phich_args_t {
  uint32_t n;
  phich_item_t it[OAI4G_MAX_PHICH];
  int16_t gain;
  uint8_t mode1;
  uint8_t n_ant;
  uint32_t nushift;
  uint32_t win;
};
hipError_t oai4g_launch_phich(int32_t *const *d_g, int32_t *d_acc, const phich_args_t &a, hipStream_t s);

#define OAI4G_FEP_MAX_SYM 14
struct fep_args_t {
  int n_units;
  int nsym;
  uint32_t in_stride, in_len, out_stride;
  uint32_t in_off[OAI4G_FEP_MAX_SYM];
  uint32_t out_off[OAI4G_FEP_MAX_SYM];
  int scale;
};
hipError_t oai4g_launch_fep(const int32_t *d_in, int32_t *d_out, int log2n, const fep_args_t &a,
                            const uint32_t *d_twf, int n_cu, hipStream_t s);
hipError_t oai4g_launch_modulate_bytes(const cfg_dev_t *d_cfg, const cfg_dev_t *h_cfg, int sf,
                                       const uint8_t *d_e0, const uint8_t *d_e1, int32_t *d_grid, hipStream_t s);

struct chest_dev_t {
  uint32_t N, N_RB, nsymb, Ncp, fco, p;
  uint32_t first_sf, sf_step;
  uint32_t branch;
  uint32_t k[2];
  uint32_t off2[2];
  uint32_t elem_syms;
  uint32_t next_syms;
  int16_t filt[2][8][24];
  uint32_t gold[20][2][14];
};
struct cc_job_t {
  uint32_t e_off;
  uint16_t E;
  uint16_t D;
  uint16_t plan_off;
  uint16_t crc_bits;
};
struct cc_args_t {
  const int8_t *e;
  size_t e_stride;
  const cc_job_t *jobs;
  uint32_t n_jobs, n_items;
  const uint16_t *plan;
  const uint32_t *gold;
  const uint8_t *quarter;
  uint8_t *out;
  uint32_t out_stride;
  uint8_t *metrics;
  uint32_t raw;
  uint32_t pbch_out;
  const uint32_t *tab;
  uint32_t tab_stride;
  const int16_t *comp;
  size_t comp_stride;
  uint32_t first_row;
};
#define OAI4G_PDCCH_NONE 0xFFFFFFFFu
static inline __host__ __device__ int8_t oai4g_pdcch_soft(const int16_t *comp, uint32_t t)
{
  if (t == OAI4G_PDCCH_NONE) return 0;
  const int v = comp[t & 0x7FFFFFFFu];
  const int c = v > 31 ? 31 : (v < -32 ? -32 : v);
  return (int8_t)((t >> 31) ? -c : c);
}
hipError_t oai4g_launch_pdcch_soft(const int16_t *d_comp, const uint32_t *d_tab, uint32_t n, int8_t *d_e, hipStream_t s);

typedef oai4g_pdcch_plan_t pdcch_plan_t;
struct pdcch_cand_t {
  uint16_t cce;
  uint8_t plan;
  uint8_t first;
};
// ... 280 lines not shown
```

Baseline: 9.475 million subframes/s.

## Make encode kernel persistent with next-codeword payload prefetch and host segment tables

Converts k_encode from one workgroup per codeword into a persistent grid sized by occupancy times CU count, looping over codewords. While rate matching runs on the current codeword, it prefetches the first payload block of the next one into registers, and it hoists CRC/RSC table loads out of the loop. Per-segment fill/offset/slab flags are now precomputed on the host into a constant table instead of being derived per thread. This is meant to hide payload load latency and cut per-block setup, at the cost of extra registers (waves_per_eu hint) and possible load imbalance from the capped grid.

```diff
diff --git a/include/oai4g.h b/include/oai4g.h
--- a/include/oai4g.h
+++ b/include/oai4g.h
@@ -112,12 +112,14 @@
 uint32_t oai4g_lte_gold_generic(uint32_t *x1, uint32_t *x2, uint8_t reset);
 int oai4g_qpp_fold32(uint32_t K, uint32_t *s, uint16_t *tab);
 int oai4g_rsc_scan_rows(uint32_t q, uint32_t rows[6]);
+int oai4g_diag_enc_seg_rows(uint32_t tbs_bits, uint32_t *rows);
 int oai4g_rm_pair_schedule(uint32_t C, uint32_t n0, const uint32_t nt[2], const uint32_t wrapt[2],
                            uint32_t *pairs, uint32_t *pair0);
 int oai4g_mod_item_map(uint32_t item, uint32_t ips, uint32_t lz, uint32_t per, uint32_t *sf, uint32_t *l,
                        uint32_t *pair);
 uint8_t oai4g_get_pmi(uint8_t N_RB_DL, uint8_t mimo_mode, uint16_t pmi_alloc, uint16_t rb);
 void oai4g_set_modofdm_grid_cap(int n_workgroups);
+void oai4g_set_encode_grid_cap(int n_workgroups);
 
 uint32_t oai4g_crc24a(const uint8_t *in, int bitlen);
 uint32_t oai4g_crc24b(const uint8_t *in, int bitlen);
diff --git a/openair4g_amd/__init__.py b/openair4g_amd/__init__.py
--- a/openair4g_amd/__init__.py
+++ b/openair4g_amd/__init__.py
@@ -344,6 +344,8 @@
                                           ctypes.POINTER(ctypes.c_uint32)]),
     "oai4g_get_pmi": (ctypes.c_uint8, [ctypes.c_uint8, ctypes.c_uint8, ctypes.c_uint16, ctypes.c_uint16]),
     "oai4g_set_modofdm_grid_cap": (None, [ctypes.c_int]),
+    "oai4g_set_encode_grid_cap": (None, [ctypes.c_int]),
+    "oai4g_diag_enc_seg_rows": (ctypes.c_int, [ctypes.c_uint32, ctypes.POINTER(ctypes.c_uint32)]),
     "oai4g_tx_mod_lz": (ctypes.c_int, [ctypes.c_void_p]),
     "oai4g_harq_advance": (ctypes.c_int, [ctypes.c_int, ctypes.c_int, ctypes.c_uint8, ctypes.c_int, ctypes.c_int]
                            + [ctypes.c_void_p] * 8 + [ctypes.c_size_t, ctypes.c_uint64, ctypes.c_void_p]),
diff --git a/openair4g_amd/csrc/oai4g_encode.hip b/openair4g_amd/csrc/oai4g_encode.hip
--- a/openair4g_amd/csrc/oai4g_encode.hip
+++ b/openair4g_amd/csrc/oai4g_encode.hip
@@ -241,9 +241,8 @@
   return reg;
 }
 
-static __device__ __forceinline__ uint32_t crc_wave_tree2(uint32_t reg, const uint32_t (*mul)[8][96])
-{
-  const uint32_t lane = threadIdx.x & 63;
+static __device__ __forceinline__ uint32_t crc_wave_tree2(uint32_t reg, const uint32_t (*mul)[8][96], uint32_t lane)
+{
   reg = crc_mul_tab(reg, mul[0][7 - (lane & 7)]);
   reg ^= __shfl_xor(reg, 1, 64);
   reg ^= __shfl_xor(reg, 2, 64);
@@ -314,9 +313,8 @@
 }
 
 static __device__ __forceinline__ void turbo_segment(const uint32_t *in, uint32_t *par_out, uint32_t K,
-                                                     uint32_t *tail_out, const enc_tabs_t *tb)
-{
-  const uint32_t lane = threadIdx.x & 63;
+                                                     uint32_t *tail_out, const enc_tabs_t *tb, uint32_t lane)
+{
   const uint32_t nch = (K + 31) >> 5;
   const uint32_t lq = nch <= 64 ? 0 : (nch <= 128 ? 1 : 2), qp = 1u << lq;
   uint32_t u[4], v[4];
@@ -390,10 +388,10 @@
 
 template <int Q>
 static __device__ __forceinline__ void turbo_segment32(const uint32_t *in, uint32_t *par_out, uint32_t nch,
-                                                       uint32_t *tail_out, const enc_tabs_t *tb)
+                                                       uint32_t *tail_out, const enc_tabs_t *tb, uint32_t lane)
 {
   constexpr uint32_t A1 = rsc_prop_packed(32), AQinv = rsc_prop_packed(7 - (32 * Q) % 7);
-  const uint32_t lane = threadIdx.x & 63, j0 = lane * Q, last = nch - 1;
+  const uint32_t j0 = lane * Q, last = nch - 1;
   uint32_t v[Q], S = 0;
 #pragma unroll
   for (int t = 0; t < Q; t++) {
@@ -571,14 +569,94 @@
   atomicOr(p + 1, (uint32_t)(s >> 32));
 }
 
+struct enc_keep_t {
+  uint32_t ca, cb, rn, rp, ra, rz;
+};
+
+static __device__ __forceinline__ enc_keep_t enc_keep_load(const cfg_dev_t *__restrict__ c)
+{
+  const uint32_t tid = threadIdx.x, tv = __builtin_bitreverse32(tid) >> 24, tr = tid & 127u;
+  enc_keep_t k;
+  const uint32_t ta = c->crctab[0][tv], tb = c->crctab[1][tv];
+  k.rn = (&c_rsc.next[0][0])[tr];
+  k.rp = (&c_rsc.par[0][0])[tr];
+  k.ra = (&c_rsc.apow[0][0])[tr & 63u];
+  k.rz = c_rsc.zs[tr & 7u];
+  k.ca = __builtin_bitreverse32(ta << 8) << 2;
+  k.cb = __builtin_bitreverse32(tb << 8) << 2;
+  return k;
+}
+
+struct enc_seg_t {
+  uint32_t C, n0, cb0, cb1, F8, Ab;
+  __device__ __forceinline__ void of(uint32_t r, uint32_t &fill, uint32_t &ncopy, uint32_t &s0) const
+  {
+    const uint32_t ki = r >= n0 ? 1u : 0u;
+    fill = r == 0 ? F8 : 0u;
+    ncopy = (ki ? cb1 : cb0) - fill;
+    s0 = r == 0 ? 0u : (ki ? n0 * cb0 + (r - n0) * cb1 : r * cb0) - F8;
+  }
+};
+
+static __device__ __forceinline__ enc_seg_t enc_seg(const cw_dev_t &cw)
+{
+  enc_seg_t g;
+  const uint32_t L8 = __builtin_amdgcn_readfirstlane(cw.L) >> 3;
+  g.C = __builtin_amdgcn_readfirstlane(cw.C);
+  g.n0 = cw.n0;
+  g.F8 = __builtin_amdgcn_readfirstlane(cw.F) >> 3;
+  g.cb0 = (__builtin_amdgcn_readfirstlane(cw.kk[0]) >> 3) - L8;
+  g.cb1 = (__builtin_amdgcn_readfirstlane(cw.kk[1]) >> 3) - L8;
+  g.Ab = cw.A_bytes;
+  return g;
+}
+
+struct enc_segrow_t {
+  uint32_t fill, x, dend, w;
+};
+static __device__ __forceinline__ enc_segrow_t enc_seg_row(const cw_dev_t &cw, uint32_t r)
+{
+  typedef uint32_t u32x4_t __attribute__((ext_vector_type(4)));
+  const u32x4_t q = *(const __attribute__((address_space(4))) u32x4_t *)cw.seg_tab[r];
+  return {q.x, q.y, q.z, q.w};
+}
+
+constexpr uint32_t ENC_BLK = 6;
+
+static __device__ __forceinline__ void enc_payload_issue(const cw_dev_t &cw, const uint8_t *__restrict__ src,
+                                                         uint32_t rb, uint32_t tid, uint32_t (&v)[ENC_BLK])
+{
+  const uint32_t i0 = 4 * tid, C = __builtin_amdgcn_readfirstlane(cw.C), lim = cw.seg_lim;
+#pragma unroll
+  for (uint32_t u = 0; u < ENC_BLK; u++) {
+    const uint32_t r = rb + u;
+    v[u] = 0;
+    if (r >= C) break;
+    const enc_segrow_t g = enc_seg_row(cw, r);
+    const uint32_t a = max(i0, g.fill) + g.x;
+    v[u] = ld_u32_any(src + min(a, lim));
+  }
+}
+
+static __device__ __forceinline__ void enc_prefetch(const cw_dev_t &cw, const uint8_t *__restrict__ src, uint32_t tid,
+                                                    uint32_t (&pv)[ENC_BLK])
+{
+  if (__builtin_amdgcn_readfirstlane(tid >> 6) < cw.seg_nsl) enc_payload_issue(cw, src, 0, tid, pv);
+}
+
+constexpr uint32_t ENC_NO_NEXT = ~0u;
+
 template <bool DEBUG, bool RV = false>
-static __device__ void encode_codeword(const cfg_dev_t *__restrict__ c, uint32_t sf, uint32_t cwi,
+static __device__ __forceinline__ bool encode_codeword(const cfg_dev_t *__restrict__ c, uint32_t sf, uint32_t cwi,
                                        const uint8_t *__restrict__ payload, uint32_t *__restrict__ ebits,
-                                       enc_debug_t dbg, uint32_t *lds_base, int stop_phase = 99, uint32_t sf0 = 0,
-                                       const enc_rv_tab_t *__restrict__ rvt = nullptr)
+                                       enc_debug_t dbg, uint32_t *lds_base, const enc_keep_t &keep,
+                                       uint32_t (&pv)[ENC_BLK], uint32_t next = ENC_NO_NEXT, int stop_phase = 99,
+                                       uint32_t sf0 = 0, const enc_rv_tab_t *__restrict__ rvt = nullptr)
 {
   const cw_dev_t &cw = c->cw[cwi];
-  const uint32_t tid = threadIdx.x, nth = blockDim.x, lane = tid & 63, nwaves = nth >> 6;
+  uint32_t tid = threadIdx.x;
+  asm volatile("" : "+v"(tid));
+  const uint32_t nth = blockDim.x, lane = tid & 63, nwaves = nth >> 6;
   const uint32_t wave = __builtin_amdgcn_readfirstlane(tid >> 6);
   const uint32_t sfi = DEBUG ? sf : (c->first_sf + (sf0 + sf) * c->sf_step) % 10;
   const uint32_t C = __builtin_amdgcn_readfirstlane(cw.C), sw = __builtin_amdgcn_readfirstlane(cw.stream_words);
@@ -596,47 +674,26 @@
   const uint32_t kw0 = __builtin_amdgcn_readfirstlane(cw.kw[0]), kw1 = __builtin_amdgcn_readfirstlane(cw.kw[1]);
   const uint32_t km0 = __builtin_amdgcn_readfirstlane(cw.kmag[0]), km1 = __builtin_amdgcn_readfirstlane(cw.kmag[1]);
   const uint32_t kk0 = __builtin_amdgcn_readfirstlane(cw.kk[0]), kk1 = __builtin_amdgcn_readfirstlane(cw.kk[1]);
-  const uint32_t L8 = __builtin_amdgcn_readfirstlane(cw.L) >> 3, F8 = __builtin_amdgcn_readfirstlane(cw.F) >> 3;
-  const uint32_t cb0 = (kk0 >> 3) - L8, cb1 = (kk1 >> 3) - L8;
-  auto seg_of = [&](uint32_t r, uint32_t &fill, uint32_t &ncopy, uint32_t &s0) {
-    const uint32_t ki = r >= n0 ? 1u : 0u;
-    fill = r == 0 ? F8 : 0u;
-    ncopy = (ki ? cb1 : cb0) - fill;
-    s0 = r == 0 ? 0u : (ki ? n0 * cb0 + (r - n0) * cb1 : r * cb0) - F8;
-  };
+  const enc_seg_t sg = enc_seg(cw);
+  const uint32_t F8 = sg.F8;
+  auto seg_of = [&](uint32_t r, uint32_t &fill, uint32_t &ncopy, uint32_t &s0) { sg.of(r, fill, ncopy, s0); };
 
   const uint8_t *src = payload + (size_t)(DEBUG ? 0 : (sf * c->n_cw + cwi)) * c->payload_stride;
   const uint32_t Ab = cw.A_bytes;
   {
-    constexpr uint32_t ENC_BLK = 6;
-    const uint32_t nsl = (kw1 + 63) >> 6;
-    const uint32_t lim = ((Ab + 3) & ~3u) - 4;
-    for (uint32_t sl = wave; sl < nsl; sl += nwaves) {
-      const uint32_t j0 = sl << 6, j = j0 + lane, i0 = 4 * j;
-      for (uint32_t rb = 0; rb < C; rb += ENC_BLK) {
-        uint32_t v[ENC_BLK];
-#pragma unroll
-        for (uint32_t u = 0; u < ENC_BLK; u++) {
-          const uint32_t r = rb + u;
-          v[u] = 0;
-          if (r >= C) break;
-          uint32_t fill, ncopy, s0;
-          seg_of(r, fill, ncopy, s0);
-          const uint32_t a = s0 + (i0 > fill ? i0 - fill : 0u);
-          v[u] = ld_u32_any(src + min(a, lim));
-        }
+    const uint32_t lim = cw.seg_lim;
+    if (wave < cw.seg_nsl) {
+      const uint32_t sl = wave, j = (sl << 6) + lane, i0 = 4 * j;
+      auto consume = [&](uint32_t rb, const uint32_t (&v)[ENC_BLK]) {
 #pragma unroll
         for (uint32_t u = 0; u < ENC_BLK; u++) {
           const uint32_t r = rb + u;
           if (r >= C) break;
-          const uint32_t kw = r < n0 ? kw0 : kw1;
-          if (j0 >= kw) continue;
-          uint32_t fill, ncopy, s0;
-          seg_of(r, fill, ncopy, s0);
-          const uint32_t nd = s0 + ncopy > Ab ? (Ab > s0 ? Ab - s0 : 0u) : ncopy;
-          const uint32_t dend = fill + nd;
+          const enc_segrow_t g = enc_seg_row(cw, r);
+          if (!(g.w & (OAI4G_SEG_SLAB << sl))) continue;
+          const uint32_t kw = g.w & 0xffffu, fill = g.fill, dend = g.dend, s0 = g.x + fill;
           uint32_t *sys = strm + r * 3 * sw;
-          if ((sl == 0 && fill != 0) || 4 * (j0 + 64) > dend) {
+          if (g.w & (OAI4G_SEG_EXACT << sl)) {
             if (j < kw) {
               const int pre = (int)fill - (int)i0, valid = (int)dend - (int)i0;
               const uint32_t a = s0 + (pre < 0 ? (uint32_t)-pre : 0u);
@@ -650,6 +707,12 @@
             sys[j] = bytes_to_seq(v[u]);
           }
         }
+      };
+      consume(0, pv);
+      for (uint32_t rb = ENC_BLK; rb < C; rb += ENC_BLK) {
+        uint32_t v[ENC_BLK];
+        enc_payload_issue(cw, src, rb, tid, v);
+        consume(rb, v);
       }
     }
     for (uint32_t i = tid; i < C * 3 * 4; i += nth) {
@@ -658,23 +721,17 @@
       if (w < sw) strm[slot * sw + w] = 0u;
     }
     if (tid == 0) crcs[0] = 0u;
-    {
-      const uint32_t tv = __builtin_bitreverse32(tid) >> 24, tr = tid & 127u;
-      const uint32_t ta = c->crctab[0][tv], tb = c->crctab[1][tv];
-      const uint32_t rsc_n = (&c_rsc.next[0][0])[tr], rsc_p = (&c_rsc.par[0][0])[tr];
-      const uint32_t rsc_a = (&c_rsc.apow[0][0])[tr & 63u], rsc_z = c_rsc.zs[tr & 7u];
-      crctab_a[tid] = __builtin_bitreverse32(ta << 8) << 2;
-      if (C > 1) crctab_b[tid] = __builtin_bitreverse32(tb << 8) << 2;
-      if (tid < 128) {
-        (&tabs->next[0][0])[tid] = (uint8_t)rsc_n;
-        (&tabs->par[0][0])[tid] = (uint8_t)rsc_p;
-        if (tid < 64) (&tabs->apow[0][0])[tid] = (uint8_t)rsc_a;
-        if (tid < 8) tabs->zs[tid] = rsc_z;
-      }
+    crctab_a[tid] = keep.ca;
+    if (C > 1) crctab_b[tid] = keep.cb;
+    if (tid < 128) {
+      (&tabs->next[0][0])[tid] = (uint8_t)keep.rn;
+      (&tabs->par[0][0])[tid] = (uint8_t)keep.rp;
+      if (tid < 64) (&tabs->apow[0][0])[tid] = (uint8_t)keep.ra;
+      if (tid < 8) tabs->zs[tid] = keep.rz;
     }
   }
   __syncthreads();
-  if (stop_phase <= 0) return;
+  if (stop_phase <= 0) return false;
 
   if (C > 1) {
     const uint32_t lpb = __builtin_amdgcn_readfirstlane(cw.crc_lpb), per = __builtin_amdgcn_readfirstlane(cw.crc_per_cb);
@@ -718,7 +775,7 @@
       p[5] = (uint8_t)(vb >> 16);
     }
   } else {
-    const uint32_t reg = crc_wave_tree2(crc_chunk_w1r(strm, F8, Ab, cw.crc_per_tb, tid, nth, (const uint8_t *)crctab_a), cw.crc2_tb);
+    const uint32_t reg = crc_wave_tree2(crc_chunk_w1r(strm, F8, Ab, cw.crc_per_tb, tid, nth, (const uint8_t *)crctab_a), cw.crc2_tb, lane);
     if (lane == 0) red[wave] = reg;
     __syncthreads();
     if (tid == 0) {
@@ -738,7 +795,7 @@
     for (uint32_t i = tid; i < Ab; i += nth) dbg.b[i] = src[i];
     if (tid < 3) dbg.b[Ab + tid] = (uint8_t)(crcs[0] >> (8 * (2 - tid)));
   }
-  if (stop_phase <= 2) return;
+  if (stop_phase <= 2) return false;
 
   auto unit_of = [&](uint32_t i, uint32_t &r, uint32_t &j, uint32_t &K, uint32_t &ki) {
     ki = i >= u0 ? 1u : 0u;
@@ -857,7 +914,7 @@
     }
   }
   __syncthreads();
-  if (stop_phase == 23) return;
+  if (stop_phase == 23) return false;
 
   for (uint32_t seg = wave; seg < 2 * C; seg += nwaves) {
     const uint32_t r = seg >> 1, e = seg & 1u;
@@ -866,13 +923,13 @@
     const uint32_t *in = e ? ilv + io : blk;
     uint32_t *par = blk + (1 + e) * sw, *tail = &tails[2 * r + e];
     const uint32_t K = r < n0 ? kk0 : kk1, nch = K >> 5;
-    if (K & 31u) turbo_segment(in, par, K, tail, tabs);
-    else if (nch > 128) turbo_segment32<3>(in, par, nch, tail, tabs);
-    else if (nch > 64) turbo_segment32<2>(in, par, nch, tail, tabs);
-    else turbo_segment32<1>(in, par, nch, tail, tabs);
+    if (K & 31u) turbo_segment(in, par, K, tail, tabs, lane);
+    else if (nch > 128) turbo_segment32<3>(in, par, nch, tail, tabs, lane);
+    else if (nch > 64) turbo_segment32<2>(in, par, nch, tail, tabs, lane);
+    else turbo_segment32<1>(in, par, nch, tail, tabs, lane);
   }
   __syncthreads();
-  if (stop_phase <= 3) return;
+  if (stop_phase <= 3) return false;
 
   if (DEBUG) {
     for (uint32_t r = 0; r < C; r++) {
@@ -902,7 +959,7 @@
         }
       }
     }
-    if (!dbg.e) return;
+    if (!dbg.e) return false;
   }
 
   const uint32_t nd0 = __builtin_amdgcn_readfirstlane(cw.NDk[0]), nd1 = __builtin_amdgcn_readfirstlane(cw.NDk[1]);
@@ -946,6 +1003,10 @@
       for (uint32_t i = tid; i < nwh + 1; i += nth) ebuf[i] = (i == 0 && h) ? carry : 0u;
       __syncthreads();
       const uint32_t pb = ppair0[rb0], pe = ppair0[rb1], bit0 = 32 * w0;
+      if (!DEBUG && h == 0 && next != ENC_NO_NEXT) {
+        const uint32_t ncwi = c->n_cw == 2 ? next & 1u : 0u;
+        enc_prefetch(c->cw[ncwi], payload + (size_t)next * c->payload_stride, tid, pv);
+      }
       const char *rsrc0 = (const char *)&cw.rm_src[0][0][0];
       const char *rdst0 = (const char *)(RV ? &rvt->rm_dst[0][0][0] : &cw.rm_dst[0][0][0]);
       auto pair_loop = [&](auto ONCE) {
@@ -1005,7 +1066,7 @@
       __syncthreads();
       if (DEBUG) {
         for (uint32_t k = tid; k < G; k += nth) dbg.e[k] = (uint8_t)((ebuf[k >> 5] >> (k & 31)) & 1u);
-        return;
+        return false;
       }
       const uint32_t nst = stop_phase <= 4 ? 0u : ((h + 1 < nhalf && (eb1 & 31u)) ? nwh - 1 : nwh);
       for (uint32_t i = tid; i < nst; i += nth) {
@@ -1021,15 +1082,31 @@
       }
     }
   }
-}
-
-__global__ void __launch_bounds__(256) __attribute__((amdgpu_num_sgpr(80))) k_encode(const cfg_dev_t *__restrict__ c, const uint8_t *__restrict__ payload,
-                                                uint32_t *__restrict__ ebits, int stop_phase, uint32_t sf0)
+  return next != ENC_NO_NEXT;
+}
+
+__global__ void __launch_bounds__(256) __attribute__((amdgpu_num_sgpr(80), amdgpu_waves_per_eu(8))) k_encode(const cfg_dev_t *__restrict__ c, const uint8_t *__restrict__ payload,
+                                                uint32_t *__restrict__ ebits, int stop_phase, uint32_t sf0, uint32_t n_cwt)
 {
   extern __shared__ uint32_t lds_dyn[];
-  uint32_t sf = blockIdx.x / c->n_cw, cwi = blockIdx.x % c->n_cw;
-  enc_debug_t none = {nullptr, nullptr, nullptr, nullptr, nullptr};
-  encode_codeword<false>(c, sf, cwi, payload, ebits, none, lds_dyn, stop_phase, sf0);
+  const enc_debug_t none = {nullptr, nullptr, nullptr, nullptr, nullptr};
+  const enc_keep_t keep = enc_keep_load(c);
+  const bool two = c->n_cw == 2;
+  uint32_t pv[ENC_BLK];
+  bool have = false;
+  for (uint32_t i = blockIdx.x; i < n_cwt; i += gridDim.x) {
+    const uint32_t sf = two ? i >> 1 : i, cwi = two ? i & 1u : 0u;
+    uint32_t zero = 0;
+    asm volatile("" : "+s"(zero));
+    const cfg_dev_t *cc = (const cfg_dev_t *)((const char *)c + zero);
+    int sp = stop_phase;
+    asm volatile("" : "+s"(sp));
+    if (!have) enc_prefetch(cc->cw[cwi], payload + (size_t)i * cc->payload_stride, threadIdx.x, pv);
+    const uint32_t nx = i + gridDim.x;
+    have = encode_codeword<false>(cc, sf, cwi, payload, ebits, none, lds_dyn, keep, pv, nx < n_cwt ? nx : ENC_NO_NEXT, sp,
+                                  sf0);
+    __syncthreads();
+  }
 }
 
 __global__ void __launch_bounds__(256) __attribute__((amdgpu_num_sgpr(80))) k_encode_rv(const cfg_dev_t *__restrict__ c, const uint8_t *__restrict__ payload,
@@ -1040,14 +1117,21 @@
   uint32_t sf = blockIdx.x / c->n_cw, cwi = blockIdx.x % c->n_cw;
   const uint32_t v = __builtin_amdgcn_readfirstlane((uint32_t)rv[blockIdx.x]) & 3u;
   enc_debug_t none = {nullptr, nullptr, nullptr, nullptr, nullptr};
-  encode_codeword<false, true>(c, sf, cwi, payload, ebits, none, lds_dyn, 99, 0, tabs + (v * c->n_cw + cwi));
+  const enc_keep_t keep = enc_keep_load(c);
+  uint32_t pv[ENC_BLK];
+  enc_prefetch(c->cw[cwi], payload + (size_t)blockIdx.x * c->payload_stride, threadIdx.x, pv);
+  encode_codeword<false, true>(c, sf, cwi, payload, ebits, none, lds_dyn, keep, pv, ENC_NO_NEXT, 99, 0,
+                               tabs + (v * c->n_cw + cwi));
 }
 
 __global__ void __launch_bounds__(256) k_encode_debug(const cfg_dev_t *__restrict__ c, uint32_t sf, uint32_t cwi,
                                                       const uint8_t *__restrict__ payload, enc_debug_t dbg)
 {
   extern __shared__ uint32_t lds_dyn[];
-  encode_codeword<true>(c, sf, cwi, payload, nullptr, dbg, lds_dyn);
+  const enc_keep_t keep = enc_keep_load(c);
+  uint32_t pv[ENC_BLK];
+  enc_prefetch(c->cw[cwi], payload, threadIdx.x, pv);
+  encode_codeword<true>(c, sf, cwi, payload, nullptr, dbg, lds_dyn, keep, pv);
 }
 
 static size_t enc_lds_bytes(const cfg_dev_t *h)
@@ -1088,8 +1172,19 @@
     (void)hipFuncSetAttribute((const void *)k_encode_debug, hipFuncAttributeMaxDynamicSharedMemorySize, 160 * 1024);
     attr_set = true;
   }
-  hipLaunchKernelGGL(k_encode, dim3(n_sf * h_cfg->n_cw), dim3(256), lds, s, d_cfg, d_payload, d_ebits, stop_phase,
-                     (uint32_t)sf0);
+  static size_t occ_lds = ~(size_t)0;
+  static int occ = 1;
+  if (occ_lds != lds) {
+    if (hipOccupancyMaxActiveBlocksPerMultiprocessor(&occ, k_encode, 256, lds) != hipSuccess || occ < 1) occ = 1;
+    occ_lds = lds;
+  }
+  const int n_cwt = n_sf * (int)h_cfg->n_cw;
+  int cap = occ * (int)h_cfg->n_cu;
+  if (g_encode_grid_cap > 0 && g_encode_grid_cap < cap) cap = g_encode_grid_cap;
+  int grid = n_cwt < cap ? n_cwt : cap;
+  if (grid < 1) grid = 1;
+  hipLaunchKernelGGL(k_encode, dim3(grid), dim3(256), lds, s, d_cfg, d_payload, d_ebits, stop_phase, (uint32_t)sf0,
+                     (uint32_t)n_cwt);
   return hipGetLastError();
 }
 
@@ -1184,7 +1279,7 @@
   for (uint32_t j = threadIdx.x; j < nw; j += blockDim.x) ilv[j] = qpp_gather_word(strm, K, qpp_start(K, f1, f2, j), d2, j);
   __syncthreads();
   uint32_t wave = threadIdx.x >> 6;
-  if (wave < 2) turbo_segment(wave ? ilv : strm, strm + (1 + wave) * sw, K, &tails[wave], &tabs);
+  if (wave < 2) turbo_segment(wave ? ilv : strm, strm + (1 + wave) * sw, K, &tails[wave], &tabs, threadIdx.x & 63);
   __syncthreads();
   for (uint32_t i = threadIdx.x; i < 3 * K + 12; i += blockDim.x) {
     uint32_t kk = i / 3, s = i - 3 * kk;
diff --git a/openair4g_amd/csrc/oai4g_host.cpp b/openair4g_amd/csrc/oai4g_host.cpp
--- a/openair4g_amd/csrc/oai4g_host.cpp
+++ b/openair4g_amd/csrc/oai4g_host.cpp
@@ -631,6 +631,38 @@
 
 int g_modofdm_grid_cap = 0;
 extern "C" void oai4g_set_modofdm_grid_cap(int n_workgroups) { g_modofdm_grid_cap = n_workgroups > 0 ? n_workgroups : 0; }
+int oai4g_enc_seg_rows(uint32_t tbs_bits, uint32_t rows[OAI4G_MAX_CB][4])
+{
+  uint32_t C, Cp, Cm, Kp, Km, F, L;
+  if (tbs_bits == 0 || (tbs_bits & 7) || seg_params(tbs_bits + 24, &C, &Cp, &Cm, &Kp, &Km, &F, &L) < 0 || C > OAI4G_MAX_CB) return -1;
+  const uint32_t A = tbs_bits >> 3;
+  uint32_t s0 = 0;
+  for (uint32_t r = 0; r < C; r++) {
+    const uint32_t K = r < Cm ? Km : Kp, kw = (K + 31) / 32;
+    const uint32_t fill = r == 0 ? F / 8 : 0, ncopy = (K - L) / 8 - fill;
+    const uint32_t nd = s0 + ncopy > A ? (A > s0 ? A - s0 : 0) : ncopy, dend = fill + nd;
+    uint32_t w = kw;
+    for (uint32_t sl = 0; 64 * sl < kw; sl++) {
+      w |= OAI4G_SEG_SLAB << sl;
+      if ((sl == 0 && fill != 0) || 4 * (64 * sl + 64) > dend) w |= OAI4G_SEG_EXACT << sl;
+    }
+    rows[r][0] = fill;
+    rows[r][1] = s0 - fill;
+    rows[r][2] = dend;
+    rows[r][3] = w;
+    s0 += ncopy;
+  }
+  return (int)C;
+}
+
+extern "C" int oai4g_diag_enc_seg_rows(uint32_t tbs_bits, uint32_t *rows )
+{
+  if (!rows) return -1;
+  return oai4g_enc_seg_rows(tbs_bits, (uint32_t (*)[4])rows);
+}
+
+int g_encode_grid_cap = 0;
+extern "C" void oai4g_set_encode_grid_cap(int n_workgroups) { g_encode_grid_cap = n_workgroups > 0 ? n_workgroups : 0; }
 
 extern "C" uint8_t oai4g_get_pmi(uint8_t N_RB_DL, uint8_t mimo_mode, uint16_t pmi_alloc, uint16_t rb)
 {
@@ -977,6 +1009,9 @@
       c.kidx[r] = (C > 1 && r < Cm) ? 0 : 1;
     }
     if (src != (c.TBS + 24) / 8) { set_err("segmentation byte accounting mismatch"); return -1; }
+    if (oai4g_enc_seg_rows(c.TBS, c.seg_tab) != (int)C) { set_err("segmentation table mismatch"); return -1; }
+    c.seg_lim = ((c.A_bytes + 3) & ~3u) - 4;
+    c.seg_nsl = ((Kp + 31) / 32 + 63) >> 6;
     for (int ki = 0; ki < 2; ki++) {
       uint32_t K = ki == 0 ? Km : Kp;
       if (K == 0 || (ki == 0 && !(C > 1 && Cm > 0))) continue;
diff --git a/openair4g_amd/csrc/oai4g_internal.h b/openair4g_amd/csrc/oai4g_internal.h
--- a/openair4g_amd/csrc/oai4g_internal.h
+++ b/openair4g_amd/csrc/oai4g_internal.h
@@ -125,7 +125,13 @@
   uint32_t rm_dst[2][OAI4G_RM_TILES + 1][32];
   uint32_t rm_pair0[OAI4G_MAX_CB + 1];
   uint32_t rm_pairs[OAI4G_MAX_CB * ((OAI4G_RM_TILES + 1) / 2)];
-};
+  alignas(16) uint32_t seg_tab[OAI4G_MAX_CB][4];
+  uint32_t seg_lim, seg_nsl;
+  uint32_t seg_pad[2];
+};
+#define OAI4G_SEG_SLAB (1u << 16)
+#define OAI4G_SEG_EXACT (1u << 20)
+int oai4g_enc_seg_rows(uint32_t tbs_bits, uint32_t rows[OAI4G_MAX_CB][4]);
 
 struct cfg_dev_t {
   uint32_t N_RB_DL, N, log2N, cp0, cp, spt, nsymb, n_ant, first_carrier;
@@ -242,6 +248,7 @@
 hipError_t oai4g_launch_subblock_deint(uint32_t D, int16_t *d_dfull, const int16_t *d_w, hipStream_t s);
 
 extern int g_modofdm_grid_cap;
+extern int g_encode_grid_cap;
 hipError_t oai4g_launch_modofdm(const cfg_dev_t *d_cfg, const cfg_dev_t *h_cfg, int sf0, int n_sf,
                                 const uint32_t *d_ebits, int32_t *d_iq, hipStream_t s);
 struct ofdm_sym_t {
```

Result: slower. 9.092 million subframes/s (-4.0%).
